# parsaeskandar/pangenome-index

Measured on AMD Instinct MI355X. Metric: find_mems reads/sec (150 bp batch), higher is better.
Workload: dtype u64

## Files before the change

### pangenome-index_amd/csrc/pgx_batch.hip

```cpp
#include <memory>
#include <string>
#include <thread>

#include "pgx_runtime_internal.hpp"

struct pgx_chunk { uint64_t r0, r1, slot_base, slots; };

struct CompactWork {
    DevBuf sizes, tab, bytes, scan_tmp;
    HostBuf h_tab, h_bytes;
    hipEvent_t ev[4] = {nullptr, nullptr, nullptr, nullptr};
    void release() {
        DevBuf *all[] = {&sizes, &tab, &bytes, &scan_tmp};
        for (DevBuf *d : all) d->release();
        h_tab.release(); h_bytes.release();
        for (auto &e : ev)
            if (e) { (void)hipEventDestroy(e); e = nullptr; }
    }
};

struct pgx_batch {
    pgx_index *h = nullptr;
    pgx_device_image *dimg = nullptr;
    int device = 0;
    hipStream_t own = nullptr;
    hipStream_t side = nullptr;
    hipEvent_t ev_side[2] = {nullptr, nullptr};
    bool class_valid = false, class_ok = false;
    uint64_t side_reads_est = 0;
    uint64_t n_reads = 0, read_bytes = 0;
    HostBuf h_off[2];
    int h_off_cur = 0;
    const uint64_t *h_offsets() const { return h_off[h_off_cur].as<uint64_t>(); }
    std::vector<pgx_chunk> chunks;
    bool plan_valid = false, slot_off_valid = false;
    uint64_t slot_off_min_len = 0;
    uint64_t plan_min_len = 0, plan_budget = 0;
    DevBuf reads, offsets;
    DevBuf slot_off, slots, mem_count, mem_off, mems, scan_tmp, counters, heavy_list, heavy_scratch, read_flags, side_list, side_count, packed, ovf_base;
    DevBuf up_side_ids, up_side_off, up_side_bytes;
    DevBuf fx_text, fx_tiles, fx_tile_base, fx_lines, fx_contrib, fx_rec, fx_out_off, fx_rec_idx, fx_offs, fx_scal, fx_scan_tmp;
    std::vector<uint64_t> h_side_off;
    hipEvent_t ev_up[2] = {nullptr, nullptr};
    float ms_upload_passes = 0;
    uint64_t last_ovf_used = 0;
    uint64_t max_read_len = 0;
    TagWork tw;
    LocWork lw;
    CompactWork cw;
    uint64_t n_mems = 0, n_positions = 0, n_ext = 0, n_tag_overflow = 0;
    bool ran = false, ran_tags = false;
    bool shape_valid = false;
    uint64_t shape_reads = 0, shape_min_len = 0, shape_min_occ = 0, last_mems = 0;
    bool shape_tags = false;
    uint32_t spec_runs = 0, spec_fallbacks = 0;
    HostBuf h_mem_off, h_mems, h_run_nums, h_pos_off, h_positions;
    hipEvent_t ev[10] = {nullptr, nullptr, nullptr, nullptr, nullptr, nullptr, nullptr, nullptr, nullptr, nullptr};
    bool timed = false;
    pgx_timing timing{};
};

static void batch_release(pgx_batch *b) {
    if (!b) return;
    if (hipSetDevice(b->device) == hipSuccess) {
        DevBuf *all[] = {&b->reads, &b->offsets, &b->slot_off, &b->slots, &b->mem_count, &b->mem_off, &b->mems, &b->scan_tmp,
                         &b->counters, &b->heavy_list, &b->heavy_scratch, &b->read_flags, &b->side_list, &b->side_count, &b->packed, &b->ovf_base,
                         &b->up_side_ids, &b->up_side_off, &b->up_side_bytes, &b->fx_text, &b->fx_tiles, &b->fx_tile_base, &b->fx_lines,
                         &b->fx_contrib, &b->fx_rec, &b->fx_out_off, &b->fx_rec_idx, &b->fx_offs, &b->fx_scal, &b->fx_scan_tmp};
        for (DevBuf *d : all) d->release();
        b->tw.release();
        b->lw.release();
        b->cw.release();
        HostBuf *hb[] = {&b->h_mem_off, &b->h_mems, &b->h_run_nums, &b->h_pos_off, &b->h_positions, &b->h_off[0], &b->h_off[1]};
        for (HostBuf *x : hb) x->release();
        for (auto &e : b->ev)
            if (e) { (void)hipEventDestroy(e); e = nullptr; }
        if (b->own) { (void)hipStreamDestroy(b->own); b->own = nullptr; }
        if (b->side) { (void)hipStreamDestroy(b->side); b->side = nullptr; }
        for (auto &e : b->ev_side)
            if (e) { (void)hipEventDestroy(e); e = nullptr; }
        for (auto &e : b->ev_up)
            if (e) { (void)hipEventDestroy(e); e = nullptr; }
    }
    delete b;
}

extern "C" void pgx_batch_free(pgx_batch *b) { batch_release(b); }

static void batch_reset_for_upload(pgx_batch *b, uint64_t n_reads, uint64_t max_read_len, uint64_t read_bytes) {
    b->h_off_cur ^= 1;
    b->n_reads = n_reads;
    b->ran = b->ran_tags = false;
    b->lw.valid = false;
    b->plan_valid = false;
    b->slot_off_valid = false;
    b->class_valid = false;
    b->ms_upload_passes = 0;
    b->max_read_len = max_read_len;
    b->read_bytes = read_bytes;
}

static void batch_take_offsets(pgx_batch *b, const uint64_t *offsets, uint64_t n_reads, const char *who) {
    const uint64_t lo = offsets[0];
    HostBuf &hb = b->h_off[b->h_off_cur ^ 1];
    hb.ensure((n_reads + 1) * 8);
    uint64_t *ho = hb.as<uint64_t>();
    ho[0] = 0;
    const unsigned nt = n_reads >= (1u << 20) ? 4u : 1u;
    uint64_t longest[4] = {0, 0, 0, 0};
    bool bad[4] = {false, false, false, false};
    auto slice = [&](unsigned t) {
        const uint64_t i0 = 1 + n_reads * t / nt, i1 = 1 + n_reads * (t + 1) / nt;
        uint64_t prev = offsets[i0 - 1], mx = 0;
        bool b_ = false;
        for (uint64_t i = i0; i < i1; i++) {
            const uint64_t o = offsets[i];
            b_ |= o < prev;
            mx = std::max(mx, o - prev);
            ho[i] = o - lo;
            prev = o;
        }
        longest[t] = mx; bad[t] = b_;
    };
    if (nt == 1) slice(0);
    else {
        std::thread th[3];
        for (unsigned t = 1; t < nt; t++) th[t - 1] = std::thread(slice, t);
        slice(0);
        for (unsigned t = 1; t < nt; t++) th[t - 1].join();
    }
    uint64_t mx = 0;
    for (unsigned t = 0; t < nt; t++) {
        if (bad[t]) throw Error(PGX_ERR_ARG, std::string(who) + ": offsets must be non-decreasing");
        mx = std::max(mx, longest[t]);
    }
    if (mx >= (1ull << 31)) throw Error(PGX_ERR_UNSUPPORTED, "read longer than 2^31 bytes");
    batch_reset_for_upload(b, n_reads, mx, offsets[n_reads] - lo);
    b->offsets.ensure((n_reads + 1) * 8);
    HIPCHECK(hipMemcpyAsync(b->offsets.p, ho, (n_reads + 1) * 8, hipMemcpyHostToDevice, b->own));
}

static void batch_upload(pgx_batch *b, const uint8_t *reads, const uint64_t *offsets, uint64_t n_reads) {
    batch_take_offsets(b, offsets, n_reads, "pgx_batch_upload");
    b->reads.ensure(b->read_bytes + 32);
    HIPCHECK(hipMemsetAsync((uint8_t *)b->reads.p + b->read_bytes, 0, 32, b->own));
    if (b->read_bytes) HIPCHECK(hipMemcpyAsync(b->reads.p, reads + offsets[0], b->read_bytes, hipMemcpyHostToDevice, b->own));
    HIPCHECK(hipStreamSynchronize(b->own));
}

static void batch_upload_packed(pgx_batch *b, const uint32_t *packed, const uint64_t *offsets, uint64_t n_reads, const uint64_t *side_ids,
                                const uint8_t *side_bytes, uint64_t n_side) {
    if (offsets[0] != 0) throw Error(PGX_ERR_ARG, "pgx_batch_upload_packed: offsets[0] must be 0 (word w of the packed stream holds symbols 16 w .. 16 w + 15)");
    if (n_side > n_reads) throw Error(PGX_ERR_ARG, "pgx_batch_upload_packed: more listed reads than reads");
    for (uint64_t k = 0; k < n_side; k++)
        if (side_ids[k] >= n_reads || (k && side_ids[k] <= side_ids[k - 1])) throw Error(PGX_ERR_ARG, "pgx_batch_upload_packed: listed read ids must ascend and lie inside the batch");
    batch_take_offsets(b, offsets, n_reads, "pgx_batch_upload_packed");
    b->h_side_off.resize(n_side + 1);
    b->h_side_off[0] = 0;
    for (uint64_t k = 0; k < n_side; k++) b->h_side_off[k + 1] = b->h_side_off[k] + (offsets[side_ids[k] + 1] - offsets[side_ids[k]]);
    const uint64_t n_chunks = (b->read_bytes + 15) >> 4, side_total = b->h_side_off[n_side];
    hipStream_t s = b->own;
    b->packed.ensure((n_chunks + 64) * 4);
    b->reads.ensure(n_chunks * 16 + 32);
    b->read_flags.ensure(((n_reads + 3) & ~3ull) + 4);
    b->side_list.ensure((n_reads ? n_reads : 1) * sizeof(pgx_heavy_item));
    b->side_count.ensure(16);
    if (n_chunks) HIPCHECK(hipMemcpyAsync(b->packed.p, packed, n_chunks * 4, hipMemcpyHostToDevice, s));
    if (n_side) {
        b->up_side_ids.ensure(n_side * 8);
        b->up_side_off.ensure((n_side + 1) * 8);
        b->up_side_bytes.ensure(side_total ? side_total : 1);
        HIPCHECK(hipMemcpyAsync(b->up_side_ids.p, side_ids, n_side * 8, hipMemcpyHostToDevice, s));
        HIPCHECK(hipMemcpyAsync(b->up_side_off.p, b->h_side_off.data(), (n_side + 1) * 8, hipMemcpyHostToDevice, s));
        if (side_total) HIPCHECK(hipMemcpyAsync(b->up_side_bytes.p, side_bytes, side_total, hipMemcpyHostToDevice, s));
    }
    for (auto &e : b->ev_up)
        if (!e) HIPCHECK(hipEventCreate(&e));
    HIPCHECK(hipEventRecord(b->ev_up[0], s));
    HIPCHECK(hipMemsetAsync(b->side_count.p, 0, 16, s));
    HIPCHECK(hipMemsetAsync(b->read_flags.p, 0, ((n_reads + 3) & ~3ull) + 4, s));
    if (n_chunks) {
        int cus = 0;
        HIPCHECK(hipDeviceGetAttribute(&cus, hipDeviceAttributeMultiprocessorCount, b->device));
        hipLaunchKernelGGL(pgx_unpack_reads_kernel, dim3(std::min<unsigned>(grid_for(n_chunks, 256), (unsigned)cus * 16u)), dim3(256), 0, s, b->packed.as<uint32_t>(), n_chunks,
                           b->reads.as<uint8_t>());
        HIPCHECK(hipGetLastError());
    }
    HIPCHECK(hipMemsetAsync((uint8_t *)b->reads.p + b->read_bytes, 0, 32, s));
    if (n_side) {
        hipLaunchKernelGGL(pgx_side_reads_kernel, dim3(grid_for(n_side * 64, 256)), dim3(256), 0, s, b->reads.as<uint8_t>(), b->offsets.as<uint64_t>(), b->up_side_ids.as<uint64_t>(),
                           b->up_side_off.as<uint64_t>(), b->up_side_bytes.as<uint8_t>(), n_side, b->read_flags.as<uint8_t>(), b->side_list.as<pgx_heavy_item>(),
                           b->side_count.as<unsigned long long>());
        HIPCHECK(hipGetLastError());
    }
    HIPCHECK(hipEventRecord(b->ev_up[1], s));
    HIPCHECK(hipStreamSynchronize(s));
    HIPCHECK(hipEventElapsedTime(&b->ms_upload_passes, b->ev_up[0], b->ev_up[1]));
    b->class_valid = true;
    b->class_ok = true;
    b->side_reads_est = n_side;
}

static void batch_upload_text(pgx_batch *b, const uint8_t *text, uint64_t n_bytes, uint32_t format, uint64_t *n_reads_out) {
    static const char *const fmt_name[3] = {"LINES", "FASTA", "FASTQ"};
    if (n_bytes >= (1ull << 40)) throw Error(PGX_ERR_UNSUPPORTED, "pgx_batch_upload_text: text of 2^40 bytes or more");
    if (n_bytes == 0) {
        static const uint64_t none[1] = {0};
        batch_upload(b, nullptr, none, 0);
        *n_reads_out = 0;
        return;
    }
    hipStream_t s = b->own;
    const uint64_t n_tiles = (n_bytes + PGX_FASTX_TILE - 1) / PGX_FASTX_TILE;
    b->fx_text.ensure(n_bytes + 64);
    b->fx_tiles.ensure(n_tiles * 4);
    b->fx_tile_base.ensure((n_tiles + 1) * 8);
    b->fx_scal.ensure(64);
    unsigned long long *scal = b->fx_scal.as<unsigned long long>();
    HIPCHECK(hipMemcpyAsync(b->fx_text.p, text, n_bytes, hipMemcpyHostToDevice, s));
    HIPCHECK(hipMemsetAsync(scal, 0, 64, s));
    HIPCHECK(hipMemsetAsync(scal, 0xFF, 8, s));
    const uint8_t *dt = b->fx_text.as<uint8_t>();
    hipLaunchKernelGGL(pgx_fastx_count_kernel, dim3(grid_for(n_tiles, 1)), dim3(256), 0, s, dt, n_bytes, b->fx_tiles.as<uint32_t>());
    HIPCHECK(hipGetLastError());
    scan_excl(0, b->fx_tiles.p, n_tiles, 0, b->fx_tile_base.as<uint64_t>(), b->fx_scan_tmp, s);
    const uint64_t n_nl = read_u64(b->fx_tile_base.as<uint64_t>() + n_tiles, s);
    const uint32_t tail = text[n_bytes - 1] != '\n';
    const uint64_t n_lines = n_nl + tail;
    b->fx_lines.ensure((n_lines + 1) * 8);
    b->fx_contrib.ensure(n_lines * 4);
    b->fx_rec.ensure(n_lines);
    b->fx_out_off.ensure((n_lines + 1) * 8);
    b->fx_rec_idx.ensure((n_lines + 1) * 8);
    b->fx_offs.ensure((n_lines + 1) * 8);
    uint64_t *ls = b->fx_lines.as<uint64_t>(), *out_off = b->fx_out_off.as<uint64_t>(), *rec_idx = b->fx_rec_idx.as<uint64_t>(), *offs = b->fx_offs.as<uint64_t>();
    hipLaunchKernelGGL(pgx_fastx_lines_kernel, dim3(grid_for(n_tiles, 1)), dim3(256), 0, s, dt, n_bytes, b->fx_tile_base.as<uint64_t>(), ls, n_lines, tail);
    hipLaunchKernelGGL(pgx_fastx_role_kernel, dim3(grid_for(n_lines, 256)), dim3(256), 0, s, dt, (const uint64_t *)ls, n_lines, format, b->fx_contrib.as<uint32_t>(),
                       b->fx_rec.as<uint8_t>(), scal);
    HIPCHECK(hipGetLastError());
    scan_excl(0, b->fx_contrib.p, n_lines, 0, out_off, b->fx_scan_tmp, s, reinterpret_cast<uint64_t *>(scal + 2));
    scan_excl(4, b->fx_rec.p, n_lines, 0, rec_idx, b->fx_scan_tmp, s, reinterpret_cast<uint64_t *>(scal + 1));
    hipLaunchKernelGGL(pgx_fastx_records_kernel, dim3(grid_for(n_lines, 256)), dim3(256), 0, s, n_lines, format, (const uint32_t *)b->fx_contrib.as<uint32_t>(),
                       (const uint8_t *)b->fx_rec.as<uint8_t>(), (const uint64_t *)out_off, (const uint64_t *)rec_idx, offs, scal);
    hipLaunchKernelGGL(pgx_fastx_longest_kernel, dim3(std::min<unsigned>(grid_for(n_lines, 256), 2048u)), dim3(256), 0, s, (const uint64_t *)offs, (const uint64_t *)(rec_idx + n_lines), scal + 3);
    HIPCHECK(hipGetLastError());
    uint64_t sc[4];
    read_scalars(sc, scal, 32, s);
    if (sc[0] != ~0ull) {
        const uint64_t line = sc[0] >> 8, code = sc[0] & 0xFF, w0 = line >= 2 ? line - 2 : 0;
        uint64_t win[4] = {0, 0, 0, 0}, ri = 0;
        read_scalars(win, ls + w0, (line + 2 - w0) * 8, s);
        ri = read_u64(rec_idx + line, s);
        const uint64_t at = win[line - w0], len = win[line - w0 + 1] - 1 - at;
        const unsigned long long rec = format == PGX_READS_FASTQ ? line / 4 + 1 : format == PGX_READS_FASTA ? std::max<uint64_t>(ri, 1) : ri + 1;
        char msg[256];
        const char *f = fmt_name[format];
        auto stripped = [&](uint64_t a, uint64_t l) { return l - ((l && text[a + l - 1] == '\r') ? 1 : 0); };
        switch (code) {
        case PGX_FASTX_ERR_NO_AT: std::snprintf(msg, sizeof msg, "%s record %llu (byte %llu): header line does not start with '@'", f, rec, (unsigned long long)at); break;
        case PGX_FASTX_ERR_NO_PLUS: std::snprintf(msg, sizeof msg, "%s record %llu (byte %llu): third line does not start with '+'", f, rec, (unsigned long long)at); break;
        case PGX_FASTX_ERR_QUAL_LEN: {
            const uint64_t sa = win[line - 2 - w0], sl = win[line - 1 - w0] - 1 - sa;
            std::snprintf(msg, sizeof msg, "%s record %llu (byte %llu): quality length %llu != sequence length %llu", f, rec, (unsigned long long)at,
                          (unsigned long long)stripped(at, len), (unsigned long long)stripped(sa, sl));
            break;
        }
        case PGX_FASTX_ERR_TRUNCATED:
            std::snprintf(msg, sizeof msg, "%s record %llu (byte %llu): truncated record (%llu of 4 lines)", f, rec, (unsigned long long)at, (unsigned long long)(n_lines - line));
            break;
        case PGX_FASTX_ERR_BEFORE_FIRST: std::snprintf(msg, sizeof msg, "%s record 1 (byte %llu): text before the first '>'", f, (unsigned long long)at); break;
        default: std::snprintf(msg, sizeof msg, "%s record %llu (byte %llu): line of 2^31 bytes or more", f, rec, (unsigned long long)at); break;
        }
        throw Error(code == PGX_FASTX_ERR_LONG_LINE ? PGX_ERR_UNSUPPORTED : PGX_ERR_FORMAT, std::string("pgx_batch_upload_text: ") + msg);
    }
    const uint64_t n_reads = sc[1], total = sc[2], longest = sc[3];
    if (longest >= (1ull << 31)) throw Error(PGX_ERR_UNSUPPORTED, "read longer than 2^31 bytes");
    HostBuf &hb = b->h_off[b->h_off_cur ^ 1];
    hb.ensure((n_reads + 1) * 8);
    b->reads.ensure(total + 32);
    if (total) {
        hipLaunchKernelGGL(pgx_fastx_copy_kernel, dim3(grid_for(total, 4096)), dim3(256), 0, s, dt, (const uint64_t *)ls, (const uint64_t *)out_off, n_lines, total,
                           b->reads.as<uint8_t>());
        HIPCHECK(hipGetLastError());
    }
    HIPCHECK(hipMemsetAsync((uint8_t *)b->reads.p + total, 0, 32, s));
    std::swap(b->offsets, b->fx_offs);
    HIPCHECK(hipMemcpyAsync(hb.p, b->offsets.p, (n_reads + 1) * 8, hipMemcpyDeviceToHost, s));
    HIPCHECK(hipStreamSynchronize(s));
    batch_reset_for_upload(b, n_reads, longest, total);
    *n_reads_out = n_reads;
}

extern "C" pgx_status pgx_batch_create(pgx_index *h, int device, const uint8_t *reads, const uint64_t *offsets,
                                       uint64_t n_reads, pgx_batch **out) {
    PGX_GUARD_BEGIN
    if (!h || !out || !offsets || (!reads && n_reads && offsets[n_reads] != offsets[0]))
        throw Error(PGX_ERR_ARG, "pgx_batch_create: null argument");
    if (!h->has_rank) throw Error(PGX_ERR_ARG, "pgx_batch_create: index opened without an r-index");
    *out = nullptr;
    pgx_device_image *dimg = device_image(h, device);
    ensure_lce(h, dimg);
    std::unique_ptr<pgx_batch, void (*)(pgx_batch *)> b(new pgx_batch(), batch_release);
    b->h = h;
    b->dimg = dimg;
    b->device = device;
    HIPCHECK(hipStreamCreateWithFlags(&b->own, hipStreamNonBlocking));
    batch_upload(b.get(), reads, offsets, n_reads);
    *out = b.release();
    return PGX_OK;
    PGX_GUARD_END
}

extern "C" pgx_status pgx_batch_upload(pgx_batch *b, const uint8_t *reads, const uint64_t *offsets, uint64_t n_reads) {
    PGX_GUARD_BEGIN
    RoctxRange range("pgx_batch_upload");
    if (!b || !offsets || (!reads && n_reads && offsets[n_reads] != offsets[0])) throw Error(PGX_ERR_ARG, "pgx_batch_upload: null argument");
    use_device(b->device);
    batch_upload(b, reads, offsets, n_reads);
    return PGX_OK;
    PGX_GUARD_END
}

extern "C" pgx_status pgx_batch_upload_packed(pgx_batch *b, const uint32_t *packed, const uint64_t *offsets, uint64_t n_reads, const uint64_t *side_ids,
                                              const uint8_t *side_bytes, uint64_t n_side) {
    PGX_GUARD_BEGIN
    RoctxRange range("pgx_batch_upload_packed");
    if (!b || !offsets || (!packed && n_reads && offsets[n_reads] != offsets[0]) || (n_side && (!side_ids || !side_bytes)))
        throw Error(PGX_ERR_ARG, "pgx_batch_upload_packed: null argument");
    use_device(b->device);
    batch_upload_packed(b, packed, offsets, n_reads, side_ids, side_bytes, n_side);
    return PGX_OK;
    PGX_GUARD_END
}

extern "C" pgx_status pgx_batch_upload_text(pgx_batch *b, const uint8_t *text, uint64_t n_bytes, uint32_t format, uint64_t *n_reads) {
    PGX_GUARD_BEGIN
    RoctxRange range("pgx_batch_upload_text");
    if (!b || !n_reads || (!text && n_bytes)) throw Error(PGX_ERR_ARG, "pgx_batch_upload_text: null argument");
    if (format > PGX_READS_FASTQ) throw Error(PGX_ERR_ARG, "pgx_batch_upload_text: unknown format " + std::to_string(format));
    use_device(b->device);
    batch_upload_text(b, text, n_bytes, format, n_reads);
    return PGX_OK;
    PGX_GUARD_END
}


struct RunKnobs {
    bool spec;
    bool arena;
    bool has_arena_cap;
    uint64_t arena_cap;
    uint64_t budget_slots;
    bool narrow;
    bool force_redo;
    bool pairs;
    bool side;
    bool packed;
    int coop;
    bool lce;
    bool has_wg_per_cu;
    int wg_per_cu;
    uint32_t heavy_ext;
    bool has_side_heavy_ext;
    uint32_t side_heavy_ext;
    bool debug_counters;
    bool fm_stats;
};

static RunKnobs read_run_knobs() {
    auto is_set = [](const char *name) { return std::getenv(name) != nullptr; };
    auto not_zero = [](const char *name) { const char *e = std::getenv(name); return !(e && e[0] == '0'); };
    RunKnobs k{};
    k.spec = not_zero("PGX_SPEC");
    k.arena = not_zero("PGX_SLOT_ARENA");
    if (const char *e = std::getenv("PGX_SLOT_ARENA_CAP")) { k.has_arena_cap = true; k.arena_cap = std::strtoull(e, nullptr, 10); }
    if (const char *e = std::getenv("PGX_SLOT_BUDGET_MB")) k.budget_slots = std::max<uint64_t>(1, std::strtoull(e, nullptr, 10)) * (1ull << 20) / sizeof(pgx_mem);
    k.narrow = not_zero("PGX_FM_NARROW");
    k.force_redo = is_set("PGX_FM_NARROW_FORCE_REDO");
    k.pairs = not_zero("PGX_FM_PAIRS");
    k.side = !is_set("PGX_FM_NO_SIDE");
    k.packed = not_zero("PGX_FM_PACKED");
    k.coop = -1;
    if (const char *e = std::getenv("PGX_FM_COOP")) k.coop = e[0] == '1';
    k.lce = not_zero("PGX_FM_LCE");
    if (const char *e = std::getenv("PGX_FM_WG_PER_CU")) { k.has_wg_per_cu = true; k.wg_per_cu = std::atoi(e); }
    k.heavy_ext = PGX_FM_HEAVY_EXT;
    if (const char *e = std::getenv("PGX_FM_HEAVY_EXT")) k.heavy_ext = (uint32_t)std::strtoul(e, nullptr, 10);
    if (const char *e = std::getenv("PGX_FM_SIDE_HEAVY_EXT")) { k.has_side_heavy_ext = true; k.side_heavy_ext = (uint32_t)std::strtoul(e, nullptr, 10); }
    k.debug_counters = is_set("PGX_DEBUG_COUNTERS");
    k.fm_stats = is_set("PGX_FM_STATS");
    return k;
}

static const void *find_mems_entry(bool in_lds, uint32_t kind, bool narrow, bool seeded) {
    using K = const void *;
    static const K tab[2][4][2][2] = {
        {{{(K)pgx_find_mems_kernel<false, 0, false, false>, nullptr}, {nullptr, nullptr}},
         {{(K)pgx_find_mems_kernel<false, 1, false, false>, (K)pgx_find_mems_kernel<false, 1, false, true>},
          {(K)pgx_find_mems_kernel<false, 1, true, false>, (K)pgx_find_mems_kernel<false, 1, true, true>}},
         {{(K)pgx_find_mems_kernel<false, 2, false, false>, (K)pgx_find_mems_kernel<false, 2, false, true>},
          {(K)pgx_find_mems_kernel<false, 2, true, false>, (K)pgx_find_mems_kernel<false, 2, true, true>}},
         {{(K)pgx_find_mems_kernel<false, 3, false, false>, (K)pgx_find_mems_kernel<false, 3, false, true>}, {nullptr, nullptr}}},
        {{{(K)pgx_find_mems_kernel<true, 0, false, false>, nullptr}, {nullptr, nullptr}},
         {{(K)pgx_find_mems_kernel<true, 1, false, false>, (K)pgx_find_mems_kernel<true, 1, false, true>},
          {(K)pgx_find_mems_kernel<true, 1, true, false>, (K)pgx_find_mems_kernel<true, 1, true, true>}},
         {{nullptr, nullptr}, {nullptr, nullptr}},
         {{nullptr, nullptr}, {nullptr, nullptr}}}};
    return kind < 4 ? tab[in_lds][kind][narrow][seeded] : nullptr;
}

static uint32_t find_mems_bits(bool in_lds, uint32_t kind, bool narrow, bool seeded) {
    return PGX_KERNELS_FM | (seeded ? PGX_KERNELS_FM_SEEDED : 0u) | (narrow ? PGX_KERNELS_FM_NARROW : 0u) | (kind << PGX_KERNELS_FM_KIND_SHIFT) | (in_lds ? PGX_KERNELS_FM_LDS : 0u);
}

static const void *find_mems_variant(bool in_lds, uint32_t kind, bool narrow, bool seeded, uint32_t &bits) {
    if (kind == 0) seeded = false;
    const void *f = find_mems_entry(in_lds, kind, narrow, seeded);
    if (!f) throw Error(PGX_ERR_UNSUPPORTED, "pgx_batch_run: no find_mems kernel for this image");
    bits = find_mems_bits(in_lds, kind, narrow, seeded);
    return f;
}

static const void *find_mems_pairs_entry(bool wide, bool packed, bool coop, bool s64, bool lce) {
    using K = const void *;
    static const K plain[2][2] = {
        {(K)pgx_find_mems_pairs_kernel<false, false, false, false, false>, (K)pgx_find_mems_pairs_kernel<false, false, false, true, false>},
        {(K)pgx_find_mems_pairs_kernel<true, false, false, false, false>, (K)pgx_find_mems_pairs_kernel<true, false, false, true, false>}};
    static const K pack[2][2][2] = {
        {{(K)pgx_find_mems_pairs_kernel<false, true, false, false, false>, (K)pgx_find_mems_pairs_kernel<false, true, false, true, false>},
         {(K)pgx_find_mems_pairs_kernel<false, true, true, false, false>, (K)pgx_find_mems_pairs_kernel<false, true, true, true, false>}},
        {{(K)pgx_find_mems_pairs_kernel<true, true, false, false, false>, (K)pgx_find_mems_pairs_kernel<true, true, false, true, false>},
         {(K)pgx_find_mems_pairs_kernel<true, true, true, false, false>, (K)pgx_find_mems_pairs_kernel<true, true, true, true, false>}}};
    static const K with_lce[2] = {(K)pgx_find_mems_pairs_kernel<false, true, false, false, true>, (K)pgx_find_mems_pairs_kernel<false, true, false, true, true>};
    if (lce) return (wide || !packed || coop) ? nullptr : with_lce[s64];
    if (!packed) return coop ? nullptr : plain[wide][s64];
    return pack[wide][coop][s64];
}

static uint32_t find_mems_pairs_bits(bool wide, bool packed, bool coop, bool s64, bool lce) {
    return PGX_KERNELS_PAIRS | (s64 ? PGX_KERNELS_PAIRS_S64 : 0u) | (coop ? PGX_KERNELS_PAIRS_COOP : 0u) | (packed ? PGX_KERNELS_PAIRS_PACKED : 0u) |
           (wide ? PGX_KERNELS_PAIRS_WIDE : 0u) | (lce ? PGX_KERNELS_PAIRS_LCE : 0u);
}

static const void *find_mems_pairs_variant(bool wide, bool packed, bool coop, bool s64, bool lce, uint32_t &bits) {
    const void *f = find_mems_pairs_entry(wide, packed, coop, s64, lce);
    if (!f && lce) throw Error(PGX_ERR_UNSUPPORTED, "pgx_batch_run: no LCE pairs kernel for this image");
    if (!f) throw Error(PGX_ERR_UNSUPPORTED, "pgx_batch_run: no cooperative pairs kernel without the packed reads");
    bits = find_mems_pairs_bits(wide, packed, coop, s64, lce);
    return f;
}

extern "C" uint32_t pgx_kernel_variants(uint32_t *out, uint32_t cap) {
    uint32_t n = 0;
    auto put = [&](uint32_t bits) { if (out && n < cap) out[n] = bits; n++; };
    for (int c = 0; c < 32; c++) {
        const bool in_lds = c & 16, narrow = c & 2, seeded = c & 1;
        const uint32_t kind = (c >> 2) & 3;
        if (find_mems_entry(in_lds, kind, narrow, seeded)) put(find_mems_bits(in_lds, kind, narrow, seeded));
    }
    for (int c = 0; c < 32; c++) {
        const bool wide = c & 16, packed = c & 8, coop = c & 4, s64 = c & 2, lce = c & 1;
        if (find_mems_pairs_entry(wide, packed, coop, s64, lce)) put(find_mems_pairs_bits(wide, packed, coop, s64, lce));
    }
    return n;
}

struct RunCtx {
    pgx_batch *b;
    hipStream_t s;
    RunKnobs k;
    PgxDevImage img;
    uint64_t n, min_len, min_occ;
    bool want_tags;
    unsigned long long *ctr = nullptr;
    bool spec = false, arena_on = false;
    uint64_t cm_cap = 0;
    const void *kfn = nullptr, *kfn_wide = nullptr, *kfn_pairs = nullptr;
    uint32_t kfn_bits = 0, kfn_pairs_bits = 0;
    size_t pairs_lds = 0;
    int cus = 0;
    bool fresh_work = false, fresh_mark = false;
    uint64_t n_ext = 0;
    float ms_fm = 0, ms_cp = 0, ms_main = 0;
};

struct FmArgs {
    PgxDevImage img;
    const uint8_t *reads;
    const uint64_t *off, *slot_off;
    uint64_t n, min_len, min_occ, base, first;
    pgx_mem *slots;
    uint32_t *cnt;
    unsigned long long *next, *cur;
    uint32_t hext, hcap;
    pgx_heavy_item *hlist;
    unsigned long long *hcount;
    uint32_t *ovf;
    uint64_t ovf_cap;
};

static void record(pgx_batch *b, int i, hipStream_t s) {
    static const char *const stage[10] = {"pgx: run begins (classify, sizing)", "pgx: find_mems launches follow", "pgx: find_mems enqueued", "pgx: compaction enqueued",
                                          "pgx: tag locate enqueued", "pgx: tag gather enqueued", "pgx: tag sort/unique enqueued", "pgx: run enqueued", "pgx: main find_mems kernel enqueued",
                                          "pgx: per-upload passes enqueued"};
    if (roctx().on) roctx().mark(stage[i]);
    if (!b->timed) return;
    if (!b->ev[i]) HIPCHECK(hipEventCreate(&b->ev[i]));
    HIPCHECK(hipEventRecord(b->ev[i], s));
}

static unsigned find_mems_grid(const RunCtx &r, const void *kfn, size_t lds, bool few_suffice, uint64_t cn) {
    int wg = 0;
    HIPCHECK(hipOccupancyMaxActiveBlocksPerMultiprocessor(&wg, kfn, PGX_FM_THREADS, lds));
    if (wg < 1) wg = 1;
    if (r.k.has_wg_per_cu) {
        if (r.k.wg_per_cu >= 1 && r.k.wg_per_cu < wg) wg = r.k.wg_per_cu;
    } else if (few_suffice)
        wg = (int)std::min<uint64_t>((uint64_t)wg, std::max<uint64_t>(2, cn / (5ull * (uint64_t)r.cus * PGX_FM_THREADS)));
    return std::min(grid_for(cn, 64), (unsigned)(wg * r.cus));
}

static void plan_slots(RunCtx &r) {
    pgx_batch *b = r.b;
    const uint64_t n = r.n, min_len = r.min_len;
    b->slot_off.ensure((n + 1) * 8);
    if (!b->slot_off_valid || b->slot_off_min_len != min_len) {
        r.fresh_work = true;
        scan_excl(2, b->offsets.p, n, min_len, b->slot_off.as<uint64_t>(), b->scan_tmp, r.s);
        b->slot_off_valid = true;
        b->slot_off_min_len = min_len;
    }
    b->mem_count.ensure((n ? n : 1) * 4);
    b->mem_off.ensure((n + 1) * 8);
    uint64_t budget_slots = (16ull << 30) / sizeof(pgx_mem);
    {
        size_t mem_free = 0, mem_total = 0;
        if (hipMemGetInfo(&mem_free, &mem_total) == hipSuccess) budget_slots = std::max<uint64_t>(budget_slots, (uint64_t)(mem_total / 4) / sizeof(pgx_mem));
        else (void)hipGetLastError();
    }
    if (r.k.budget_slots) budget_slots = r.k.budget_slots;
    if (!b->plan_valid || b->plan_min_len != min_len || b->plan_budget != budget_slots) {
        b->chunks.clear();
        uint64_t r0 = 0, base = 0, acc = 0;
        if (n && b->read_bytes <= budget_slots) b->chunks.push_back({0, n, 0, std::max<uint64_t>(b->read_bytes, 1)});
        else {
            for (uint64_t i = 0; i < n; i++) {
                const uint64_t len = b->h_offsets()[i + 1] - b->h_offsets()[i];
                const uint64_t cap = len < min_len ? 0 : std::min<uint64_t>(len, len - min_len + 1);
                if (acc && acc + cap > budget_slots) { b->chunks.push_back({r0, i, base, acc}); r0 = i; base += acc; acc = 0; }
                acc += cap;
            }
            if (n) b->chunks.push_back({r0, n, base, acc});
        }
        b->plan_valid = true; b->plan_min_len = min_len; b->plan_budget = budget_slots;
    }
    uint64_t max_chunk_reads = 1;
    for (auto &c : b->chunks) max_chunk_reads = std::max(max_chunk_reads, c.r1 - c.r0);
    b->ovf_base.ensure(max_chunk_reads * 4);
}

static void choose_kernels(RunCtx &r) {
    pgx_batch *b = r.b;
    const PgxDevImage &img = r.img;
    const bool in_lds = b->dimg->lds_bytes != 0;
    const bool seeded = img.seed_k != 0 && r.min_len >= img.seed_k;
    r.kfn = r.kfn_wide = find_mems_variant(in_lds, img.dense, false, seeded, r.kfn_bits);
    bool c_fits = true;
    for (int i = 0; i < 8; i++) c_fits = c_fits && !(b->h->img.consts.C[i] >> 32);
    if (img.dense && img.dense != 3 && img.n < (1ull << 30) && c_fits && r.k.narrow) r.kfn = find_mems_variant(in_lds, img.dense, true, seeded, r.kfn_bits);
    r.kfn_pairs = nullptr;
    if (img.pairs && seeded && !(r.n >> 32) && b->read_bytes < (1ull << 35) && r.k.pairs)
        r.kfn_pairs = find_mems_pairs_variant(img.wide != 0, false, false, img.pairs_stride == PGX_PAIRS_STRIDE64, false, r.kfn_pairs_bits);
    r.pairs_lds = img.wide ? (size_t)img.n_sbp * 192 : 0;
    HIPCHECK(hipDeviceGetAttribute(&r.cus, hipDeviceAttributeMultiprocessorCount, b->device));
}

static void classify_reads(RunCtx &r, uint64_t cn) {
    pgx_batch *b = r.b;
    hipStream_t s = r.s;
    r.fresh_work = true;
    const uint64_t cap = std::max<uint64_t>(cn, 1024);
    b->read_flags.ensure(((cn + 3) & ~3ull) + 4);
    b->side_list.ensure((cn ? cn : 1) * sizeof(pgx_heavy_item));
    b->side_count.ensure(16);
    b->scan_tmp.ensure(cap * 8);
    b->scan_tmp.scan_epoch = 0;
    b->packed.ensure(((b->read_bytes + 15) / 16 + 64) * 4);
    HIPCHECK(hipMemsetAsync(b->side_count.p, 0, 16, s));
    HIPCHECK(hipMemsetAsync(b->read_flags.p, 0, ((cn + 3) & ~3ull) + 4, s));
    unsigned long long *d_bad = b->side_count.as<unsigned long long>() + 1;
    hipLaunchKernelGGL(pgx_bad_chunks_kernel, dim3(std::min<unsigned>(grid_for((b->read_bytes + 15) / 16, 256), (unsigned)r.cus * 16u)), dim3(256), 0, s,
                       (const uint8_t *)b->reads.as<uint8_t>(), b->read_bytes, b->scan_tmp.as<uint64_t>(), d_bad, cap, b->packed.as<uint32_t>());
    HIPCHECK(hipGetLastError());
    unsigned long long n_bad = 0;
    read_scalars(&n_bad, d_bad, sizeof n_bad, s);
    b->class_ok = n_bad <= cap;
    b->side_reads_est = n_bad / 4;
    if (b->class_ok && n_bad) {
        hipLaunchKernelGGL(pgx_classify_reads_kernel, dim3(grid_for(n_bad, 256)), dim3(256), 0, s, (const uint8_t *)b->reads.as<uint8_t>(),
                           (const uint64_t *)b->offsets.as<uint64_t>(), cn, (const uint64_t *)b->scan_tmp.as<uint64_t>(), (const unsigned long long *)d_bad, cap,
                           b->read_flags.as<uint32_t>(), b->side_list.as<pgx_heavy_item>(), b->side_count.as<unsigned long long>());
        HIPCHECK(hipGetLastError());
    }
    b->class_valid = true;
}

static void launch_side(RunCtx &r, FmArgs &a, const void *kf, unsigned grid) {
    pgx_batch *b = r.b;
    HIPCHECK(hipEventRecord(b->ev_side[0], r.s));
    HIPCHECK(hipStreamWaitEvent(b->side, b->ev_side[0], 0));
    const pgx_heavy_item *s_list = b->side_list.as<pgx_heavy_item>();
    const unsigned long long *s_count = b->side_count.as<unsigned long long>();
    unsigned long long *s_cur = r.ctr + PGX_CTR_SIDE_CURSOR;
    uint32_t s_hext = r.k.heavy_ext ? std::min<uint32_t>(r.k.heavy_ext, PGX_FM_SIDE_HEAVY_EXT) : 0u;
    if (r.k.has_side_heavy_ext) s_hext = r.k.side_heavy_ext;
    void *sargs[] = {&a.img, &a.reads, &a.off, &a.n, &a.min_len, &a.min_occ, &a.slot_off, &a.slots, &a.cnt, &a.next, &s_cur, &a.first, &a.base,
                     &s_hext, &a.hcap, &a.hlist, &a.hcount, &s_list, &s_count, &a.ovf, &a.ovf_cap};
    const uint64_t cus = (uint64_t)r.cus;
    const unsigned side_wgs = (unsigned)std::min<uint64_t>(4 * cus, std::max<uint64_t>(cus, b->side_reads_est / (2ull * PGX_FM_THREADS) + 1));
    HIPCHECK(hipLaunchKernel(kf, dim3(std::min<unsigned>(grid, side_wgs)), dim3(PGX_FM_THREADS), sargs, b->dimg->lds_bytes, b->side));
    b->timing.kernels |= r.kfn_bits | PGX_KERNELS_SIDE | (kf != r.kfn ? PGX_KERNELS_FM_REDO : 0u);
    HIPCHECK(hipEventRecord(b->ev_side[1], b->side));
}

static void launch_pairs(RunCtx &r, FmArgs &a, const uint8_t *skip, uint64_t cn, unsigned grid) {
    pgx_batch *b = r.b;
    const PgxDevImage &img = r.img;
    const void *kp = r.kfn_pairs;
    uint32_t kp_bits = r.kfn_pairs_bits;
    size_t plds = r.pairs_lds;
    const uint32_t *a_packed = nullptr;
    uint32_t a_pkw = 0;
    const uint32_t pkw = (uint32_t)((15 + b->max_read_len + 15) >> 4) + 1u;
    if (skip && pkw <= 24 && r.k.packed) {
        const bool coop = r.k.coop >= 0 ? r.k.coop != 0 : b->h->img.pairs.size() > (3ull << 30);
        const bool lce = img.lce_sa && !coop && !img.wide && r.min_occ <= 1 && r.k.lce;
        kp = find_mems_pairs_variant(img.wide != 0, true, coop, img.pairs_stride == PGX_PAIRS_STRIDE64, lce, kp_bits);
        const size_t lce_lds = lce ? (size_t)PGX_FM_THREADS * (16 + 4 + 20) : 0;
        a_packed = b->packed.as<uint32_t>();
        a_pkw = pkw;
        plds = (size_t)pkw * PGX_FM_THREADS * 4 + (coop ? (size_t)(PGX_FM_THREADS / 64) * 8192 : 0) + (img.wide ? (size_t)img.n_sbp * 192 : 0) + lce_lds;
        b->timing.pairs_reads = lce ? 4u : coop ? 3u : 2u;
        grid = find_mems_grid(r, kp, plds, true, cn);
    }
    void *pargs[] = {&a.img, &a.reads, &a.off, &a.n, &a.min_len, &a.min_occ, &a.slot_off, &a.slots, &a.cnt, &a.next, &a.cur, &a.first, &a.base,
                     &a.hext, &a.hcap, &a.hlist, &a.hcount, &skip, &a_packed, &a_pkw, &a.ovf, &a.ovf_cap};
    HIPCHECK(hipLaunchKernel(kp, dim3(grid), dim3(PGX_FM_THREADS), pargs, plds, r.s));
    b->timing.kernels |= kp_bits;
}

static uint64_t arena_slots(const RunCtx &r, const pgx_chunk &c) {
    const pgx_batch *b = r.b;
    if (!r.arena_on) return 0;
    const uint64_t cn = c.r1 - c.r0;
    uint64_t want = b->shape_valid && b->shape_reads == r.n && b->shape_min_len == r.min_len && b->chunks.size() == 1 ? with_slack(b->last_ovf_used) + 4096 : 8 * cn + 4096;
    if (r.k.has_arena_cap) want = r.k.arena_cap;
    want = std::max<uint64_t>(want, b->max_read_len + 1);
    want = std::max<uint64_t>(want, (uint64_t)PGX_ARENA_SUBS * (b->max_read_len + 1));
    want = (want + PGX_ARENA_SUBS - 1) / PGX_ARENA_SUBS * PGX_ARENA_SUBS;
    return want < c.slots && want < (1ull << 32) ? want : 0;
}

static uint64_t find_mems_chunk(RunCtx &r, size_t ci, uint64_t &ovf_cap) {
    pgx_batch *b = r.b;
    hipStream_t s = r.s;
    const pgx_chunk &c = b->chunks[ci];
    const uint64_t cn = c.r1 - c.r0;
    const bool one_chunk = b->chunks.size() == 1;
    const uint32_t heavy_ext = r.k.heavy_ext;
    const unsigned grid = find_mems_grid(r, r.kfn_pairs ? r.kfn_pairs : r.kfn, r.kfn_pairs ? r.pairs_lds : b->dimg->lds_bytes, r.img.dense != 0, cn);
    uint64_t *local = b->mem_off.as<uint64_t>() + c.r0;
    const void *kf = r.kfn;
    ovf_cap = arena_slots(r, c);
    for (int attempt = 0;; attempt++) {
        b->slots.ensure(((ovf_cap ? ovf_cap : c.slots) + 4 * cn) * sizeof(pgx_mem));
        if (ci || attempt) {
            HIPCHECK(hipMemsetAsync(r.ctr, 0, PGX_CTR_TAG0 * 8, s));
            HIPCHECK(hipMemsetAsync(r.ctr + PGX_CTR_ARENA0, 0, (PGX_CTR_ALL - PGX_CTR_ARENA0) * 8, s));
        }
        FmArgs a;
        a.img = r.img;
        a.reads = b->reads.as<uint8_t>();
        a.off = b->offsets.as<uint64_t>(); a.slot_off = b->slot_off.as<uint64_t>();
        a.n = c.r1; a.min_len = r.min_len; a.min_occ = r.min_occ; a.base = c.slot_base; a.first = c.r0;
        a.slots = b->slots.as<pgx_mem>();
        a.cnt = b->mem_count.as<uint32_t>();
        a.next = r.ctr; a.cur = r.ctr + PGX_CTR_CURSOR;
        a.hext = heavy_ext; a.hcap = PGX_FM_HEAVY_CAP;
        a.hlist = b->heavy_list.as<pgx_heavy_item>();
        a.hcount = r.ctr + PGX_CTR_HEAVY;
        a.ovf = b->ovf_base.as<uint32_t>() - c.r0;
        a.ovf_cap = ovf_cap;
        bool side_running = false;
        if (r.kfn_pairs) {
            const uint8_t *skip = nullptr;
            if (one_chunk && r.k.side) {
                if (!b->side) {
                    HIPCHECK(hipStreamCreateWithFlags(&b->side, hipStreamNonBlocking));
                    for (auto &e : b->ev_side) HIPCHECK(hipEventCreateWithFlags(&e, hipEventDisableTiming));
                }
                if (!b->class_valid) classify_reads(r, cn);
                record(b, 9, s); r.fresh_mark = true;
                if (b->class_ok) {
                    skip = b->read_flags.as<uint8_t>();
                    launch_side(r, a, kf, grid);
                    side_running = true;
                }
            }
            launch_pairs(r, a, skip, cn, grid);
        } else {
            const pgx_heavy_item *a_rlist = nullptr;
            const unsigned long long *a_rcount = nullptr;
            void *args[] = {&a.img, &a.reads, &a.off, &a.n, &a.min_len, &a.min_occ, &a.slot_off, &a.slots, &a.cnt, &a.next, &a.cur, &a.first, &a.base,
                            &a.hext, &a.hcap, &a.hlist, &a.hcount, &a_rlist, &a_rcount, &a.ovf, &a.ovf_cap};
            if (ci == 0 && attempt == 0) { record(b, 9, s); r.fresh_mark = true; }
            HIPCHECK(hipLaunchKernel(kf, dim3(grid), dim3(PGX_FM_THREADS), args, b->dimg->lds_bytes, s));
            b->timing.kernels |= r.kfn_bits | (kf != r.kfn ? PGX_KERNELS_FM_REDO : 0u);
        }
        record(b, 8, s);
        if (side_running) HIPCHECK(hipStreamWaitEvent(s, b->ev_side[1], 0));
        if (heavy_ext) {
            b->timing.kernels |= PGX_KERNELS_HEAVY;
            if (b->dimg->lds_bytes)
                hipLaunchKernelGGL(pgx_find_mems_heavy_kernel<true>, dim3(PGX_FM_HEAVY_GRID), dim3(256), b->dimg->lds_bytes, s, r.img, a.reads, a.off,
                                   r.min_len, r.min_occ, a.slot_off, c.slot_base, a.slots, a.cnt, r.ctr, (const pgx_heavy_item *)a.hlist,
                                   (const unsigned long long *)a.hcount, (uint32_t)PGX_FM_HEAVY_CAP, b->heavy_scratch.as<PgxHeavyResult>(), c.r0, cn, a.ovf, a.ovf_cap);
            else
                hipLaunchKernelGGL(pgx_find_mems_heavy_kernel<false>, dim3(PGX_FM_HEAVY_GRID), dim3(256), 0, s, r.img, a.reads, a.off, r.min_len, r.min_occ,
                                   a.slot_off, c.slot_base, a.slots, a.cnt, r.ctr, (const pgx_heavy_item *)a.hlist,
                                   (const unsigned long long *)a.hcount, (uint32_t)PGX_FM_HEAVY_CAP, b->heavy_scratch.as<PgxHeavyResult>(), c.r0, cn, a.ovf, a.ovf_cap);
        }
        if (ovf_cap) hipLaunchKernelGGL(pgx_arena_demand_kernel, dim3(1), dim3(PGX_ARENA_SUBS), 0, s, r.ctr);
        HIPCHECK(hipGetLastError());
        b->timing.find_mems_launches++;
        record(b, 2, s);
        scan_excl(0, b->mem_count.as<uint32_t>() + c.r0, cn, 0, local, b->scan_tmp, s, reinterpret_cast<uint64_t *>(r.ctr + PGX_CTR_MEMS));
        if (r.spec) return r.cm_cap;
        unsigned long long cc[16];
        read_scalars(cc, r.ctr, sizeof cc, s);
        if (ovf_cap) b->last_ovf_used = cc[PGX_CTR_OVF_TOP];
        if (ovf_cap && cc[PGX_CTR_OVF_ABORT]) { ovf_cap = 0; continue; }
        const bool forced = attempt == 0 && kf != r.kfn_wide && r.k.force_redo;
        if ((cc[PGX_CTR_OVF32] || forced) && kf != r.kfn_wide) { kf = r.kfn_wide; continue; }
        r.n_ext += cc[PGX_CTR_EXT];
        b->timing.heavy_reads += (uint32_t)std::min<unsigned long long>(cc[PGX_CTR_HEAVY], PGX_FM_HEAVY_CAP);
        b->timing.pairs_other_steps += (uint32_t)cc[PGX_CTR_REDO];
        return cc[PGX_CTR_MEMS];
    }
}

static void compact_chunk(RunCtx &r, const pgx_chunk &c, uint64_t cm, uint64_t mem_base, uint64_t ovf_cap) {
    pgx_batch *b = r.b;
    hipStream_t s = r.s;
    const uint64_t cn = c.r1 - c.r0;
    b->mems.ensure_keep((mem_base + cm ? mem_base + cm : 1) * sizeof(pgx_mem), mem_base * sizeof(pgx_mem));
    hipLaunchKernelGGL(pgx_compact_mems_kernel, dim3(grid_for(cn, 256)), dim3(256), 0, s, c.r0, cn, b->slot_off.as<uint64_t>(),
                       c.slot_base, b->slots.as<pgx_mem>(), b->mem_count.as<uint32_t>(), (const uint64_t *)(b->mem_off.as<uint64_t>() + c.r0), mem_base,
                       b->mems.as<pgx_mem>(), r.spec ? r.cm_cap : ~0ull, reinterpret_cast<uint64_t *>(r.ctr + PGX_CTR_ABORT),
                       (const uint32_t *)(b->ovf_base.as<uint32_t>() - c.r0), ovf_cap);
    HIPCHECK(hipGetLastError());
    record(b, 3, s);
    if (b->timed && b->chunks.size() > 1) {
        HIPCHECK(hipStreamSynchronize(s));
        float t1 = 0, t2 = 0, t3 = 0;
        HIPCHECK(hipEventElapsedTime(&t1, b->ev[1], b->ev[2]));
        HIPCHECK(hipEventElapsedTime(&t2, b->ev[2], b->ev[3]));
        HIPCHECK(hipEventElapsedTime(&t3, b->ev[1], b->ev[8]));
        r.ms_fm += t1; r.ms_cp += t2; r.ms_main += t3;
    }
}

static bool read_back(RunCtx &r, bool &force_worst) {
    pgx_batch *b = r.b;
    const size_t n_chunks = b->chunks.size();
    unsigned long long cnt[PGX_CTR_SLOTS];
    read_scalars(cnt, b->counters.p, sizeof cnt, r.s);
    if (r.spec) {
        b->spec_runs++;
        if (cnt[PGX_CTR_OVF_ABORT]) { force_worst = true; b->last_ovf_used = cnt[PGX_CTR_OVF_TOP]; }
        if (r.k.debug_counters)
            std::fprintf(stderr, "[pgx] speculative run: abort flags %llu, 32-bit overflow %llu, arena overflow %llu (top %llu), MEMs %llu of capacity %llu\n", cnt[PGX_CTR_ABORT], cnt[PGX_CTR_OVF32],
                         cnt[PGX_CTR_OVF_ABORT], cnt[PGX_CTR_OVF_TOP], cnt[PGX_CTR_MEMS], (unsigned long long)r.cm_cap);
        if (cnt[PGX_CTR_ABORT] || cnt[PGX_CTR_OVF32] || cnt[PGX_CTR_OVF_ABORT] || cnt[PGX_CTR_MEMS] > r.cm_cap) { b->spec_fallbacks++; b->ran_tags = false; return false; }
        b->last_ovf_used = cnt[PGX_CTR_OVF_TOP];
        b->n_mems = cnt[PGX_CTR_MEMS];
        r.n_ext = cnt[PGX_CTR_EXT];
        b->timing.heavy_reads = (uint32_t)std::min<unsigned long long>(cnt[PGX_CTR_HEAVY], PGX_FM_HEAVY_CAP);
        b->timing.pairs_other_steps = (uint32_t)cnt[PGX_CTR_REDO];
        if (r.want_tags) {
            TagWork &w = b->tw;
            const unsigned long long *tc = cnt + PGX_CTR_TAG0;
            w.last_big = tc[0]; w.last_large = tc[1]; w.last_largest = tc[2]; w.last_G = tc[3]; w.last_small = tc[5];
            w.last_rep = tc[6]; w.last_dup = tc[7]; w.last_P = tc[8];
            w.n_positions = tc[8];
            b->n_positions = tc[8];
        }
    }
    if (r.kfn_pairs) {
        b->timing.main_lines = cnt[PGX_CTR_PAIRS_LINES]; b->timing.main_seed_loads = cnt[PGX_CTR_PAIRS_SEEDS];
        b->timing.other_lines = cnt[PGX_CTR_FM_LINES]; b->timing.other_seed_loads = cnt[PGX_CTR_FM_SEEDS];
        b->timing.two_step_trips = cnt[PGX_CTR_PAIRS_TWO];
    } else { b->timing.main_lines = cnt[PGX_CTR_FM_LINES]; b->timing.main_seed_loads = cnt[PGX_CTR_FM_SEEDS]; }
    b->last_mems = b->n_mems;
    b->shape_valid = true; b->shape_reads = r.n; b->shape_min_len = r.min_len; b->shape_min_occ = r.min_occ; b->shape_tags = r.want_tags;
    if (cnt[PGX_CTR_ST_TRIPS] && r.k.fm_stats)
        std::fprintf(stderr, "[pgx] find_mems wave trips %llu, live lane-trips %llu (%.1f%% of lanes), longest wave %llu trips, extensions %llu\n", cnt[PGX_CTR_ST_TRIPS],
                     cnt[PGX_CTR_ST_LIVE], 100.0 * (double)cnt[PGX_CTR_ST_LIVE] / (64.0 * (double)cnt[PGX_CTR_ST_TRIPS]), cnt[PGX_CTR_ST_LONGEST], cnt[PGX_CTR_EXT]);
    if (cnt[PGX_CTR_ST_PAIR_TRIPS] && r.k.fm_stats)
        std::fprintf(stderr, "[pgx] pairs kernel wave trips %llu, live lane-trips %llu (%.1f%%), with two extensions %llu, waiting for a second block %llu, fresh %llu, extensions through the other image %llu\n",
                     cnt[PGX_CTR_ST_PAIR_TRIPS], cnt[PGX_CTR_ST_PAIR_LIVE], 100.0 * (double)cnt[PGX_CTR_ST_PAIR_LIVE] / (64.0 * (double)cnt[PGX_CTR_ST_PAIR_TRIPS]),
                     cnt[PGX_CTR_PAIRS_TWO], cnt[PGX_CTR_ST_PAIR_WAIT], cnt[PGX_CTR_ST_PAIR_FRESH], cnt[PGX_CTR_REDO]);
    if (cnt[PGX_CTR_ST_PAIR_T_TOTAL] && r.k.fm_stats)
        std::fprintf(stderr, "[pgx] pairs kernel clock ticks: %.1f%% of the waves' time in the refill loop (%llu of %llu), %llu trips with a refill round; waiting for the seed entry %.1f%%, then for the block line %.1f%%\n",
                     100.0 * (double)cnt[PGX_CTR_ST_PAIR_T_REFILL] / (double)cnt[PGX_CTR_ST_PAIR_T_TOTAL], cnt[PGX_CTR_ST_PAIR_T_REFILL], cnt[PGX_CTR_ST_PAIR_T_TOTAL], cnt[PGX_CTR_ST_PAIR_REFILLS],
                     100.0 * (double)cnt[PGX_CTR_ST_PAIR_T_SEED] / (double)cnt[PGX_CTR_ST_PAIR_T_TOTAL], 100.0 * (double)cnt[PGX_CTR_ST_PAIR_T_LINE] / (double)cnt[PGX_CTR_ST_PAIR_T_TOTAL]);
    if (r.k.debug_counters)
        std::fprintf(stderr, "[pgx] counters: extensions %llu tag overflows %llu heavy %llu other-image steps %llu lines %llu + %llu seeds %llu + %llu\n", cnt[PGX_CTR_EXT], cnt[PGX_CTR_TAG_OVERFLOW],
                     cnt[PGX_CTR_HEAVY], cnt[PGX_CTR_REDO], cnt[PGX_CTR_PAIRS_LINES], cnt[PGX_CTR_FM_LINES], cnt[PGX_CTR_PAIRS_SEEDS], cnt[PGX_CTR_FM_SEEDS]);
    b->n_ext = r.n_ext;
    b->n_tag_overflow = cnt[PGX_CTR_TAG_OVERFLOW];
    if (b->timed) {
        auto el = [&](int a, int c) { float ms = 0; HIPCHECK(hipEventElapsedTime(&ms, b->ev[a], b->ev[c])); return ms; };
        b->timing.ms_find_mems = n_chunks > 1 ? r.ms_fm : el(1, 2);
        b->timing.ms_find_mems_main = n_chunks > 1 ? r.ms_main : (r.n ? el(1, 8) : 0.0f);
        b->timing.ms_compact = n_chunks > 1 ? r.ms_cp : el(2, 3);
        if (r.want_tags) {
            b->timing.ms_tag_locate = el(3, 4);
            b->timing.ms_tag_gather = el(4, 5);
            b->timing.ms_tag_sort = el(5, 6);
        }
        b->timing.ms_total = el(0, 7);
        if (r.fresh_work) b->timing.ms_per_upload = b->ms_upload_passes + (r.fresh_mark ? el(0, 9) : 0.0f);
    }
    if (r.fresh_work) b->ms_upload_passes = 0;
    return true;
}

static bool run_pass(RunCtx &r, bool may_speculate, bool &force_worst) {
    pgx_batch *b = r.b;
    hipStream_t s = r.s;
    b->n_mems = b->n_positions = b->n_ext = b->n_tag_overflow = 0;
    std::memset(&b->timing, 0, sizeof b->timing);
    r.fresh_work = r.fresh_mark = false;
    r.n_ext = 0;
    r.ms_fm = r.ms_cp = r.ms_main = 0;
    b->counters.ensure(PGX_CTR_ALL * 8);
    HIPCHECK(hipMemsetAsync(b->counters.p, 0, PGX_CTR_ALL * 8, s));
    r.ctr = b->counters.as<unsigned long long>();

    record(b, 0, s);
    plan_slots(r);
    const std::vector<pgx_chunk> &chunks = b->chunks;
    r.arena_on = r.k.arena && !force_worst;
    r.kfn = r.kfn_wide = r.kfn_pairs = nullptr;
    r.cus = 0;
    if (r.n) choose_kernels(r);
    if (r.k.heavy_ext) {
        b->heavy_list.ensure((size_t)PGX_FM_HEAVY_CAP * sizeof(pgx_heavy_item));
        b->heavy_scratch.ensure((size_t)PGX_FM_HEAVY_GRID * PGX_FM_HEAVY_MAXLEN * sizeof(PgxHeavyResult));
    }
    r.spec = may_speculate && chunks.size() == 1 && b->shape_valid && b->shape_reads == r.n && b->shape_min_len == r.min_len && b->shape_min_occ == r.min_occ &&
             b->shape_tags == r.want_tags && (!r.want_tags || (b->tw.have_last && b->tw.last_largest <= PGX_SORT_WG_LDS_CAP)) && r.k.spec && !r.k.force_redo;
    r.cm_cap = with_slack(b->last_mems);
    uint64_t mem_base = 0;
    for (size_t ci = 0; ci < chunks.size(); ci++) {
        record(b, 1, s);
        uint64_t ovf_cap = 0;
        const uint64_t cm = find_mems_chunk(r, ci, ovf_cap);
        compact_chunk(r, chunks[ci], cm, mem_base, ovf_cap);
        mem_base += cm;
    }
    b->n_mems = mem_base;
    if (!r.kfn_pairs) b->timing.pairs_reads = 0u;
    else if (!b->timing.pairs_reads) b->timing.pairs_reads = 1u;
    b->timing.seed_depth = (r.img.seed_k != 0 && r.min_len >= r.img.seed_k && r.img.dense) ? r.img.seed_k : 0u;
    if (chunks.size() != 1) {
        if (chunks.empty()) { record(b, 1, s); record(b, 2, s); }
        scan_excl(0, b->mem_count.p, r.n, 0, b->mem_off.as<uint64_t>(), b->scan_tmp, s);
        b->mems.ensure_keep((b->n_mems ? b->n_mems : 1) * sizeof(pgx_mem), b->n_mems * sizeof(pgx_mem));
        record(b, 3, s);
    }
    record(b, 3, s);
    if (r.want_tags) {
        tag_pipeline(r.img, b->mems.as<pgx_mem>(), nullptr, nullptr, b->n_mems, b->tw, r.ctr + PGX_CTR_TAG_OVERFLOW, r.ctr + PGX_CTR_TAG0, s,
                     [&](int stage) { record(b, 4 + stage, s); }, r.spec, reinterpret_cast<const uint64_t *>(r.ctr + PGX_CTR_MEMS),
                     reinterpret_cast<uint64_t *>(r.ctr + PGX_CTR_ABORT));
        b->n_positions = b->tw.n_positions;
        b->ran_tags = true;
    }
    record(b, 7, s);
    return read_back(r, force_worst);
}

extern "C" pgx_status pgx_batch_run(pgx_batch *b, uint64_t min_len, uint64_t min_occ, uint32_t flags, void *stream) {
    PGX_GUARD_BEGIN
    RoctxRange range("pgx_batch_run");
    if (!b) throw Error(PGX_ERR_ARG, "pgx_batch_run: null batch");
    use_device(b->device);
    RunCtx r{b, stream ? (hipStream_t)stream : b->own, read_run_knobs(), b->dimg->img, b->n_reads, min_len, min_occ, (flags & PGX_RUN_TAGS) != 0};
    PgxDevImage &img = r.img;
    if (img.seed_k_main && min_len < img.seed_k_main && img.seed_k_small && min_len >= img.seed_k_small) { img.seed = img.seed_small; img.seed_k = img.seed_k_small; }
    if (r.want_tags && !b->h->has_tags) throw Error(PGX_ERR_ARG, "pgx_batch_run: PGX_RUN_TAGS without a tag array");
    b->timed = (flags & PGX_RUN_TIMING) != 0;
    b->ran = false;
    b->ran_tags = false;
    b->lw.valid = false;
    b->n_mems = b->n_positions = b->n_ext = b->n_tag_overflow = 0;
    std::memset(&b->timing, 0, sizeof b->timing);
    bool force_worst = false;
    if (!run_pass(r, true, force_worst)) run_pass(r, false, force_worst);
    b->ran = true;
    return PGX_OK;
    PGX_GUARD_END
}

extern "C" pgx_status pgx_batch_device_result(pgx_batch *b, pgx_device_result *out) {
    PGX_GUARD_BEGIN
    if (!b || !out || !b->ran) throw Error(PGX_ERR_ARG, "pgx_batch_device_result: batch has not been run");
    std::memset(out, 0, sizeof *out);
    out->n_reads = b->n_reads;
    out->n_mems = b->n_mems;
    out->mem_offsets = b->mem_off.as<uint64_t>();
    out->mems = b->mems.as<pgx_mem>();
    if (b->ran_tags) {
        out->n_positions = b->n_positions;
        out->tag_run_counts = b->tw.run_nums.as<uint64_t>();
        out->pos_offsets = b->tw.pos_off.as<uint64_t>();
        out->positions = b->tw.positions.as<uint64_t>();
    }
    return PGX_OK;
    PGX_GUARD_END
}

extern "C" pgx_status pgx_batch_counts(pgx_batch *b, uint64_t *n_mems, uint64_t *n_positions, uint64_t *n_extensions) {
    PGX_GUARD_BEGIN
    if (!b || !b->ran) throw Error(PGX_ERR_ARG, "pgx_batch_counts: batch has not been run");
    if (n_mems) *n_mems = b->n_mems;
    if (n_positions) *n_positions = b->n_positions;
    if (n_extensions) *n_extensions = b->n_ext;
    return PGX_OK;
    PGX_GUARD_END
}

extern "C" pgx_status pgx_batch_spec_stats(pgx_batch *b, uint32_t *speculative_runs, uint32_t *fallbacks) {
    PGX_GUARD_BEGIN
    if (!b) throw Error(PGX_ERR_ARG, "pgx_batch_spec_stats: null batch");
    if (speculative_runs) *speculative_runs = b->spec_runs;
    if (fallbacks) *fallbacks = b->spec_fallbacks;
    return PGX_OK;
    PGX_GUARD_END
}

extern "C" pgx_status pgx_batch_timing(pgx_batch *b, pgx_timing *out) {
    PGX_GUARD_BEGIN
    if (!b || !out || !b->ran) throw Error(PGX_ERR_ARG, "pgx_batch_timing: batch has not been run");
    if (!b->timed) throw Error(PGX_ERR_ARG, "pgx_batch_timing: run without PGX_RUN_TIMING");
    *out = b->timing;
    return PGX_OK;
    PGX_GUARD_END
}

extern "C" pgx_status pgx_batch_result(pgx_batch *b, pgx_result *out) {
    PGX_GUARD_BEGIN
    RoctxRange range("pgx_batch_result");
    if (!b || !out || !b->ran) throw Error(PGX_ERR_ARG, "pgx_batch_result: batch has not been run");
    use_device(b->device);
    const uint64_t n = b->n_reads, m = b->n_mems;
    b->h_mem_off.ensure((n + 1) * 8);
    HIPCHECK(hipMemcpyAsync(b->h_mem_off.p, b->mem_off.p, (n + 1) * 8, hipMemcpyDeviceToHost, b->own));
    b->h_mems.ensure((m ? m : 1) * sizeof(pgx_mem));
    if (m) HIPCHECK(hipMemcpyAsync(b->h_mems.p, b->mems.p, m * sizeof(pgx_mem), hipMemcpyDeviceToHost, b->own));
    std::memset(out, 0, sizeof *out);
    out->n_reads = n;
    out->n_mems = m;
    out->mem_offsets = b->h_mem_off.as<uint64_t>();
    out->mems = b->h_mems.as<pgx_mem>();
    out->n_extensions = b->n_ext;
    if (b->ran_tags) {
        b->h_run_nums.ensure((m ? m : 1) * 8);
        b->h_pos_off.ensure((m + 1) * 8);
        b->h_positions.ensure((b->n_positions ? b->n_positions : 1) * 8);
        if (m) HIPCHECK(hipMemcpyAsync(b->h_run_nums.p, b->tw.run_nums.p, m * 8, hipMemcpyDeviceToHost, b->own));
        HIPCHECK(hipMemcpyAsync(b->h_pos_off.p, b->tw.pos_off.p, (m + 1) * 8, hipMemcpyDeviceToHost, b->own));
        if (b->n_positions) HIPCHECK(hipMemcpyAsync(b->h_positions.p, b->tw.positions.p, b->n_positions * 8, hipMemcpyDeviceToHost, b->own));
        out->tag_run_counts = b->h_run_nums.as<uint64_t>();
        out->pos_offsets = b->h_pos_off.as<uint64_t>();
        out->positions = b->h_positions.as<uint64_t>();
        out->n_positions = b->n_positions;
        out->n_tag_overflow = b->n_tag_overflow;
    }
    HIPCHECK(hipStreamSynchronize(b->own));
    return PGX_OK;
    PGX_GUARD_END
}

static uint64_t compact_tables(CompactWork &w, const uint64_t *d_mem_off, const pgx_mem *d_mems, const uint64_t *d_run_nums, const uint64_t *d_pos_off,
                               const uint64_t *d_positions, uint64_t n_reads, bool tags, bool timed, hipStream_t s) {
    const uint64_t nb = (n_reads + PGX_COMPACT_BLOCK_READS - 1) / PGX_COMPACT_BLOCK_READS;
    w.sizes.ensure((nb ? nb : 1) * 8);
    w.tab.ensure(3 * (nb + 1) * 8);
    w.h_tab.ensure(3 * (nb + 1) * 8);
    uint64_t *bo = w.tab.as<uint64_t>(), *fm = bo + (nb + 1), *fp = fm + (nb + 1);
    if (timed) {
        for (auto &e : w.ev)
            if (!e) HIPCHECK(hipEventCreate(&e));
        HIPCHECK(hipEventRecord(w.ev[0], s));
    }
    hipLaunchKernelGGL(pgx_compact_size_kernel, dim3(grid_for(nb + 1, 4)), dim3(256), 0, s, d_mem_off, d_mems, d_run_nums, d_pos_off, d_positions, n_reads, nb,
                       tags ? 1 : 0, w.sizes.as<uint64_t>(), fm, fp);
    HIPCHECK(hipGetLastError());
    scan_excl(1, w.sizes.p, nb, 0, bo, w.scan_tmp, s);
    if (timed) HIPCHECK(hipEventRecord(w.ev[1], s));
    HIPCHECK(hipMemcpyAsync(w.h_tab.p, w.tab.p, 3 * (nb + 1) * 8, hipMemcpyDeviceToHost, s));
    HIPCHECK(hipStreamSynchronize(s));
    return w.h_tab.as<uint64_t>()[nb];
}

static void compact_fill(CompactWork &w, const uint64_t *d_mem_off, const pgx_mem *d_mems, const uint64_t *d_run_nums, const uint64_t *d_pos_off,
                         const uint64_t *d_positions, uint64_t n_reads, bool tags, bool timed, uint64_t total, hipStream_t s) {
    const uint64_t nb = (n_reads + PGX_COMPACT_BLOCK_READS - 1) / PGX_COMPACT_BLOCK_READS;
    w.bytes.ensure(total ? total : 8);
    if (timed) HIPCHECK(hipEventRecord(w.ev[2], s));
    if (nb) {
        const char *e = std::getenv("PGX_COMPACT_STAGE");
        const bool staged = e && e[0] == '1' && e[1] == 0;
        hipLaunchKernelGGL(staged ? pgx_compact_fill_staged_kernel : pgx_compact_fill_kernel, dim3(grid_for(nb, 4)), dim3(256), 0, s, d_mem_off, d_mems, d_run_nums, d_pos_off, d_positions, n_reads, nb,
                           tags ? 1 : 0, (const uint64_t *)w.tab.as<uint64_t>(), w.bytes.as<uint8_t>());
        HIPCHECK(hipGetLastError());
    }
    if (timed) HIPCHECK(hipEventRecord(w.ev[3], s));
}

static float compact_ms(CompactWork &w) {
    float a = 0, c = 0;
    HIPCHECK(hipEventElapsedTime(&a, w.ev[0], w.ev[1]));
    HIPCHECK(hipEventElapsedTime(&c, w.ev[2], w.ev[3]));
    return a + c;
}

extern "C" pgx_status pgx_batch_result_compact(pgx_batch *b, pgx_compact_result *out) {
    PGX_GUARD_BEGIN
    RoctxRange range("pgx_batch_result_compact");
    checked_device_count();
    if (!b || !out || !b->ran) throw Error(PGX_ERR_ARG, "pgx_batch_result_compact: batch has not been run");
    use_device(b->device);
    CompactWork &w = b->cw;
    hipStream_t s = b->own;
    const bool tags = b->ran_tags, timed = b->timed;
    const uint64_t n = b->n_reads, nb = (n + PGX_COMPACT_BLOCK_READS - 1) / PGX_COMPACT_BLOCK_READS;
    const uint64_t *run_nums = tags ? b->tw.run_nums.as<uint64_t>() : nullptr, *pos_off = tags ? b->tw.pos_off.as<uint64_t>() : nullptr;
    const uint64_t *positions = tags ? b->tw.positions.as<uint64_t>() : nullptr;
    const uint64_t total = compact_tables(w, b->mem_off.as<uint64_t>(), b->mems.as<pgx_mem>(), run_nums, pos_off, positions, n, tags, timed, s);
    compact_fill(w, b->mem_off.as<uint64_t>(), b->mems.as<pgx_mem>(), run_nums, pos_off, positions, n, tags, timed, total, s);
    w.h_bytes.ensure(total ? total : 8);
    if (total) HIPCHECK(hipMemcpyAsync(w.h_bytes.p, w.bytes.p, total, hipMemcpyDeviceToHost, s));
    HIPCHECK(hipStreamSynchronize(s));
    std::memset(out, 0, sizeof *out);
    out->n_reads = n;
    out->n_mems = b->n_mems;
    out->n_extensions = b->n_ext;
    if (tags) {
        out->n_positions = b->n_positions;
        out->n_tag_overflow = b->n_tag_overflow;
        out->flags = PGX_COMPACT_TAGS;
    }
    out->block_reads = PGX_COMPACT_BLOCK_READS;
    out->n_blocks = nb;
    out->n_bytes = total;
    out->block_offsets = w.h_tab.as<uint64_t>();
    out->block_first_mem = out->block_offsets + (nb + 1);
    out->block_first_pos = out->block_first_mem + (nb + 1);
    out->bytes = w.h_bytes.as<uint8_t>();
    out->ms_encode = timed ? compact_ms(w) : 0;
    return PGX_OK;
    PGX_GUARD_END
}

extern "C" pgx_status pgx_compact_encode(int device, const pgx_result *in, uint8_t *bytes, uint64_t bytes_cap, uint64_t *block_offsets,
                                         uint64_t *block_first_mem, uint64_t *block_first_pos, uint64_t *n_bytes) {
    PGX_GUARD_BEGIN
    RoctxRange range("pgx_compact_encode");
    use_device(device);
    if (!in || !in->mem_offsets || (in->n_mems && !in->mems) || (bytes_cap && !bytes) || !block_offsets || !block_first_mem || !block_first_pos || !n_bytes)
        throw Error(PGX_ERR_ARG, "pgx_compact_encode: null argument");
    const bool tags = in->pos_offsets != nullptr;
    const uint64_t n = in->n_reads, m = in->n_mems, np = tags ? in->n_positions : 0;
    if (tags && ((m && !in->tag_run_counts) || (np && !in->positions))) throw Error(PGX_ERR_ARG, "pgx_compact_encode: pos_offsets without tag_run_counts / positions");
    auto check_csr = [](const uint64_t *off, uint64_t cnt, uint64_t last, const char *name) {
        bool ok = off[0] == 0 && off[cnt] == last;
        for (uint64_t i = 0; ok && i < cnt; i++) ok = off[i] <= off[i + 1];
        if (!ok) throw Error(PGX_ERR_ARG, std::string("pgx_compact_encode: ") + name + " must start at 0, never decrease and end at the count of what it indexes");
    };
    check_csr(in->mem_offsets, n, m, "mem_offsets");
    if (tags) check_csr(in->pos_offsets, m, np, "pos_offsets");
    struct Work {
        DevBuf mem_off, mems, run_nums, pos_off, positions;
        CompactWork w;
        ~Work() {
            DevBuf *all[] = {&mem_off, &mems, &run_nums, &pos_off, &positions};
            for (DevBuf *d : all) d->release();
            w.release();
        }
    } k;
    upload(k.mem_off, in->mem_offsets, (n + 1) * 8);
    upload(k.mems, in->mems, m * sizeof(pgx_mem));
    if (tags) {
        upload(k.run_nums, in->tag_run_counts, m * 8);
        upload(k.pos_off, in->pos_offsets, (m + 1) * 8);
        upload(k.positions, in->positions, np * 8);
    }
    hipStream_t s = nullptr;
    const uint64_t nb = (n + PGX_COMPACT_BLOCK_READS - 1) / PGX_COMPACT_BLOCK_READS;
    const uint64_t total = compact_tables(k.w, k.mem_off.as<uint64_t>(), k.mems.as<pgx_mem>(), k.run_nums.as<uint64_t>(), k.pos_off.as<uint64_t>(),
                                          k.positions.as<uint64_t>(), n, tags, false, s);
    *n_bytes = total;
    const uint64_t *t = k.w.h_tab.as<uint64_t>();
    std::memcpy(block_offsets, t, (nb + 1) * 8);
    std::memcpy(block_first_mem, t + (nb + 1), (nb + 1) * 8);
    std::memcpy(block_first_pos, t + 2 * (nb + 1), (nb + 1) * 8);
    if (total > bytes_cap)
        throw Error(PGX_ERR_NOMEM, "pgx_compact_encode: the stream takes " + std::to_string(total) + " bytes, bytes_cap is " + std::to_string(bytes_cap));
    compact_fill(k.w, k.mem_off.as<uint64_t>(), k.mems.as<pgx_mem>(), k.run_nums.as<uint64_t>(), k.pos_off.as<uint64_t>(), k.positions.as<uint64_t>(), n, tags,
                 false, total, s);
    if (total) HIPCHECK(hipMemcpyAsync(bytes, k.w.bytes.p, total, hipMemcpyDeviceToHost, s));
    HIPCHECK(hipStreamSynchronize(s));
    return PGX_OK;
    PGX_GUARD_END
}

static uint64_t locate_budget_values() {
    uint64_t bytes = 0;
    if (const char *e = std::getenv("PGX_LOCATE_BUDGET_MB")) {
        const double mb = std::strtod(e, nullptr);
        if (mb > 0) bytes = (uint64_t)(mb * 1048576.0);
    }
    if (!bytes) {
        size_t mem_free = 0, mem_total = 0;
        if (hipMemGetInfo(&mem_free, &mem_total) != hipSuccess) { (void)hipGetLastError(); mem_free = 1ull << 30; }
        bytes = mem_free / 4;
    }
    return std::max<uint64_t>(bytes / 8, 1);
}

static bool locate_sets_enabled() {
    const char *e = std::getenv("PGX_LOCATE_SETS");
    return !(e && e[0] == '0' && e[1] == 0);
}

extern "C" pgx_status pgx_batch_locate(pgx_batch *b, uint32_t flags, uint64_t max_occ, void *stream) {
    PGX_GUARD_BEGIN
    RoctxRange range("pgx_batch_locate");
    if ((flags & PGX_LOCATE_SEQ_SETS) && (flags & (PGX_LOCATE_SEQ_IDS | PGX_LOCATE_UNIQUE)))
        throw Error(PGX_ERR_ARG, "pgx_batch_locate: PGX_LOCATE_SEQ_SETS goes with PGX_LOCATE_CHAINS alone");
    checked_device_count();
    if (!b) throw Error(PGX_ERR_ARG, "pgx_batch_locate: null batch");
    if (flags & ~(PGX_LOCATE_SEQ_IDS | PGX_LOCATE_UNIQUE | PGX_LOCATE_CHAINS | PGX_LOCATE_SEQ_SETS)) throw Error(PGX_ERR_ARG, "pgx_batch_locate: unknown flag");
    if (!b->ran) throw Error(PGX_ERR_ARG, "pgx_batch_locate: batch has not been run");
    LocWork &w = b->lw;
    w.valid = false;
    locate_check_supported(b->h, "pgx_batch_locate");
    use_device(b->device);
    pgx_device_image *d = locate_image(b->h, b->device);
    hipStream_t s = stream ? (hipStream_t)stream : b->own;
    const uint64_t n = b->n_mems, bwt_n = d->loc.n;
    const bool sets_form = (flags & PGX_LOCATE_SEQ_SETS) != 0;
    const bool seq_ids = sets_form || (flags & PGX_LOCATE_SEQ_IDS) != 0, uniq = (flags & PGX_LOCATE_UNIQUE) != 0;
    const uint64_t n_seq = b->h->ri.C.size() > 1 ? b->h->ri.C[1] - b->h->ri.C[0] : 0;
    const uint64_t W = (n_seq + 63) / 64;
    const bool sets_fit = W >= 1 && W <= PGX_ML_SET_WORDS_MAX;
    if (sets_form && !sets_fit)
        throw Error(PGX_ERR_UNSUPPORTED, "pgx_batch_locate: PGX_LOCATE_SEQ_SETS serves at most " + std::to_string(64 * PGX_ML_SET_WORDS_MAX) + " sequences, the index has " +
                                             std::to_string(n_seq));
    const bool routed = !sets_form && seq_ids && uniq && sets_fit && locate_sets_enabled();
    const bool build_sets = sets_form || routed, sort_uniq = uniq && !routed;
    const bool resident = !(flags & PGX_LOCATE_CHAINS) && d->lce_state == 1 && d->img.lce_sa && d->lce_seq_start.p && d->lce_n_seq && d->img.n == bwt_n;
    const bool timed = b->timed;
    if (timed) {
        for (auto &e : w.ev)
            if (!e) HIPCHECK(hipEventCreate(&e));
        HIPCHECK(hipEventRecord(w.ev[0], s));
    }
    w.cnt.ensure((n ? n : 1) * 8); w.qs.ensure((n ? n : 1) * 8); w.qe.ensure((n ? n : 1) * 8); w.voff.ensure((n + 1) * 8); w.ctr.ensure(64);
    unsigned long long *ctr = w.ctr.as<unsigned long long>();
    HIPCHECK(hipMemsetAsync(w.ctr.p, 0, 64, s));
    if (n) {
        hipLaunchKernelGGL(pgx_ml_plan_kernel, dim3(grid_for(n, 256)), dim3(256), 0, s, (const pgx_mem *)b->mems.as<pgx_mem>(), n, bwt_n, max_occ,
                           w.cnt.as<uint64_t>(), w.qs.as<uint64_t>(), w.qe.as<uint64_t>(), ctr + 4);
        HIPCHECK(hipGetLastError());
    }
    scan_excl(1, w.cnt.p, n, 0, w.voff.as<uint64_t>(), w.scan_tmp, s, reinterpret_cast<uint64_t *>(ctr + 5));
    uint64_t tot[2];
    read_scalars(tot, ctr + 4, 16, s);
    const uint64_t n_not = tot[0], V = tot[1];
    const uint64_t *voff = w.voff.as<uint64_t>();
    const uint64_t budget = locate_budget_values();
    if (sets_form) {
        w.vals.ensure((n ? n * W : 1) * 8); w.uoff.ensure((n + 1) * 8);
        if (n) HIPCHECK(hipMemsetAsync(w.vals.p, 0, n * W * 8, s));
        hipLaunchKernelGGL(pgx_ml_stride_kernel, dim3(grid_for(n + 1, 256)), dim3(256), 0, s, w.uoff.as<uint64_t>(), n + 1, W);
        HIPCHECK(hipGetLastError());
    } else if (!uniq) w.vals.ensure((V ? V : 1) * 8);
    else { w.ucount.ensure((n ? n : 1) * 8); w.uoff.ensure((n + 1) * 8); }
    const bool value_buffer = sort_uniq || (build_sets && !resident);
    const uint64_t set_mems = std::max<uint64_t>(budget / (W ? W : 1), 1);
    uint64_t U = 0;
    for (uint64_t m0 = 0, o0 = 0; m0 < n;) {
        uint64_t m1 = n, o1 = V;
        const bool by_values = !(build_sets && resident) && V - o0 > budget;
        const uint64_t m_lim = routed && n - m0 > set_mems ? m0 + set_mems : n;
        if (by_values || m_lim < n) {
            hipLaunchKernelGGL(pgx_ml_cut_kernel, dim3(1), dim3(64), 0, s, voff, m_lim, m0, by_values ? budget : V, reinterpret_cast<uint64_t *>(ctr + 6));
            HIPCHECK(hipGetLastError());
            uint64_t c[2];
            read_scalars(c, ctr + 6, 16, s);
            m1 = c[0]; o1 = c[1];
        }
        const uint64_t np = m1 - m0, nv = o1 - o0;
        if (value_buffer) w.gbuf.ensure((nv ? nv : 1) * 8);
        uint64_t *dst = value_buffer ? w.gbuf.as<uint64_t>() : w.vals.as<uint64_t>() + o0;
        unsigned long long *sets = nullptr;
        if (sets_form) sets = w.vals.as<unsigned long long>() + m0 * W;
        else if (routed) {
            w.sets.ensure(np * W * 8);
            sets = w.sets.as<unsigned long long>();
            HIPCHECK(hipMemsetAsync(sets, 0, np * W * 8, s));
        }
        if (nv && resident && build_sets) {
            hipLaunchKernelGGL(pgx_ml_sets_kernel, dim3(grid_for(nv, PGX_ML_SPAN)), dim3(256), 0, s, (const pgx_mem *)b->mems.as<pgx_mem>(), voff, m0, m1, o0, nv,
                               (const uint32_t *)d->img.lce_sa, bwt_n, (const uint64_t *)d->lce_seq_start.as<uint64_t>(), d->lce_n_seq, (uint32_t)W, sets);
            HIPCHECK(hipGetLastError());
        } else if (nv && resident) {
            hipLaunchKernelGGL(pgx_ml_gather_kernel, dim3(grid_for(nv, PGX_ML_SPAN)), dim3(256), 0, s, (const pgx_mem *)b->mems.as<pgx_mem>(), voff, m0, m1, o0, nv,
                               (const uint32_t *)d->img.lce_sa, bwt_n, (const uint64_t *)d->lce_seq_start.as<uint64_t>(), d->lce_n_seq, d->loc.max_length,
                               seq_ids ? 1 : 0, dst);
            HIPCHECK(hipGetLastError());
        } else if (nv) {
            w.run0.ensure(np * 8); w.npieces.ensure(np * 8); w.poff.ensure((np + 1) * 8);
            const uint64_t *qs = w.qs.as<uint64_t>() + m0, *qe = w.qe.as<uint64_t>() + m0;
            hipLaunchKernelGGL(pgx_locate_plan_kernel, dim3(grid_for(np, 256)), dim3(256), 0, s, d->loc, qs, qe, np, w.run0.as<uint64_t>(), w.npieces.as<uint64_t>());
            HIPCHECK(hipGetLastError());
            scan_excl(1, w.npieces.p, np, 0, w.poff.as<uint64_t>(), w.scan_tmp, s);
            const uint64_t n_pieces = read_u64(w.poff.as<uint64_t>() + np, s);
            if (n_pieces) {
                hipLaunchKernelGGL(pgx_locate_walk_kernel, dim3(grid_for(n_pieces, 256)), dim3(256), 0, s, d->loc, qs, qe, np, (const uint64_t *)w.run0.as<uint64_t>(),
                                   (const uint64_t *)w.poff.as<uint64_t>(), n_pieces, voff + m0, o0, seq_ids ? 1 : 0, dst);
                HIPCHECK(hipGetLastError());
                if (build_sets) {
                    hipLaunchKernelGGL(pgx_ml_sets_ids_kernel, dim3(grid_for(nv, PGX_ML_SPAN)), dim3(256), 0, s, voff, m0, m1, o0, nv, (const uint64_t *)dst, (uint32_t)W,
                                       sets);
                    HIPCHECK(hipGetLastError());
                }
            }
        }
        if (routed) {
            uint32_t Wp = 1;
            while (Wp < W) Wp <<= 1;
            uint64_t *ucount = w.ucount.as<uint64_t>() + m0;
            w.uloc.ensure((np + 1) * 8);
            hipLaunchKernelGGL(pgx_ml_set_count_kernel, dim3(grid_for(np * Wp, 256)), dim3(256), 0, s, (const unsigned long long *)sets, np, (uint32_t)W, Wp, ucount);
            HIPCHECK(hipGetLastError());
            scan_excl(1, ucount, np, 0, w.uloc.as<uint64_t>(), w.scan_tmp, s, reinterpret_cast<uint64_t *>(ctr + 3));
            const uint64_t Up = read_u64(reinterpret_cast<const uint64_t *>(ctr + 3), s);
            w.vals.ensure_keep((U + Up ? U + Up : 1) * 8, U * 8);
            if (Up) {
                hipLaunchKernelGGL(pgx_ml_set_expand_kernel, dim3(grid_for(np, 4)), dim3(256), 0, s, (const unsigned long long *)sets, np, (uint32_t)W,
                                   (const uint64_t *)w.uloc.as<uint64_t>(), w.vals.as<uint64_t>() + U);
                HIPCHECK(hipGetLastError());
            }
            U += Up;
        }
        if (sort_uniq) {
            w.seg.ensure((np + 1) * 8); w.lists.ensure(2 * np * 8); w.need.ensure(np * 8); w.soff.ensure((np + 1) * 8); w.uloc.ensure((np + 1) * 8);
            uint64_t *seg = w.seg.as<uint64_t>(), *wave_list = w.lists.as<uint64_t>(), *wg_list = wave_list + np, *ucount = w.ucount.as<uint64_t>() + m0;
            const uint64_t *cnt = w.cnt.as<uint64_t>() + m0;
            HIPCHECK(hipMemsetAsync(w.ctr.p, 0, 32, s));
            hipLaunchKernelGGL(pgx_ml_classify_kernel, dim3(grid_for(np + 1, 256)), dim3(256), 0, s, cnt, voff + m0, np, seg, wave_list, wg_list,
                               w.need.as<uint64_t>(), ucount, ctr);
            HIPCHECK(hipGetLastError());
            scan_excl(1, w.need.p, np, 0, w.soff.as<uint64_t>(), w.scan_tmp, s, reinterpret_cast<uint64_t *>(ctr + 2));
            uint64_t c[3];
            read_scalars(c, ctr, 24, s);
            const uint64_t n_wave = c[0], n_wg = c[1], S = c[2];
            if (n_wave)
                hipLaunchKernelGGL(pgx_tag_sort_unique_kernel<PgxTagDense>, dim3(grid_for(n_wave, 4)), dim3(256), 0, s, PgxTagDense{wave_list, cnt, seg}, n_wave,
                                   (const uint64_t *)nullptr, (const uint64_t *)nullptr, w.gbuf.as<uint64_t>(), ucount);
            if (n_wg) {
                w.scratch.ensure((S ? S : 1) * 8);
                HIPCHECK(hipFuncSetAttribute((const void *)pgx_tag_sort_large_kernel<PgxTagDense>, hipFuncAttributeMaxDynamicSharedMemorySize, (int)(PGX_SORT_WG_LDS_CAP * 8)));
                hipLaunchKernelGGL(pgx_tag_sort_large_kernel<PgxTagDense>, dim3(grid_for(n_wg, 1)), dim3(1024), (size_t)PGX_SORT_WG_LDS_CAP * 8, s, PgxTagDense{wg_list, cnt, seg},
                                   n_wg, (const uint64_t *)nullptr, (const uint64_t *)nullptr, w.gbuf.as<uint64_t>(), w.scratch.as<uint64_t>(),
                                   (const uint64_t *)w.soff.as<uint64_t>(), ucount);
            }
            HIPCHECK(hipGetLastError());
            scan_excl(1, ucount, np, 0, w.uloc.as<uint64_t>(), w.scan_tmp, s, reinterpret_cast<uint64_t *>(ctr + 3));
            const uint64_t Up = read_u64(reinterpret_cast<const uint64_t *>(ctr + 3), s);
            w.vals.ensure_keep((U + Up ? U + Up : 1) * 8, U * 8);
            if (Up) {
                hipLaunchKernelGGL(pgx_tag_compact_kernel<PgxTagDense>, dim3(grid_for(np, 16)), dim3(256), 0, s, PgxTagDense{nullptr, nullptr, seg}, np,
                                   (const uint64_t *)nullptr, (const uint64_t *)nullptr, (const uint64_t *)ucount, (const uint64_t *)w.gbuf.as<uint64_t>(),
                                   (const uint64_t *)w.uloc.as<uint64_t>(), w.vals.as<uint64_t>() + U, ~0ull);
                HIPCHECK(hipGetLastError());
            }
            U += Up;
        }
        m0 = m1; o0 = o1;
    }
    if (uniq) scan_excl(1, w.ucount.p, n, 0, w.uoff.as<uint64_t>(), w.scan_tmp, s);
    w.vals.ensure(8);
    if (timed) HIPCHECK(hipEventRecord(w.ev[1], s));
    HIPCHECK(hipStreamSynchronize(s));
    w.ms = 0;
    if (timed) HIPCHECK(hipEventElapsedTime(&w.ms, w.ev[0], w.ev[1]));
    w.d_off = uniq || sets_form ? w.uoff.as<uint64_t>() : voff;
    w.n_mems = n;
    w.n_values = sets_form ? n * W : uniq ? U : V;
    w.n_not_located = n_not;
    w.flags = flags & (PGX_LOCATE_SEQ_IDS | PGX_LOCATE_UNIQUE | PGX_LOCATE_SEQ_SETS);
    w.set_words = build_sets ? (uint32_t)W : 0;
    w.resident = resident;
    w.valid = true;
    return PGX_OK;
    PGX_GUARD_END
}

static void locations_header(const pgx_batch *b, pgx_locations *out) {
    const LocWork &w = b->lw;
    std::memset(out, 0, sizeof *out);
    out->n_mems = w.n_mems;
    out->n_values = w.n_values;
    out->n_not_located = w.n_not_located;
    out->flags = w.flags;
    out->resident = w.resident ? 1u : 0u;
    out->ms_locate = w.ms;
    out->set_words = w.set_words;
}

extern "C" pgx_status pgx_batch_device_locations(pgx_batch *b, pgx_locations *out) {
    PGX_GUARD_BEGIN
    if (!b || !out || !b->lw.valid) throw Error(PGX_ERR_ARG, "pgx_batch_device_locations: batch has no locate result");
    locations_header(b, out);
    out->loc_offsets = b->lw.d_off;
    out->values = b->lw.vals.as<uint64_t>();
    return PGX_OK;
    PGX_GUARD_END
}

extern "C" pgx_status pgx_batch_locations(pgx_batch *b, pgx_locations *out) {
    PGX_GUARD_BEGIN
    if (!b || !out || !b->lw.valid) throw Error(PGX_ERR_ARG, "pgx_batch_locations: batch has no locate result");
    use_device(b->device);
    LocWork &w = b->lw;
    w.h_off.ensure((w.n_mems + 1) * 8);
    w.h_vals.ensure((w.n_values ? w.n_values : 1) * 8);
    HIPCHECK(hipMemcpyAsync(w.h_off.p, w.d_off, (w.n_mems + 1) * 8, hipMemcpyDeviceToHost, b->own));
    if (w.n_values) HIPCHECK(hipMemcpyAsync(w.h_vals.p, w.vals.p, w.n_values * 8, hipMemcpyDeviceToHost, b->own));
    HIPCHECK(hipStreamSynchronize(b->own));
    locations_header(b, out);
    out->loc_offsets = w.h_off.as<uint64_t>();
    out->values = w.h_vals.as<uint64_t>();
    return PGX_OK;
    PGX_GUARD_END
}

extern "C" pgx_status pgx_find_mems_batch(pgx_index *h, int device, const uint8_t *reads, const uint64_t *offsets,
                                          uint64_t n_reads, uint64_t min_len, uint64_t min_occ, uint32_t flags,
                                          pgx_batch **batch_out, pgx_result *result_out) {
    if (!batch_out || !result_out) { pgx::set_last_error("pgx_find_mems_batch: null argument"); return PGX_ERR_ARG; }
    *batch_out = nullptr;
    pgx_batch *b = nullptr;
    pgx_status st = pgx_batch_create(h, device, reads, offsets, n_reads, &b);
    if (st == PGX_OK) st = pgx_batch_run(b, min_len, min_occ, flags, nullptr);
    if (st == PGX_OK) st = pgx_batch_result(b, result_out);
    if (st != PGX_OK) { pgx_batch_free(b); return st; }
    *batch_out = b;
    return PGX_OK;
}

extern "C" pgx_status pgx_find_mems_sharded(pgx_index *h, const int *devices, uint32_t n_slices, const uint8_t *reads, const uint64_t *offsets,
                                            uint64_t n_reads, uint64_t min_len, uint64_t min_occ, uint32_t flags, pgx_batch **batches_out,
                                            pgx_result *results_out, uint64_t *first_read) {
    PGX_GUARD_BEGIN
    if (!h || !devices || !n_slices || !offsets || !batches_out || !results_out || !first_read)
        throw Error(PGX_ERR_ARG, "pgx_find_mems_sharded: null argument");
    for (uint32_t i = 0; i < n_slices; i++) { batches_out[i] = nullptr; first_read[i] = n_reads * i / n_slices; }
    first_read[n_slices] = n_reads;
    for (uint32_t i = 0; i < n_slices; i++) (void)device_image(h, devices[i]);
    std::vector<pgx_status> st(n_slices, PGX_OK);
    std::vector<std::string> err(n_slices);
    std::vector<std::thread> th;
    for (uint32_t i = 0; i < n_slices; i++)
        th.emplace_back([&, i]() {
            const uint64_t a = first_read[i], b = first_read[i + 1];
            st[i] = pgx_find_mems_batch(h, devices[i], reads, offsets + a, b - a, min_len, min_occ, flags, &batches_out[i], &results_out[i]);
            if (st[i] != PGX_OK) err[i] = pgx_last_error();
        });
    for (auto &t : th) t.join();
    for (uint32_t i = 0; i < n_slices; i++)
        if (st[i] != PGX_OK) {
            for (uint32_t k = 0; k < n_slices; k++) { pgx_batch_free(batches_out[k]); batches_out[k] = nullptr; }
            throw Error(st[i], "slice " + std::to_string(i) + " (device " + std::to_string(devices[i]) + "): " + err[i]);
        }
    return PGX_OK;
    PGX_GUARD_END
}
```

### pangenome-index_amd/csrc/pgx_device.h

```cpp
#pragma once

#include <hip/hip_runtime.h>
#include <stdint.h>

#include "../../include/pgx.h"
#include "pgx_image.h"

enum PgxCounterSlot {
    PGX_CTR_EXT = 0,
    PGX_CTR_TAG_OVERFLOW = 1,
    PGX_CTR_CURSOR = 5,
    PGX_CTR_HEAVY = 8,
    PGX_CTR_OVF32 = 9,
    PGX_CTR_MEMS = 10,
    PGX_CTR_REDO = 11,
    PGX_CTR_REDO_CURSOR = 12,
    PGX_CTR_SIDE_CURSOR = 13,
    PGX_CTR_OVF_TOP = 14,
    PGX_CTR_OVF_ABORT = 15,
    PGX_CTR_TAG0 = 16,
    PGX_CTR_ABORT = 30,
    PGX_CTR_PAIRS_LINES = 32,
    PGX_CTR_PAIRS_SEEDS = 33,
    PGX_CTR_FM_LINES = 34,
    PGX_CTR_FM_SEEDS = 35,
    PGX_CTR_PAIRS_TWO = 36,
    PGX_CTR_ST_TRIPS = 40, PGX_CTR_ST_LIVE = 41, PGX_CTR_ST_LONGEST = 42,
    PGX_CTR_ST_PAIR_TRIPS = 43, PGX_CTR_ST_PAIR_LIVE = 44, PGX_CTR_ST_PAIR_WAIT = 45, PGX_CTR_ST_PAIR_FRESH = 46,
    PGX_CTR_ST_PAIR_T_REFILL = 47, PGX_CTR_ST_PAIR_T_TOTAL = 48, PGX_CTR_ST_PAIR_REFILLS = 49, PGX_CTR_ST_PAIR_T_SEED = 50, PGX_CTR_ST_PAIR_T_LINE = 51,
    PGX_CTR_SLOTS = 64,
    PGX_CTR_ARENA0 = 64,
    PGX_CTR_ALL = 64 + 16 * 64
};
#define PGX_ARENA_SUBS 64u
#define PGX_TBUCKET_RUNS 10u

#define PGX_DENSE_LDS_U4 5
#define PGX_FM_THREADS 256
#define PGX_LCE_MAX_OCC 128u
#define PGX_FM_WAVES_PER_SIMD 4

struct PgxDevImage {
    const uint4 *blocks;
    const uint64_t *dir;
    const uint16_t *blow;
    const PgxConsts *consts;
    const uint64_t *tstart;
    const uint64_t *tvals;
    const uint32_t *tdir;
    const ulonglong2 *tpair;
    const uint4 *tbucket;
    uint64_t n_tbuckets;
    uint32_t tbucket_shift;
    uint64_t n;
    uint64_t dir_entries;
    uint64_t n_tag_runs, n_tag_items, tag_dir_entries;
    uint32_t n_blocks;
    uint32_t dir_shift;
    uint32_t excl_mask;
    uint32_t tag_dir_shift;
    uint32_t dense;
    const uint32_t *exc;
    uint32_t seed_k;
    const uint4 *seed;
    uint32_t seed_end_k;
    const uint4 *seed_end;
    uint32_t seed_k_main, seed_k_small;
    const uint4 *seed_main, *seed_small;
    const uint4 *pairs;
    const uint4 *first_ext;
    uint32_t pair_runs;
    const uint64_t *sbase2, *pbase;
    uint32_t d2_sb_shift, pairs_sb_shift, n_sb2, n_sbp;
    uint32_t wide;
    uint32_t pairs_stride;
    const uint32_t *lce_sa;
    const uint32_t *lce_text;
    const uint32_t *lce_flags;
    const uint8_t *lce_lcp;
    uint32_t lce_max;
    uint32_t refill_min;
};
#define PGX_LCP_CAP 254u
#define PGX_LCP_UNKNOWN 255u
#define PGX_SEED_UNUSABLE 255u
#define PGX_SEED_MAX_K 16
#define PGX_SEED_SMALL_K 10

struct pgx_heavy_item {
    uint64_t rid;
    uint32_t x, nm;
};
struct PgxHeavyResult {
    pgx_mem mem;
    uint32_t next_x, n_ext, has_mem, pad;
};
#define PGX_FM_HEAVY_EXT 2048u
#define PGX_FM_SIDE_HEAVY_EXT 2048u
#define PGX_FM_HEAVY_MAXLEN 4096u
#define PGX_FM_HEAVY_CAP 8192u
#define PGX_FM_HEAVY_GRID 64u

template <bool LDS_IMAGE, int DENSE, bool NARROW, bool SEED>
__global__ void pgx_find_mems_kernel(PgxDevImage img, const uint8_t *reads, const uint64_t *offsets, uint64_t n_reads,
                                     uint64_t min_len, uint64_t min_occ, const uint64_t *slot_off, pgx_mem *slots,
                                     uint32_t *mem_count, unsigned long long *n_ext_total, unsigned long long *cursor, uint64_t first_read,
                                     uint64_t slot_base, uint32_t heavy_ext, uint32_t heavy_cap, pgx_heavy_item *heavy_list, unsigned long long *heavy_count,
                                     const pgx_heavy_item *rid_list, const unsigned long long *rid_count, uint32_t *ovf_base, uint64_t ovf_cap);
template <bool LDS_IMAGE>
__global__ void pgx_find_mems_heavy_kernel(PgxDevImage img, const uint8_t *reads, const uint64_t *offsets, uint64_t min_len, uint64_t min_occ,
                                           const uint64_t *slot_off, uint64_t slot_base, pgx_mem *slots, uint32_t *mem_count,
                                           unsigned long long *n_ext_total, const pgx_heavy_item *heavy_list,
                                           const unsigned long long *heavy_count, uint32_t heavy_cap, PgxHeavyResult *scratch, uint64_t chunk_first,
                                           uint64_t chunk_reads, uint32_t *ovf_base, uint64_t ovf_cap);
__global__ void pgx_fmf_kernel(PgxDevImage img, const uint8_t *reads, const uint64_t *offsets, const uint64_t *read_of, const uint64_t *xs, uint64_t n,
                               uint64_t min_len, uint64_t min_occ, PgxHeavyResult *out);
__global__ void pgx_arena_demand_kernel(unsigned long long *ctr);

template <bool WIDE, bool PACKED, bool COOP, bool S64, bool LCE>
__global__ void pgx_find_mems_pairs_kernel(PgxDevImage img, const uint8_t *reads, const uint64_t *offsets, uint64_t n_reads,
                                           uint64_t min_len, uint64_t min_occ, const uint64_t *slot_off, pgx_mem *slots,
                                           uint32_t *mem_count, unsigned long long *n_ext_total, unsigned long long *cursor, uint64_t first_read,
                                           uint64_t slot_base, uint32_t heavy_ext, uint32_t heavy_cap, pgx_heavy_item *heavy_list, unsigned long long *heavy_count,
                                           const uint8_t *skip, const uint32_t *packed, uint32_t pk_words,
                                           uint32_t *ovf_base, uint64_t ovf_cap);

__global__ void pgx_bad_chunks_kernel(const uint8_t *reads, uint64_t n_bytes, uint64_t *chunks, unsigned long long *count, uint64_t cap, uint32_t *packed);
__global__ void pgx_unpack_reads_kernel(const uint32_t *packed, uint64_t n_chunks, uint8_t *reads);
__global__ void pgx_side_reads_kernel(uint8_t *reads, const uint64_t *offsets, const uint64_t *side_ids, const uint64_t *side_off, const uint8_t *side_bytes, uint64_t n_side,
                                      uint8_t *flags, pgx_heavy_item *list, unsigned long long *count);
__global__ void pgx_classify_reads_kernel(const uint8_t *reads, const uint64_t *offsets, uint64_t n_reads, const uint64_t *chunks, const unsigned long long *n_chunks,
                                          uint64_t cap, uint32_t *flag_words, pgx_heavy_item *list, unsigned long long *count);

__global__ void pgx_seed_build_kernel(PgxDevImage img, const uint4 *src, uint4 *dst, uint32_t level, uint64_t n_dst, uint64_t limit, int end_table);
__global__ void pgx_first_ext_kernel(PgxDevImage img, uint4 *out);
__global__ void pgx_rank_kernel(PgxDevImage img, const uint64_t *pos, uint64_t n, int true_codes, uint64_t *out);
template <bool LOOP, bool MULHI> __global__ void pgx_rank_probe_kernel(PgxDevImage img, const uint64_t *pos, uint64_t n, uint64_t *out);
template <bool LDS_IMAGE>
__global__ void pgx_extend_kernel(PgxDevImage img, const pgx_biint *in, const uint8_t *sym, const uint8_t *forward, uint64_t n,
                                  pgx_biint *out);
template <bool LDS_IMAGE>
__global__ void pgx_count_kernel(PgxDevImage img, const uint8_t *reads, const uint64_t *offsets, uint64_t n_reads, pgx_range *out);
__global__ void pgx_lf_kernel(PgxDevImage img, const pgx_range *in, const uint8_t *sym, uint64_t n, pgx_range *out);

__global__ void pgx_scan_partial_kernel(int mode, const void *in, const void *in2, uint64_t n, uint64_t min_len, uint64_t *block_sums, const uint64_t *n_dev);
template <int MODE>
__global__ void pgx_scan_onepass_kernel(const void *in, uint64_t n, uint64_t min_len, uint64_t *out, uint64_t *total_out, const uint64_t *n_dev,
                                        unsigned long long *state, uint32_t epoch);
__global__ void pgx_scan_sums_kernel(uint64_t *block_sums, uint64_t nb);
__global__ void pgx_scan_tag_tail_kernel(const uint64_t *run_nums, const uint64_t *uval, uint64_t n, const uint64_t *n_dev, uint64_t *pos_off, uint64_t *total_out,
                                         uint64_t *positions, uint64_t pos_cap, uint64_t *abort, unsigned long long *state, uint32_t epoch);
__global__ void pgx_scan_apply_kernel(int mode, const void *in, const void *in2, uint64_t n, uint64_t min_len, const uint64_t *block_sums,
                                      uint64_t nb, uint64_t *out, uint64_t *total_out, int raw_sums, const uint64_t *n_dev);
__global__ void pgx_compact_mems_kernel(uint64_t first_read, uint64_t n_reads, const uint64_t *slot_off, uint64_t slot_base,
                                        const pgx_mem *slots, const uint32_t *mem_count, const uint64_t *local_off,
                                        uint64_t mem_base, pgx_mem *mems, uint64_t cap_mems, uint64_t *abort, const uint32_t *ovf_base, uint64_t ovf_cap);

__global__ void pgx_compact_size_kernel(const uint64_t *mem_off, const pgx_mem *mems, const uint64_t *run_nums, const uint64_t *pos_off,
                                        const uint64_t *positions, uint64_t n_reads, uint64_t n_blocks, int tags, uint64_t *sizes, uint64_t *first_mem,
                                        uint64_t *first_pos);
__global__ void pgx_compact_fill_kernel(const uint64_t *mem_off, const pgx_mem *mems, const uint64_t *run_nums, const uint64_t *pos_off,
                                        const uint64_t *positions, uint64_t n_reads, uint64_t n_blocks, int tags, const uint64_t *block_offsets,
                                        uint8_t *bytes);
__global__ void pgx_compact_fill_staged_kernel(const uint64_t *mem_off, const pgx_mem *mems, const uint64_t *run_nums, const uint64_t *pos_off,
                                               const uint64_t *positions, uint64_t n_reads, uint64_t n_blocks, int tags, const uint64_t *block_offsets,
                                               uint8_t *bytes);

__global__ void pgx_tag_pair_kernel(const uint64_t *tstart, const uint64_t *tvals, uint64_t n_runs, uint64_t n_items, ulonglong2 *out);
__global__ void pgx_tag_bucket_kernel(const uint64_t *tstart, const uint64_t *tvals, uint64_t n_runs, uint64_t n_items, uint32_t shift, uint64_t n_buckets, uint4 *out);
#define PGX_TAG_LOCATE_THREADS 1024
#define PGX_SORT_LDS_CAP 2048
#define PGX_TAG_SMALL 16
#define PGX_SORT_WG_LDS_CAP 16384

struct __attribute__((aligned(32))) PgxTagRec { uint64_t q, first, cnt, seg; };
struct PgxTagRecs {
    const PgxTagRec *recs;
    __device__ __forceinline__ void get(uint64_t e, uint64_t &q, uint64_t &cnt, uint64_t &seg) const { const PgxTagRec r = recs[e]; q = r.q; cnt = r.cnt; seg = r.seg; }
    __device__ __forceinline__ uint64_t scratch_index(uint64_t e, uint64_t q) const { return e; }
};
struct PgxTagDense {
    const uint64_t *list, *cnt, *seg;
    __device__ __forceinline__ void get(uint64_t e, uint64_t &q, uint64_t &c, uint64_t &s) const { q = list ? list[e] : e; c = cnt ? cnt[q] : 0; s = seg[q]; }
    __device__ __forceinline__ uint64_t scratch_index(uint64_t e, uint64_t q) const { return q; }
};

__global__ void pgx_tag_locate_kernel(PgxDevImage img, const pgx_mem *mems, const uint64_t *qstart, const uint64_t *qend,
                                      uint64_t n, const uint64_t *n_dev, const uint64_t *abort, uint64_t *run_nums, uint64_t *uval,
                                      PgxTagRec *small_recs, PgxTagRec *big_recs, PgxTagRec *large_recs, unsigned long long *sc,
                                      unsigned long long *n_overflow);
__global__ void pgx_tag_small_kernel(PgxDevImage img, const PgxTagRec *recs, uint64_t n, const uint64_t *n_dev, const uint64_t *abort, uint64_t *buf,
                                     uint64_t *uval, unsigned long long *n_overflow);
__global__ void pgx_tag_gather_kernel(PgxDevImage img, const PgxTagRec *recs, uint64_t n_list, const uint64_t *n_dev, const uint64_t *abort, uint64_t *buf,
                                      unsigned long long *n_overflow);
template <class L>
__global__ void pgx_tag_sort_unique_kernel(L src, uint64_t n_list, const uint64_t *n_dev, const uint64_t *abort, uint64_t *buf, uint64_t *ucount);
template <class L>
__global__ void pgx_tag_sort_large_kernel(L src, uint64_t n_list, const uint64_t *n_dev, const uint64_t *abort, uint64_t *buf, uint64_t *scratch,
                                          const uint64_t *scratch_off, uint64_t *ucount);
__global__ void pgx_tag_need_kernel(const PgxTagRec *recs, uint64_t n_list, uint64_t *need);
__global__ void pgx_tag_dedup_kernel(const PgxTagRec *recs, uint64_t n_list, const uint64_t *n_dev, const uint64_t *abort, unsigned long long *table,
                                     uint64_t table_mask, PgxTagRec *reps, unsigned long long *n_rep, uint64_t *pairs, unsigned long long *n_dup);
__global__ void pgx_tag_copy_dups_kernel(const uint64_t *pairs, uint64_t n_pairs, const uint64_t *n_dev, const uint64_t *abort, uint64_t n_tag_items,
                                         PgxTagRec *recs, uint64_t *uval, unsigned long long *n_overflow);
template <class L>
__global__ void pgx_tag_compact_kernel(L src, uint64_t n, const uint64_t *n_dev, const uint64_t *abort, const uint64_t *ucount, const uint64_t *buf,
                                       const uint64_t *pos_off, uint64_t *positions, uint64_t max_count);
__global__ void pgx_tag_compact_single_kernel(uint64_t n, const uint64_t *n_dev, const uint64_t *abort, const uint64_t *run_nums, const uint64_t *uval,
                                              const uint64_t *pos_off, uint64_t *positions);
template <class L>
__global__ void pgx_tag_compact_list_kernel(L src, uint64_t n_list, const uint64_t *n_dev, const uint64_t *abort, const uint64_t *ucount,
                                            const uint64_t *buf, const uint64_t *pos_off, uint64_t *positions, uint64_t max_count);
__global__ void pgx_spec_check_kernel(const uint64_t *v0, uint64_t c0, const uint64_t *v1, uint64_t c1, const uint64_t *v2, uint64_t c2,
                                      const uint64_t *v3, uint64_t c3, const uint64_t *v4, uint64_t c4, uint64_t *abort);
#define PGX_TAG_COMPACT_SMALL 256

struct PgxLocImage {
    const uint64_t *rstart, *rsamp;
    const uint32_t *rdir;
    const uint64_t *lpos, *lnext;
    const uint32_t *ldir;
    uint64_t n, n_runs, n_last, max_length, rdir_entries, ldir_entries;
    uint32_t rdir_shift, ldir_shift;
};
__global__ void pgx_locate_next_kernel(PgxLocImage loc, const uint64_t *prev, uint64_t n, uint64_t *out);
__global__ void pgx_lce_seqlen_kernel(const uint64_t *sa, uint64_t n_seq, uint64_t max_length, unsigned long long *seq_len);
__global__ void pgx_lce_scatter_kernel(const uint64_t *sa, uint64_t n, uint64_t max_length, const uint64_t *seq_start, uint64_t n_seq, uint64_t c1, uint64_t c2, uint64_t c3,
                                       uint64_t c4, uint64_t c5, uint32_t *sa32, uint8_t *text8, unsigned long long *bad);
__global__ void pgx_lce_pack_kernel(const uint8_t *text8, uint64_t n, uint64_t n_words, uint32_t *text32, uint32_t *flags);
__global__ void pgx_lce_lcp_kernel(const uint32_t *sa32, const uint32_t *text32, const uint32_t *flags, uint64_t n, uint8_t *lcp);
__global__ void pgx_lce_rc_check_kernel(const uint8_t *text8, const uint64_t *seq_start, uint64_t n_seq, uint64_t n, unsigned long long *bad);
__global__ void pgx_locate_plan_kernel(PgxLocImage loc, const uint64_t *qs, const uint64_t *qe, uint64_t n, uint64_t *run0,
                                       uint64_t *n_pieces);
__global__ void pgx_locate_walk_kernel(PgxLocImage loc, const uint64_t *qs, const uint64_t *qe, uint64_t n_queries,
                                       const uint64_t *run0, const uint64_t *piece_off, uint64_t n_pieces, const uint64_t *val_off,
                                       uint64_t val_base, int seq_ids, uint64_t *out);

#define PGX_ML_SPAN 4096
#define PGX_ML_WIN 1024
__global__ void pgx_ml_plan_kernel(const pgx_mem *mems, uint64_t n, uint64_t bwt_n, uint64_t max_occ, uint64_t *cnt, uint64_t *qs, uint64_t *qe,
                                   unsigned long long *n_not_located);
__global__ void pgx_ml_cut_kernel(const uint64_t *off, uint64_t n, uint64_t m0, uint64_t budget, uint64_t *out);
__global__ void pgx_ml_gather_kernel(const pgx_mem *mems, const uint64_t *off, uint64_t m0, uint64_t m1, uint64_t o_first, uint64_t nv,
                                     const uint32_t *sa32, uint64_t bwt_n, const uint64_t *seq_start, uint64_t n_seq, uint64_t max_length,
                                     int seq_ids, uint64_t *out);
__global__ void pgx_ml_classify_kernel(const uint64_t *cnt, const uint64_t *off, uint64_t np, uint64_t *seg, uint64_t *wave_list,
                                       uint64_t *wg_list, uint64_t *need, uint64_t *ucount, unsigned long long *ctr);
#define PGX_ML_SET_WORDS_MAX 64
#define PGX_ML_SET_BATCH 8
#define PGX_ML_SET_WIN 2048
__global__ void pgx_ml_sets_kernel(const pgx_mem *mems, const uint64_t *off, uint64_t m0, uint64_t m1, uint64_t o_first, uint64_t nv,
                                   const uint32_t *sa32, uint64_t bwt_n, const uint64_t *seq_start, uint64_t n_seq, uint32_t W,
                                   unsigned long long *sets);
__global__ void pgx_ml_sets_ids_kernel(const uint64_t *off, uint64_t m0, uint64_t m1, uint64_t o_first, uint64_t nv, const uint64_t *ids, uint32_t W,
                                       unsigned long long *sets);
__global__ void pgx_ml_set_count_kernel(const unsigned long long *sets, uint64_t np, uint32_t W, uint32_t Wp, uint64_t *ucount);
__global__ void pgx_ml_set_expand_kernel(const unsigned long long *sets, uint64_t np, uint32_t W, const uint64_t *uloc, uint64_t *out);
__global__ void pgx_ml_stride_kernel(uint64_t *out, uint64_t n, uint64_t stride);

struct PgxLitImage {
    const uint64_t *bstart, *cum, *runs;
    const uint32_t *roff;
    const uint32_t *code_of, *cslot_of;
    uint64_t C[8];
    uint64_t n, n_blocks;
};
__global__ void pgx_lit_count_kernel(PgxLitImage lit, const uint8_t *reads, const uint64_t *offsets, const pgx_range *in, const uint8_t *sym,
                                     uint64_t n, pgx_range *out);

__global__ void pgx_mt_file_of_kernel(const uint64_t *da, uint64_t n, uint64_t n_seq, const uint32_t *seq_to_file, uint32_t n_files,
                                      uint8_t *file_of, unsigned long long *n_bad);
__global__ void pgx_mt_expand_kernel(const uint64_t *start, const uint64_t *val, uint64_t n_runs, uint64_t *out);
__global__ void pgx_mt_gather_kernel(const uint8_t *file_of, uint32_t f, const uint64_t *rank, const uint64_t *expanded, uint64_t total,
                                     uint64_t n, uint64_t *tags);
__global__ void pgx_mt_flags_kernel(const uint64_t *tags, uint64_t n, uint64_t n_seq, uint8_t *flags);
__global__ void pgx_mt_compact_kernel(const uint64_t *tags, const uint8_t *flags, const uint64_t *idx, uint64_t n, uint64_t n_seq,
                                      uint64_t *out_val, uint64_t *out_start);

__global__ void pgx_bt_endmarker_kernel(const uint64_t *sa, uint64_t n_seq, uint64_t max_length, uint64_t *idx_len);
__global__ void pgx_bt_tag_kernel(uint64_t *sa, uint64_t n, uint64_t n_seq, uint64_t max_length, const uint64_t *seq_len, const uint64_t *dir_off,
                                  const uint64_t *dir, const uint64_t *node_start, const uint64_t *path_nodes, unsigned long long *bad);
__global__ void pgx_bt_heads_kernel(const uint64_t *tags, uint64_t n, uint64_t n_seq, uint8_t *head);
__global__ void pgx_bt_compact_kernel(const uint64_t *tags, const uint8_t *head, const uint64_t *idx, uint64_t n, uint64_t *run_val, uint64_t *run_start);
__global__ void pgx_bt_length_kernel(const uint64_t *run_start, uint64_t n_runs, uint64_t n, uint32_t reference_runs, uint64_t *run_len);
__global__ void pgx_bt_size_kernel(const uint64_t *run_val, const uint64_t *run_len, uint64_t n_runs, uint64_t *bytes);
__global__ void pgx_bt_write_kernel(const uint64_t *run_val, const uint64_t *run_len, const uint64_t *byte_off, uint64_t n_runs, uint8_t *body);

#define PGX_FASTX_ROUNDS 4
#define PGX_FASTX_TILE (256 * 16 * PGX_FASTX_ROUNDS)
#define PGX_FASTX_ERR_NO_AT 1u
#define PGX_FASTX_ERR_NO_PLUS 2u
#define PGX_FASTX_ERR_QUAL_LEN 3u
#define PGX_FASTX_ERR_TRUNCATED 4u
#define PGX_FASTX_ERR_BEFORE_FIRST 5u
#define PGX_FASTX_ERR_LONG_LINE 6u
__global__ void pgx_fastx_count_kernel(const uint8_t *text, uint64_t n, uint32_t *tile_count);
__global__ void pgx_fastx_lines_kernel(const uint8_t *text, uint64_t n, const uint64_t *tile_base, uint64_t *ls, uint64_t n_lines, uint32_t tail);
__global__ void pgx_fastx_role_kernel(const uint8_t *text, const uint64_t *ls, uint64_t n_lines, uint32_t format, uint32_t *contrib, uint8_t *rec,
                                      unsigned long long *err);
__global__ void pgx_fastx_records_kernel(uint64_t n_lines, uint32_t format, const uint32_t *contrib, const uint8_t *rec, const uint64_t *out_off,
                                         const uint64_t *rec_idx, uint64_t *offs, unsigned long long *err);
__global__ void pgx_fastx_longest_kernel(const uint64_t *offs, const uint64_t *n_reads, unsigned long long *longest);
__global__ void pgx_fastx_copy_kernel(const uint8_t *text, const uint64_t *ls, const uint64_t *out_off, uint64_t n_lines, uint64_t total, uint8_t *out);

#define PGX_SA_K 10
#define PGX_SA_TILE 2048
#define PGX_SA_SORT_TILE 4096
__global__ void pgx_sa_classify_kernel(const uint8_t *text, uint64_t n, uint64_t *codes, uint64_t n_words, uint32_t *tile_nl, unsigned long long *first_bad);
__global__ void pgx_sa_keys_kernel(const uint64_t *codes, uint64_t n_words, uint64_t n, const uint64_t *tile_off, uint64_t n_seq, uint32_t *hi, uint32_t *lo,
                                   uint32_t *idx, uint32_t *seq_start);
__global__ void pgx_sa_hist_kernel(const uint32_t *key, uint64_t n, uint32_t shift, uint32_t n_blocks, uint32_t *hist);
__global__ void pgx_sa_scatter_kernel(const uint32_t *hi, const uint32_t *lo, const uint32_t *idx, uint64_t n, int key_is_hi, uint32_t shift, uint32_t n_blocks,
                                      const uint64_t *offs, uint32_t *hi_out, uint32_t *lo_out, uint32_t *idx_out);
__global__ void pgx_sa_heads_kernel(const uint32_t *hi, const uint32_t *lo, uint64_t n, uint32_t *tile_cnt);
__global__ void pgx_sa_ranks_kernel(const uint32_t *hi, const uint32_t *lo, const uint32_t *idx, uint64_t n, const uint64_t *tile_off, uint32_t *hi_out,
                                    uint32_t *rank);
__global__ void pgx_sa_gather_kernel(const uint32_t *idx, const uint32_t *rank, uint64_t n, uint64_t h, uint32_t *lo);
__global__ void pgx_sa_bwt_kernel(const uint32_t *sa, const uint8_t *text, uint64_t n, uint8_t *bwt);
__global__ void pgx_sa_run_heads_kernel(const uint8_t *bwt, uint64_t n, uint32_t *tile_cnt);
__global__ void pgx_sa_runs_kernel(const uint8_t *bwt, const uint32_t *sa, uint64_t n, const uint64_t *tile_off, uint64_t n_runs, uint8_t *run_sym,
                                   uint32_t *run_start, uint32_t *run_head, uint32_t *run_tail);

#define PGX_SCAN_BLOCK_ITEMS 2048
#define PGX_SCAN1_TILE_ITEMS 4096
```

### pangenome-index_amd/csrc/pgx_pairs_kernels.hip

```cpp
#include <hip/hip_runtime.h>
#include <stdint.h>

#include <type_traits>

#include "pgx_device.h"
#include "pgx_rank_device.h"
#include "pgx_slots_device.h"

#ifndef PGX_PAIRS_PACKED_WAVES
#define PGX_PAIRS_PACKED_WAVES 5
#endif
#ifndef PGX_LCE_WAVES
#define PGX_LCE_WAVES PGX_FM_WAVES_PER_SIMD
#endif
#ifndef PGX_LCE_ENTRY_CAP
#define PGX_LCE_ENTRY_CAP 3u
#endif
#define PGX_PK_GROUP 12u

__device__ __forceinline__ uint32_t pgx_window_byte(uint64_t w0, uint64_t w1, uint64_t a) {
    return (uint32_t)(((a & 8ull) ? w1 : w0) >> (8u * (uint32_t)(a & 7ull))) & 0xFFu;
}
__device__ __forceinline__ uint32_t pgx_packed_seed_index(const uint32_t *s_rd, uint32_t rd_stride, uint32_t q, int32_t K) {
    const uint32_t w0 = s_rd[(q >> 4) * rd_stride + threadIdx.x], w1 = s_rd[((q >> 4) + 1u) * rd_stride + threadIdx.x];
    return (uint32_t)((((uint64_t)w1 << 32) | w0) >> (2u * (q & 15u))) & (uint32_t)((1ull << (2 * K)) - 1ull);
}
template <bool WIDE, bool PACKED, bool COOP, bool S64, bool LCE>
__global__ void __launch_bounds__(PGX_FM_THREADS, LCE ? PGX_LCE_WAVES : ((PACKED && !WIDE && !COOP) ? PGX_PAIRS_PACKED_WAVES : PGX_FM_WAVES_PER_SIMD))
pgx_find_mems_pairs_kernel(PgxDevImage img, const uint8_t *__restrict__ reads, const uint64_t *__restrict__ offsets,
                           uint64_t n_reads, uint64_t min_len, uint64_t min_occ, const uint64_t *__restrict__ slot_off,
                           pgx_mem *__restrict__ slots, uint32_t *__restrict__ mem_count, unsigned long long *__restrict__ n_ext_total,
                           unsigned long long *__restrict__ cursor, uint64_t first_read, uint64_t slot_base, uint32_t heavy_ext, uint32_t heavy_cap,
                           pgx_heavy_item *__restrict__ heavy_list, unsigned long long *__restrict__ heavy_count, const uint8_t *__restrict__ skip,
                           const uint32_t *__restrict__ packed, uint32_t pk_words, uint32_t *__restrict__ ovf_base, uint64_t ovf_cap) {
    typedef typename std::conditional<WIDE, uint64_t, uint32_t>::type pos_t;
    __shared__ uint32_t s_ext[512];
    __shared__ pos_t s_C[8];
    __shared__ pos_t s_t2[32];
    __shared__ uint4 s_fe[PACKED ? 16 : 512];
    extern __shared__ __align__(16) unsigned char pgx_dyn_lds[];
    static_assert(!COOP || PACKED, "the cooperative loads come with the packed reads");
    static_assert(!LCE || (PACKED && !WIDE && !COOP), "the text comparison reads the packed reads and 32-bit suffix array entries");
    constexpr uint32_t SYMS = PGX_PAIRS_SYMS, STRIDE = S64 ? PGX_PAIRS_STRIDE64 : PGX_PAIRS_SYMS;
    uint32_t *s_rd = reinterpret_cast<uint32_t *>(pgx_dyn_lds);
    const uint32_t rd_stride = blockDim.x;
    uint4 *s_stage = reinterpret_cast<uint4 *>(pgx_dyn_lds + (size_t)pk_words * PGX_FM_THREADS * 4) + (size_t)(threadIdx.x >> 6) * 512;
    uint64_t *s_pb = reinterpret_cast<uint64_t *>(pgx_dyn_lds + (size_t)pk_words * PGX_FM_THREADS * 4 + (COOP ? (size_t)(PGX_FM_THREADS / 64) * 8192 : 0));
    uint4 *s_sa4 = reinterpret_cast<uint4 *>(pgx_dyn_lds + (size_t)pk_words * PGX_FM_THREADS * 4);
    uint32_t *s_sae = reinterpret_cast<uint32_t *>(s_sa4 + PGX_FM_THREADS);
    uint32_t *s_lcp = s_sae + PGX_FM_THREADS;
    for (uint32_t i = threadIdx.x; i < 512; i += blockDim.x) s_ext[i] = img.consts->ext_tab[i];
    if (threadIdx.x < 8) s_C[threadIdx.x] = (pos_t)img.consts->C[threadIdx.x];
    if (threadIdx.x < 32) s_t2[threadIdx.x] = (pos_t)img.consts->pair_t2w[threadIdx.x];
    if (WIDE) for (uint32_t i = threadIdx.x; i < img.n_sbp * 24u; i += blockDim.x) s_pb[i] = img.pbase[i];
    if (PACKED) { if (threadIdx.x < 9) s_fe[threadIdx.x] = img.first_ext[threadIdx.x == 4 ? 0u : (threadIdx.x > 4 ? 256u : 0u) + ((0x47544341u >> (8u * ((threadIdx.x > 4 ? threadIdx.x - 5u : threadIdx.x) & 3u))) & 0xFFu)]; }
    else for (uint32_t i = threadIdx.x; i < 512; i += blockDim.x) s_fe[i] = img.first_ext[i];
    __syncthreads();

    const int lane = threadIdx.x & 63;
    const pos_t n = (pos_t)img.n;
    const pos_t mo = WIDE ? (pos_t)min_occ : (pos_t)(min_occ > 0xFFFFFFFFull ? 0xFFFFFFFFu : (uint32_t)min_occ);
    const bool mo_huge = !WIDE && min_occ > 0xFFFFFFFFull;
    auto ent_k = [](const uint4 &e) { return WIDE ? (pos_t)((uint64_t)e.x | ((uint64_t)(e.w & 0xFFu) << 32)) : (pos_t)e.x; };
    auto ent_q = [](const uint4 &e) { return WIDE ? (pos_t)((uint64_t)e.y | ((uint64_t)((e.w >> 8) & 0xFFu) << 32)) : (pos_t)e.y; };
    auto ent_s = [](const uint4 &e) { return WIDE ? (pos_t)((uint64_t)e.z | ((uint64_t)((e.w >> 16) & 0xFFu) << 32)) : (pos_t)e.z; };
    uint32_t rid = 0;
    uint64_t base = 0;
    int32_t len = 0, x = 0, j = 0;
    pos_t k = 0, kp = 0, s = 0, Jk = 0, Js = 0;
    uint32_t nm = 0, next = 0, next0 = 0;
    int ph = 0;
    uint64_t win = 0, win_hi = 0;
    uint32_t win_at = ~0u;
    uint32_t X0 = 0;
    pos_t X0e = 0, X0f = 0;
    uint32_t pend = 0, fresh = 0, restart = 0;
    uint64_t rnext = 0, rend = 0;
    bool exhausted = false;
    unsigned long long ln_blk = 0, ln_seed = 0, ln_two = 0;
    uint32_t did2 = 0;
    uint32_t lce_st = 0, lce_best = 0, lce_pos = 0;
    constexpr bool FUSE = LCE;
    typedef uint32_t pgx_u32x4 __attribute__((ext_vector_type(4)));
    pgx_u32x4 row = {0u, 0u, 0u, 0u}, hs = row, d0 = row, d1 = row, d2 = row;
    uint32_t lce_f0 = 0u, lce_f1 = 0u;
    auto ld4 = [](const uint4 *q) __attribute__((always_inline)) { return *reinterpret_cast<const pgx_u32x4 *>(q); };
#ifdef PGX_FM_STATS
    unsigned long long st_trips = 0, st_live = 0, st_wait = 0, st_fresh = 0;
    unsigned long long st_t_refill = 0, st_refills = 0, st_t_seed = 0, st_t_line = 0;
    const unsigned long long st_t0 = __builtin_readcyclecounter();
#endif

    auto begin = [&]() __attribute__((always_inline)) {
        if (x >= len || (uint64_t)(len - x) < min_len) { ph = 0; mem_count[rid] = nm; return; }
        if (heavy_ext && next - next0 >= heavy_ext && len <= (int32_t)PGX_FM_HEAVY_MAXLEN) {
            const unsigned long long at = atomicAdd(heavy_count, 1ull);
            if (at < (unsigned long long)heavy_cap) {
                pgx_heavy_item it;
                it.rid = (uint64_t)rid; it.x = (uint32_t)x; it.nm = nm;
                heavy_list[at] = it;
                ph = 0;
                return;
            }
        }
        k = 0; kp = 0; s = n;
        if (LCE) lce_st = 0u;
        if (min_len == 0) { Jk = 0; Js = n; j = x; ph = 2; }
        else { j = x + (int32_t)min_len - 1; ph = 1; fresh = 1u; }
    };
    auto lce_ask = [&](uint32_t k32, uint32_t t, bool cmp) __attribute__((always_inline)) {
        if (cmp) __builtin_amdgcn_global_load_lds((const void __attribute__((address_space(1))) *)(img.lce_sa + k32 + t), (void __attribute__((address_space(3))) *)(s_sae + (threadIdx.x >> 6) * 64u), 4, 0, 0);
        if (img.lce_lcp) {
            const uint32_t e0 = k32 + t + (cmp ? 1u : 0u), lb = e0 & ~3u;
#pragma unroll
            for (uint32_t q = 0; q < 5u; q++)
                if (q < 4u || (e0 & 3u) != 0u)
                    __builtin_amdgcn_global_load_lds((const void __attribute__((address_space(1))) *)(img.lce_lcp + lb + 4u * q),
                                                     (void __attribute__((address_space(3))) *)(s_lcp + ((threadIdx.x >> 6) * 5u + q) * 64u), 4, 0, 0);
        }
    };
    auto emit = [&]() __attribute__((always_inline)) {
        pgx_mem m;
        m.start = (uint64_t)x; m.end = (uint64_t)j; m.bwt_start = (uint64_t)Jk; m.size = (int64_t)(uint64_t)Js;
        const uint64_t slot = nm < PGX_FAST_SLOTS ? 0ull : pgx_slot_extent(slot_off, slot_base, ovf_base, ovf_cap, n_ext_total, (uint64_t)rid, nm, len, x, min_len);
        slots[pgx_slot_index((uint64_t)rid - first_read, n_reads - first_read, slot, nm)] = m;
        nm++;
        k = 0; kp = 0; s = n;
        if (LCE) lce_st = 0u;
        const bool more = j > x;
        ph = more ? 3 : ph;
        fresh = more ? 1u : fresh;
        x = more ? x : x + 1;
        restart = more ? restart : 1u;
    };

    for (;;) {
        __builtin_amdgcn_s_setprio(3);
        unsigned long long idle = __ballot(ph == 0);
        if (LCE && idle && (uint32_t)__popcll(idle) < img.refill_min && __popcll(idle) != 64) idle = 0ull;
#ifdef PGX_FM_STATS
        const unsigned long long st_r0 = __builtin_readcyclecounter();
        if (idle) st_refills++;
#endif
        while (idle) {
            if (rnext == rend) {
                if (exhausted) break;
                unsigned long long got = 0;
                if (lane == 0) got = first_read + atomicAdd(cursor, 32ull);
                got = ((unsigned long long)(uint32_t)__builtin_amdgcn_readfirstlane((int)(uint32_t)(got >> 32)) << 32) |
                      (uint32_t)__builtin_amdgcn_readfirstlane((int)(uint32_t)got);
                if (got >= n_reads) { exhausted = true; break; }
                rnext = got;
                rend = got + 32ull < n_reads ? got + 32ull : n_reads;
            }
            const uint64_t avail = rend - rnext;
            const uint32_t rank = (uint32_t)__popcll(idle & ((1ull << lane) - 1ull));
            if (ph == 0 && (uint64_t)rank < avail) {
                rid = (uint32_t)(rnext + rank);
                const uint8_t *skp = skip ? skip + rid : reinterpret_cast<const uint8_t *>(offsets);
                const uint32_t skv = (uint32_t)*skp;
                const uint64_t o0 = offsets[rid], o1 = offsets[rid + 1];
                const uint32_t sk = skip ? skv : 0u;
                base = o0;
                len = (int32_t)(o1 - o0);
                if (sk) ph = -1;
                else {
                    if (PACKED) {
                        const uint32_t *src = packed + (base >> 4);
                        const uint32_t nw = ((uint32_t)(base & 15ull) + (uint32_t)len + 15u) >> 4;
#pragma unroll 1
                        for (uint32_t w0 = 0; w0 < nw; w0 += PGX_PK_GROUP) {
                            uint32_t t[PGX_PK_GROUP];
#pragma unroll
                            for (uint32_t i = 0; i < PGX_PK_GROUP; i++) t[i] = src[w0 + i < nw ? w0 + i : nw - 1u];
#pragma unroll
                            for (uint32_t i = 0; i < PGX_PK_GROUP; i++) if (w0 + i < nw) s_rd[(w0 + i) * rd_stride + threadIdx.x] = t[i];
                        }
                    }
                    x = 0; nm = 0;
                    next0 = next;
                    begin();
                    if (ph == 0) ph = -1;
                }
            }
            const uint32_t want = (uint32_t)__popcll(idle);
            rnext += (uint64_t)want < avail ? (uint64_t)want : avail;
            idle = __ballot(ph == 0);
        }
#ifdef PGX_FM_STATS
        asm volatile("s_waitcnt vmcnt(0) lgkmcnt(0)" ::: "memory");
        st_t_refill += __builtin_readcyclecounter() - st_r0;
#endif
        if (ph == -1) ph = 0;
        if (!__any(ph > 0)) {
            if (exhausted && rnext == rend) break;
            continue;
        }
#ifdef PGX_FM_STATS
        st_trips++;
        st_live += (unsigned long long)__popcll(__ballot(ph > 0));
        st_fresh += (unsigned long long)__popcll(__ballot(ph > 0 && fresh != 0u));
#endif
        if (!FUSE) ln_blk += (unsigned long long)__popcll(__ballot(ph > 0 && fresh == 0u));
        ln_two += (unsigned long long)__popcll(__ballot(did2 != 0u));
        did2 = 0u;
        if (!FUSE) ln_seed += (unsigned long long)__popcll(__ballot(ph > 0 && fresh != 0u));
        if (COOP) {
            const pos_t kk_c = (ph == 2) ? kp : k;
            const uint32_t myblk = ph > 0 ? (S64 ? (uint32_t)(kk_c >> 6) : (uint32_t)(((uint64_t)(kk_c >> 5) * 0xAAAAAAABull) >> 33)) + pend : 0u;
#pragma unroll
            for (int i = 0; i < 8; i++) {
                const uint32_t q = 8u * (uint32_t)i + ((uint32_t)lane >> 3), piece = ((uint32_t)lane & 7u) ^ (q & 7u);
                const uint32_t blk = (uint32_t)__shfl((int)myblk, (int)q, 64);
                __builtin_amdgcn_global_load_lds((const void __attribute__((address_space(1))) *)(img.pairs + ((size_t)blk * 8 + piece)),
                                                 (void __attribute__((address_space(3))) *)(s_stage + 64 * i), 16, 0, 0);
            }
            __builtin_amdgcn_s_setprio(0);
            asm volatile("s_waitcnt vmcnt(0)" ::: "memory");
            __builtin_amdgcn_wave_barrier();
        }
        if (LCE) asm volatile("" : "=v"(row), "=v"(hs), "=v"(d0), "=v"(lce_f0), "=v"(lce_f1));
        const bool lce_lane = LCE && ph == 2 && (lce_st & 1u) != 0u;
        uint32_t lce_g0 = 0u;
        bool em_now = false;
        restart = 0u;
        if (LCE && __any(lce_lane)) asm volatile("s_waitcnt vmcnt(0)" ::: "memory");
#ifdef PGX_FM_STATS
        if (FUSE && __any(ph > 0 && fresh >= 2u)) {
            const unsigned long long st_s0 = __builtin_readcyclecounter();
            asm volatile("s_waitcnt vmcnt(0)" ::: "memory");
            st_t_seed += __builtin_readcyclecounter() - st_s0;
        }
#endif
        if (FUSE && __any(ph > 0 && fresh >= 0x100u)) asm volatile("s_waitcnt vmcnt(0)" ::: "memory");
        auto prestep = [&]() __attribute__((always_inline)) {
            const uint32_t kuse = fresh >> 8;
            const uint4 se_pre = s_sa4[threadIdx.x];
            fresh = 0u;
            const bool at_end = j >= len, q1 = ph == 1;
            const uint32_t qa = (uint32_t)(base & 15ull) + (uint32_t)(at_end ? len : j);
            const uint32_t qs1 = at_end ? qa - 1u : qa, qs2 = qa ? qa - 1u : 0u;
            const uint32_t wa = s_rd[(qs1 >> 4) * rd_stride + threadIdx.x], wb = s_rd[(qs2 >> 4) * rd_stride + threadIdx.x];
            const uint4 f1 = s_fe[at_end ? 4u : ((wa >> (2u * (qs1 & 15u))) & 3u)], f2 = s_fe[5u + ((wb >> (2u * (qs2 & 15u))) & 3u)];
            const bool small1 = f1.z == 0u || f1.z < mo || mo_huge;
            const uint32_t sdepth = se_pre.w >> 24, se_s = se_pre.z;
            const bool seed_alive = kuse != 0u && se_s != 0u && se_s >= mo && !mo_huge;
            const bool seed_dead = kuse != 0u && se_s == 0u && sdepth != PGX_SEED_UNUSABLE && min_occ <= 1;
            const bool rem2 = q1 ? (j - 1 >= x) : (j - 1 > x);
            const bool do2 = at_end && rem2 && !seed_alive && !seed_dead && !small1;
            uint32_t ns = do2 ? f2.z : f1.z, nk = do2 ? f2.x : f1.x, nq = do2 ? f2.y : f1.y;
            if (ns == 0u) { nk = 0u; nq = 0u; }
            j -= do2 ? 1 : 0;
            next += do2 ? 2u : 1u;
            did2 = do2 ? 1u : 0u;
            s = ns; k = nk; kp = nq;
            bool small = ns == 0u || ns < mo || mo_huge;
            if (seed_alive) {
                k = se_pre.x; kp = se_pre.y; s = se_s;
                small = false;
                j -= (int32_t)kuse - 1;
                next += kuse - 1u;
            } else if (seed_dead) {
                k = 0u; kp = 0u; s = 0u;
                small = true;
                j -= (int32_t)sdepth - 1;
                next += sdepth - 1u;
            }
            const bool adv = !small, at_x = j == x;
            const bool to2 = q1 && adv && at_x;
            Jk = to2 ? k : Jk;
            Js = to2 ? s : Js;
            const int32_t jn = adv ? (q1 ? (at_x ? x + (int32_t)min_len : j - 1) : j - 1) : j;
            const bool rs_end = !q1 && adv && jn <= x;
            restart = (small || rs_end) ? 1u : 0u;
            x = small ? j + 1 : (rs_end ? x + 1 : x);
            ph = to2 ? 2 : ph;
            j = jn;
            em_now = to2 && jn >= len;
        };
        auto prefetch = [&]() __attribute__((always_inline)) {
            const bool ask = ph > 0 && fresh == 1u;
            bool asked = false;
            if (ask) {
                const bool endw = j >= len;
                const int32_t K = endw ? (int32_t)img.seed_end_k : (int32_t)img.seed_k;
                const int32_t avail = (ph == 1) ? (j - x + 1) : (j - x);
                uint32_t kuse = 0u;
                if (K && avail >= K + (endw ? 1 : 0)) {
                    const uint32_t sidx = pgx_packed_seed_index(s_rd, rd_stride, (uint32_t)(base & 15ull) + (uint32_t)((endw ? len - 1 : j) - K + 1), K);
                    const uint4 *sp = (endw ? img.seed_end : img.seed) + sidx;
                    __builtin_amdgcn_global_load_lds((const void __attribute__((address_space(1))) *)sp, (void __attribute__((address_space(3))) *)(s_sa4 + (threadIdx.x >> 6) * 64u), 16, 0, 0);
                    kuse = (uint32_t)K + (endw ? 1u : 0u);
                    asked = true;
                }
                fresh = 2u | (kuse << 8);
            }
            ln_seed += (unsigned long long)__popcll(__ballot(asked));
        };
        if (FUSE && ph > 0 && fresh >= 2u) prestep();
        const bool sit_out = FUSE && (fresh != 0u || em_now || restart != 0u);
        if (FUSE) ln_blk += (unsigned long long)__popcll(__ballot(ph > 0 && !sit_out));
        const bool lce_cmp = lce_lane && (lce_st & 4u) == 0u;
        if (LCE && lce_cmp) {
            lce_pos = s_sae[threadIdx.x];
            lce_g0 = lce_pos + (uint32_t)(j - x);
            const uint32_t w0 = lce_g0 >> 4;
            const uint32_t *tp = img.lce_text + w0;
            asm volatile("global_load_dwordx4 %0, %3, off\n\tglobal_load_dwordx4 %1, %3, off offset:16\n\tglobal_load_dwordx4 %2, %3, off offset:32"
                         : "+v"(row), "+v"(hs), "+v"(d0) : "v"(tp) : "memory");
            const uint32_t l0 = w0 >> 5, l1 = (w0 + 11u) >> 5;
            const uint32_t *fp0 = img.lce_flags + (l0 >> 5), *fp1 = img.lce_flags + (l1 >> 5);
            asm volatile("global_load_dword %0, %2, off\n\tglobal_load_dword %1, %3, off" : "+v"(lce_f0), "+v"(lce_f1) : "v"(fp0), "v"(fp1) : "memory");
        }
        if (LCE) ln_blk += (unsigned long long)(__popcll(__ballot(lce_cmp && ((lce_g0 >> 4) >> 5) != (((lce_g0 >> 4) + 11u) >> 5))) +
                                                __popcll(__ballot(lce_cmp)) +
                                                (img.lce_lcp ? __popcll(__ballot(lce_lane && s > 1u)) : 0)) -
                             (unsigned long long)__popcll(__ballot(lce_lane && !lce_cmp));
        if (ph > 0 && !lce_lane && !sit_out) {
            const bool fr = !FUSE && fresh != 0u;
            bool seed_lane = false;
            uint32_t kuse = 0u;
            uint4 se = make_uint4(0u, 0u, 0u, 0u);
            if (!FUSE) {
                const uint4 *sp = img.seed;
                if (fr) {
                    const bool endw = j >= len;
                    const int32_t K = endw ? (int32_t)img.seed_end_k : (int32_t)img.seed_k;
                    const int32_t avail = (ph == 1) ? (j - x + 1) : (j - x);
                    if (K && avail >= K + (endw ? 1 : 0)) {
                        if (PACKED) {
                            const uint32_t sidx = pgx_packed_seed_index(s_rd, rd_stride, (uint32_t)(base & 15ull) + (uint32_t)((endw ? len - 1 : j) - K + 1), K);
                            seed_lane = true; sp = (endw ? img.seed_end : img.seed) + sidx; kuse = (uint32_t)K + (endw ? 1u : 0u);
                        } else {
                        const uint64_t a = base + (uint64_t)((endw ? len - 1 : j) - K + 1);
                        const uint32_t sh = (uint32_t)(a & 7ull) * 8u;
                        const uint64_t *wp = reinterpret_cast<const uint64_t *>(reads + (a & ~7ull));
                        const uint64_t w0 = wp[0], w1 = wp[1], w2 = wp[2];
                        const uint64_t lo = sh ? (w0 >> sh) | (w1 << (64u - sh)) : w0, hi = sh ? (w1 >> sh) | (w2 << (64u - sh)) : w1;
                        uint32_t sidx;
                        if (pgx_seed_index(lo, hi, (uint32_t)K, sidx)) { seed_lane = true; sp = (endw ? img.seed_end : img.seed) + sidx; kuse = (uint32_t)K + (endw ? 1u : 0u); }
                        }
                    }
                }
#ifdef PGX_FM_STATS
                const unsigned long long st_s0 = __builtin_readcyclecounter();
#endif
                se = *sp;
#ifdef PGX_FM_STATS
                asm volatile("s_waitcnt vmcnt(0)" ::: "memory");
                st_t_seed += __builtin_readcyclecounter() - st_s0;
#endif
            }
            if (!FUSE) fresh = 0u;
            const bool fwd = (ph == 2);
            const uint64_t at = base + (uint64_t)j;
            const bool at_end = j >= len;
            uint32_t byte, byte2;
            bool have2;
            if (PACKED) {
                const uint32_t qa = (uint32_t)(base & 15ull) + (uint32_t)(at_end ? len : j);
                const uint32_t q1 = at_end ? qa - 1u : qa, q2 = (fwd && !at_end) ? qa + 1u : (qa ? qa - 1u : 0u);
                const uint32_t wa = s_rd[(q1 >> 4) * rd_stride + threadIdx.x], wb = s_rd[(q2 >> 4) * rd_stride + threadIdx.x];
                byte = at_end ? 0u : ((0x47544341u >> (8u * ((wa >> (2u * (q1 & 15u))) & 3u))) & 0xFFu);
                byte2 = (0x47544341u >> (8u * ((wb >> (2u * (q2 & 15u))) & 3u))) & 0xFFu;
                have2 = true;
            } else {
            const uint64_t atw = at_end ? at - 1ull : at;
            if ((uint32_t)(atw >> 4) != win_at) {
                win_at = (uint32_t)(atw >> 4);
                const ulonglong2 w2 = *reinterpret_cast<const ulonglong2 *>(reads + (atw & ~15ull));
                win = w2.x; win_hi = w2.y;
            }
            byte = at_end ? 0u : pgx_window_byte(win, win_hi, at);
            const uint64_t at2 = (fwd && !at_end) ? at + 1ull : at - 1ull;
            have2 = (uint32_t)(at2 >> 4) == win_at;
            byte2 = pgx_window_byte(win, win_hi, at2);
            }
            const uint32_t e1 = s_ext[(fwd ? 256u : 0u) + byte], e2 = s_ext[(fwd ? 256u : 0u) + byte2];
            const uint32_t cv1 = PGX_EXT_CV(e1), cv2 = PGX_EXT_CV(e2);
            const bool reg1 = !PGX_EXT_KILL(e1) && ((0x2Eu >> cv1) & 1u), reg2 = !PGX_EXT_KILL(e2) && ((0x2Eu >> cv2) & 1u);
            const uint32_t t1 = reg1 ? cv1 - 1u - (cv1 >> 2) : 0u, t2 = reg2 ? cv2 - 1u - (cv2 >> 2) : 0u;
            const bool rem2 = ph == 1 ? (j - 1 >= x) : (fwd ? (j + 1 < len) : (j - 1 > x));
            const bool two = !fr && rem2 && have2 && reg1 && reg2;
            const pos_t kk = fwd ? kp : k, kq = fwd ? k : kp;
            const pos_t p0 = kk, p1 = kk + s;
            const uint32_t bfirst = S64 ? (uint32_t)(p0 >> 6) : (uint32_t)(((uint64_t)(p0 >> 5) * 0xAAAAAAABull) >> 33);
            const pos_t endrel_p = p1 - (pos_t)bfirst * STRIDE;
            const uint32_t endrel = endrel_p > (pos_t)0xFFFFu ? 0xFFFFu : (uint32_t)endrel_p;
            const uint32_t relA = pend ? SYMS - STRIDE : p0 - bfirst * STRIDE;
            const uint32_t relB = pend ? endrel - STRIDE : (endrel < SYMS ? endrel : SYMS);
            if (COOP) {
                const uint4 *mine = s_stage + (uint32_t)lane * 8u;
                const uint32_t sw = (uint32_t)lane & 7u;
                row = ld4(mine + (t1 ^ sw)); hs = ld4(mine + (4u ^ sw)); d0 = ld4(mine + (5u ^ sw)); d1 = ld4(mine + (6u ^ sw)); d2 = ld4(mine + (7u ^ sw));
            } else {
#ifdef PGX_FM_STATS
                const unsigned long long st_l0 = __builtin_readcyclecounter();
#endif
                const uint4 *bp = img.pairs + (size_t)(bfirst + pend) * 8;
                if (LCE) {
                    const uint4 *rp = bp + t1;
                    asm volatile("global_load_dwordx4 %0, %3, off\n\tglobal_load_dwordx4 %1, %4, off offset:64\n\tglobal_load_dwordx4 %2, %4, off offset:80"
                                 : "+v"(row), "+v"(hs), "+v"(d0) : "v"(rp), "v"(bp) : "memory");
                    d1 = ld4(bp + 6); d2 = ld4(bp + 7);
                } else {
                    row = ld4(bp + t1); hs = ld4(bp + 4); d0 = ld4(bp + 5); d1 = ld4(bp + 6); d2 = ld4(bp + 7);
                }
                __builtin_amdgcn_s_setprio(0);
#ifdef PGX_FM_STATS
                asm volatile("s_waitcnt vmcnt(0)" : "+v"(row), "+v"(hs), "+v"(d0), "+v"(d1), "+v"(d2) :: "memory");
                st_t_line += __builtin_readcyclecounter() - st_l0;
#endif
            }
            const uint32_t i0 = (t1 & 1u) ? 0u : 0xFFFFFFFFu, i1 = (t1 & 2u) ? 0u : 0xFFFFFFFFu, j0 = (t2 & 1u) ? 0u : 0xFFFFFFFFu, j1 = (t2 & 2u) ? 0u : 0xFFFFFFFFu;
            const uint32_t ua = t1 < 2u ? 0xFFFFFFFFu : 0u, va = t1 == 0u ? 0xFFFFFFFFu : 0u, wa = (t1 & 1u) ? 0u : 0xFFFFFFFFu;
            const uint32_t ub = t2 < 2u ? 0xFFFFFFFFu : 0u, vb = t2 == 0u ? 0xFFFFFFFFu : 0u, wb = (t2 & 1u) ? 0u : 0xFFFFFFFFu;
            if (LCE && !COOP) asm volatile("s_waitcnt vmcnt(0)" : "+v"(row), "+v"(hs), "+v"(d0) :: "memory");
            const bool flagged = (hs.x >> 31) != 0u;
            const uint32_t pts = (t1 == 0u ? hs.x : (t1 == 1u ? hs.y : (t1 == 2u ? hs.z : hs.w))) & 0x00FFFFFFu;
            const uint32_t PX[3] = {d0.x, d0.y, d0.z}, PY[3] = {d0.w, d1.x, d1.y}, PU[3] = {d1.z, d1.w, d2.x}, PV[3] = {d2.y, d2.z, d2.w};
            uint32_t e1p = 0, e2p = 0, e1r = 0, g1r = 0, e2r = 0, g2r = 0;
#pragma unroll
            for (int h = 0; h < 3; h++) {
                const int32_t ta = (int32_t)relA - 32 * h, tb = (int32_t)relB - 32 * h;
                const uint32_t mP = ta >= 32 ? 0xFFFFFFFFu : (ta > 0 ? ((1u << ta) - 1u) : 0u);
                const uint32_t mR = (tb >= 32 ? 0xFFFFFFFFu : (tb > 0 ? ((1u << tb) - 1u) : 0u)) & ~mP;
                const uint32_t x = PX[h], y = PY[h], u = PU[h], v = PV[h];
                const uint32_t m1 = (x ^ i0) & (y ^ i1);
                const uint32_t g1 = (y & ua) | (x & (y | va) & wa);
                const uint32_t q2 = m1 & (u ^ j0) & (v ^ j1);
                const uint32_t g2 = m1 & ((v & ub) | (u & (v | vb) & wb));
                e1p += __popc(m1 & mP); e2p += __popc(q2 & mP);
                e1r += __popc(m1 & mR); g1r += __popc(g1 & mR); e2r += __popc(q2 & mR); g2r += __popc(g2 & mR);
            }
            pos_t a01 = (pos_t)(row.x + row.y + row.z + row.w + pts + e1p);
            pos_t a02 = (pos_t)((t2 == 0u ? row.x : (t2 == 1u ? row.y : (t2 == 2u ? row.z : row.w))) + e2p);
            if (WIDE) {
                const uint64_t *pb = s_pb + (size_t)((bfirst + pend) >> img.pairs_sb_shift) * 24u;
                a01 += (pos_t)pb[16u + t1];
                a02 += (pos_t)pb[4u * t1 + t2];
            }
            const bool straddle = endrel > SYMS, far = endrel > STRIDE + SYMS;
            const uint32_t over = endrel - SYMS;
            const bool cont2 = !pend && straddle && over <= (hs.y >> 24), cont1 = !pend && straddle && !cont2 && over <= (hs.z >> 24);
            const bool cont = cont1 || cont2;
            if (cont) {
                const uint32_t l1 = (PX[2] >> 31) | ((PY[2] >> 31) << 1), l2 = (PU[2] >> 31) | ((PV[2] >> 31) << 1);
                e1r += l1 == t1 ? over : 0u;
                g1r += l1 > t1 ? over : 0u;
                e2r += (cont2 && l1 == t1 && l2 == t2) ? over : 0u;
                g2r += (cont2 && l1 == t1 && l2 > t2) ? over : 0u;
            }
            const bool bail = !fr && (flagged || (far && !cont));
            const bool wait = !fr && !pend && straddle && !bail && !cont;
#ifdef PGX_FM_STATS
            st_wait += wait ? 1ull : 0ull;
#endif
            if (wait) {
                X0 = e1r | (g1r << 8) | (e2r << 16) | (g2r << 24); X0e = a01; X0f = a02;
                pend = 1u;
            } else {
                const uint32_t Xp = pend ? X0 : 0u;
                const uint32_t c1 = (Xp & 0xFFu) + e1r, w1 = ((Xp >> 8) & 0xFFu) + g1r, c2 = ((Xp >> 16) & 0xFFu) + e2r, w2 = (Xp >> 24) + g2r;
                const pos_t r1 = pend ? X0e : a01, r2 = pend ? X0f : a02;
                pend = 0u;
                pos_t s1 = reg1 ? (pos_t)c1 : (pos_t)0;
                pos_t k1 = r1 + s_C[PGX_EXT_V(e1)], q1v = kq + (pos_t)w1;
                if (bail) {
                    const uint64_t q0 = (uint64_t)p0 > (uint64_t)n ? (uint64_t)n : (uint64_t)p0, q1 = (uint64_t)p1 > (uint64_t)n ? (uint64_t)n : (uint64_t)p1;
                    uint64_t A0 = 0, A1 = 0, B0 = 0, B1 = 0;
#pragma unroll 1
                    for (int it = 0; it < 2; it++) {
                        const uint64_t q = it ? q1 : q0;
                        uint64_t a, bq;
                        if (WIDE) pgx_dense2w_rank(img, q, PGX_EXT_CV(e1), PGX_EXT_M(e1), a, bq);
                        else if (img.dense == 1) {
                            const PgxDenseBlk db = pgx_dense_load<false>(img, nullptr, q);
                            pgx_dense_rank(db, q, PGX_EXT_CV(e1), PGX_EXT_M(e1), a, bq);
                        } else pgx_dense2_rank(img, (uint32_t)q, PGX_EXT_CV(e1), PGX_EXT_M(e1), a, bq);
                        A1 = a; B1 = bq;
                        if (!it) { A0 = a; B0 = bq; }
                    }
                    const uint64_t dB = B1 - B0;
                    {
                        const unsigned long long here = __ballot(true);
                        if (lane == (int)__ffsll((long long)here) - 1) {
                            atomicAdd(n_ext_total + PGX_CTR_REDO, (unsigned long long)__popcll(here));
                            atomicAdd(n_ext_total + PGX_CTR_PAIRS_LINES, 2ull * (unsigned long long)__popcll(here));
                        }
                    }
                    const bool none = PGX_EXT_KILL(e1) || A0 >= A1;
                    s1 = none ? (pos_t)0 : (pos_t)(A1 - A0);
                    k1 = (pos_t)A0 + s_C[PGX_EXT_V(e1)];
                    q1v = kq + (pos_t)dB;
                }
                if (fr) { const uint4 f = s_fe[PACKED ? (at_end ? 4u : ((byte >> 1) & 3u)) : byte]; k1 = ent_k(f); q1v = ent_q(f); s1 = ent_s(f); }
                const bool small1 = s1 == 0u || s1 < mo || mo_huge;
                const uint32_t sdepth = se.w >> 24;
                const pos_t se_s = ent_s(se);
                const bool seed_alive = seed_lane && se_s != 0u && se_s >= mo && !mo_huge;
                const bool seed_dead = seed_lane && se_s == 0u && sdepth != PGX_SEED_UNUSABLE && min_occ <= 1;
                const bool do2 = (fr ? (at_end && rem2 && have2 && !seed_alive && !seed_dead) : (two && !bail && !cont1)) && !small1;
                pos_t s2 = (pos_t)c2, k2 = r2 + s_C[PGX_EXT_V(e2)] + s_t2[8u * t1 + cv2], q2v = q1v + (pos_t)w2;
                if (fr) { const uint4 f = s_fe[PACKED ? 5u + ((byte2 >> 1) & 3u) : 256u + byte2]; k2 = ent_k(f); q2v = ent_q(f); s2 = ent_s(f); }
                pos_t ns = do2 ? s2 : s1, nk = do2 ? k2 : k1, nq = do2 ? q2v : q1v;
                if (ns == 0u) { nk = 0u; nq = 0u; }
                if (do2) {
                    Jk = fwd ? q1v : Jk;
                    Js = fwd ? s1 : Js;
                    j = fwd ? j + 1 : j - 1;
                }
                next += do2 ? 2u : 1u;
                did2 = do2 ? 1u : 0u;
                s = ns;
                k = fwd ? nq : nk;
                kp = fwd ? nk : nq;
                bool small = ns == 0u || ns < mo || mo_huge;
                if (seed_alive) {
                    k = ent_k(se); kp = ent_q(se); s = se_s;
                    small = false;
                    j -= (int32_t)kuse - 1;
                    next += kuse - 1u;
                } else if (seed_dead) {
                    k = 0u; kp = 0u; s = 0u;
                    small = true;
                    j -= (int32_t)sdepth - 1;
                    next += sdepth - 1u;
                }
                const bool adv = !small, q1 = ph == 1, q2 = ph == 2, at_x = j == x;
                const bool to2 = q1 && adv && at_x;
                const bool keep = adv && (to2 || q2);
                Jk = keep ? k : Jk;
                Js = keep ? s : Js;
                const int32_t jn = adv ? (q1 ? (at_x ? x + (int32_t)min_len : j - 1) : (q2 ? j + 1 : j - 1)) : j;
                const bool em = (q2 && (small || jn >= len)) || (to2 && jn >= len);
                const bool rs_small = small && !q2, rs_end = !q1 && !q2 && adv && jn <= x;
                restart = (rs_small || rs_end) ? 1u : 0u;
                x = rs_small ? j + 1 : (rs_end ? x + 1 : x);
                ph = to2 ? 2 : ph;
                j = jn;
                em_now = em;
                if (LCE && img.lce_sa && ph == 2 && !em && !restart && !(lce_st & 2u) && s >= 1u && (uint32_t)s <= img.lce_max && mo <= 1u && j < len &&
                    (uint32_t)(len - j) >= 2u * (img.lce_lcp && (uint32_t)s > PGX_LCE_ENTRY_CAP ? PGX_LCE_ENTRY_CAP : (uint32_t)s) && (uint32_t)(len - j) <= 144u &&
                    ((uint32_t)s <= 16u || (img.lce_lcp && (uint32_t)(len - x) <= PGX_LCP_CAP - 1u))) {
                    lce_st = 1u;
                    lce_best = 0u;
                    lce_ask((uint32_t)k, 0u, true);
                }
            }
        }
        if (LCE) asm volatile("s_waitcnt vmcnt(0)" : "+v"(row), "+v"(hs), "+v"(d0), "+v"(lce_f0), "+v"(lce_f1) :: "memory");
        if (LCE && lce_lane) {
            const uint32_t rem = (uint32_t)(len - j), i = (lce_st >> 8) & 0xFFu;
            uint32_t a = (lce_st >> 16) & 0xFFu, cnt = lce_st >> 24, t0 = i;
            bool fin = false, banned = false;
            if (lce_cmp) {
                const uint32_t T[12] = {row.x, row.y, row.z, row.w, hs.x, hs.y, hs.z, hs.w, d0.x, d0.y, d0.z, d0.w};
                const uint32_t fl0 = lce_g0 >> 9, fl1 = ((lce_g0 >> 4) + 11u) >> 5;
                banned = (((lce_f0 >> (fl0 & 31u)) | (lce_f1 >> (fl1 & 31u))) & 1u) != 0u;
                const uint32_t q0 = (uint32_t)(base & 15ull) + (uint32_t)j;
                const uint32_t tsh = 2u * (lce_g0 & 15u), rsh = 2u * (q0 & 15u), rw0 = q0 >> 4;
                uint32_t R[10];
#pragma unroll
                for (uint32_t u = 0; u < 10; u++) { const uint32_t wi = rw0 + u; R[u] = s_rd[(wi < pk_words ? wi : pk_words - 1u) * rd_stride + threadIdx.x]; }
                uint32_t l = 144u;
#pragma unroll
                for (int u = 8; u >= 0; u--) {
                    const uint32_t df = __builtin_amdgcn_alignbit(R[u + 1], R[u], rsh) ^ __builtin_amdgcn_alignbit(T[u + 1], T[u], tsh);
                    l = df ? 16u * (uint32_t)u + ((uint32_t)__builtin_ctz(df) >> 1) : l;
                }
                l = l < rem ? l : rem;
                const bool better = i == 0u || l > lce_best;
                fin = !better && l < lce_best;
                cnt = better ? 1u : (l == lce_best ? cnt + 1u : cnt);
                a = better ? i : a;
                lce_best = better ? l : lce_best;
                t0 = i + 1u;
            }
            if (banned) lce_st = 2u;
            else {
                uint32_t tt = t0;
                bool cmp_next = true;
                if (!fin && tt < (uint32_t)s && img.lce_lcp && (uint32_t)(len - x) <= PGX_LCP_CAP - 1u) {
                    const uint32_t m = (uint32_t)(j - x), bsh = ((uint32_t)k + t0) & 3u;
                    uint32_t L5[5];
#pragma unroll
                    for (uint32_t t = 0; t < 5u; t++) L5[t] = s_lcp[((threadIdx.x >> 6) * 5u + t) * 64u + (uint32_t)lane];
                    const uint32_t W[4] = {__builtin_amdgcn_alignbyte(L5[1], L5[0], bsh), __builtin_amdgcn_alignbyte(L5[2], L5[1], bsh), __builtin_amdgcn_alignbyte(L5[3], L5[2], bsh),
                                           __builtin_amdgcn_alignbyte(L5[4], L5[3], bsh)};
                    bool stop = false;
                    cmp_next = false;
#pragma unroll
                    for (uint32_t u = 0; u < 16u; u++) {
                        if ((u & 3u) == 0u && u > 0u && !__any(!stop && t0 + u < (uint32_t)s)) break;
                        const uint32_t c = (W[u >> 2] >> (8u * (u & 3u))) & 0xFFu, rel = c - m;
                        const bool act = !stop && t0 + u < (uint32_t)s;
                        const bool hard = c == PGX_LCP_UNKNOWN || c < m || (rel == lce_best && lce_best < rem);
                        const bool drop = !hard && rel < lce_best;
                        cmp_next = cmp_next || (act && hard);
                        fin = fin || (act && drop);
                        stop = stop || (act && (hard || drop));
                        if (act && !hard && !drop) { cnt++; tt = t0 + u + 1u; }
                    }
                }
                if (!fin && tt < (uint32_t)s) {
                    lce_st = 1u | (cmp_next ? 0u : 4u) | (tt << 8) | (a << 16) | (cnt << 24);
                    lce_ask((uint32_t)k, tt, cmp_next);
                } else {
                    Jk = k + (pos_t)a; Js = (pos_t)cnt;
                    next += lce_best + (lce_best < rem ? 1u : 0u);
                    j += (int32_t)lce_best;
                    lce_st = 0u;
                    em_now = true;
                }
            }
        }
        if (em_now) emit();
        if (restart) begin();
        if (FUSE) prefetch();
    }
    unsigned long long tot = next;
#pragma unroll
    for (int off = 32; off > 0; off >>= 1) tot += __shfl_down(tot, off, 64);
    if (lane == 0 && tot) atomicAdd(n_ext_total + PGX_CTR_EXT, tot);
    ln_two += (unsigned long long)__popcll(__ballot(did2 != 0u));
    if (lane == 0 && ln_blk) { atomicAdd(n_ext_total + PGX_CTR_PAIRS_LINES, ln_blk); atomicAdd(n_ext_total + PGX_CTR_PAIRS_SEEDS, ln_seed); atomicAdd(n_ext_total + PGX_CTR_PAIRS_TWO, ln_two); }
#ifdef PGX_FM_STATS
#pragma unroll
    for (int off = 32; off > 0; off >>= 1) st_wait += __shfl_down(st_wait, off, 64);
    if (lane == 0) { atomicAdd(n_ext_total + PGX_CTR_ST_PAIR_T_REFILL, st_t_refill); atomicAdd(n_ext_total + PGX_CTR_ST_PAIR_T_TOTAL, __builtin_readcyclecounter() - st_t0); atomicAdd(n_ext_total + PGX_CTR_ST_PAIR_REFILLS, st_refills);
                     atomicAdd(n_ext_total + PGX_CTR_ST_PAIR_T_SEED, st_t_seed); atomicAdd(n_ext_total + PGX_CTR_ST_PAIR_T_LINE, st_t_line); }
    if (lane == 0) { atomicAdd(n_ext_total + PGX_CTR_ST_PAIR_TRIPS, st_trips); atomicAdd(n_ext_total + PGX_CTR_ST_PAIR_LIVE, st_live); atomicAdd(n_ext_total + PGX_CTR_ST_PAIR_WAIT, st_wait); atomicAdd(n_ext_total + PGX_CTR_ST_PAIR_FRESH, st_fresh); }
#endif
}
#define PGX_PAIRS_INSTANTIATE(...)                                                                                                                \
    template __global__ void pgx_find_mems_pairs_kernel<__VA_ARGS__>(PgxDevImage, const uint8_t *, const uint64_t *, uint64_t, uint64_t, uint64_t, const uint64_t *, \
                                                                     pgx_mem *, uint32_t *, unsigned long long *, unsigned long long *, uint64_t, uint64_t, uint32_t, \
                                                                     uint32_t, pgx_heavy_item *, unsigned long long *, const uint8_t *, const uint32_t *, uint32_t,  \
                                                                     uint32_t *, uint64_t);
PGX_PAIRS_INSTANTIATE(false, false, false, false, false)
PGX_PAIRS_INSTANTIATE(true, false, false, false, false)
PGX_PAIRS_INSTANTIATE(false, true, false, false, false)
PGX_PAIRS_INSTANTIATE(true, true, false, false, false)
PGX_PAIRS_INSTANTIATE(false, true, true, false, false)
PGX_PAIRS_INSTANTIATE(true, true, true, false, false)
PGX_PAIRS_INSTANTIATE(false, false, false, true, false)
PGX_PAIRS_INSTANTIATE(true, false, false, true, false)
PGX_PAIRS_INSTANTIATE(false, true, false, true, false)
PGX_PAIRS_INSTANTIATE(true, true, false, true, false)
PGX_PAIRS_INSTANTIATE(false, true, true, true, false)
PGX_PAIRS_INSTANTIATE(true, true, true, true, false)
PGX_PAIRS_INSTANTIATE(false, true, false, false, true)
PGX_PAIRS_INSTANTIATE(false, true, false, true, true)
```

Measured before the change: 1.140 billion.

## Pass a compact pairs-kernel argument struct and reload cold fields from kernarg

Replaces the large PgxDevImage-by-value parameter list of the pairs kernel with a flat PgxPairsArgs struct that carries only the fields the kernel uses. Rarely used fields (heavy list, overflow slot state, counters, dense rank tables) are read through a volatile kernarg-segment pointer at their point of use instead of being held in scalar registers. Read cursors and line counters are narrowed to 32 bits, and the LCE variant gets constant-folded min_occ and heavy_ext checks. The aim is to cut SGPR/VGPR pressure in the hot loop, at the cost of extra scalar loads on cold paths and a more fragile interface.

```diff
diff --git a/pangenome-index_amd/csrc/pgx_batch.hip b/pangenome-index_amd/csrc/pgx_batch.hip
--- a/pangenome-index_amd/csrc/pgx_batch.hip
+++ b/pangenome-index_amd/csrc/pgx_batch.hip
@@ -643,8 +643,21 @@
         b->timing.pairs_reads = lce ? 4u : coop ? 3u : 2u;
         grid = find_mems_grid(r, kp, plds, true, cn);
     }
-    void *pargs[] = {&a.img, &a.reads, &a.off, &a.n, &a.min_len, &a.min_occ, &a.slot_off, &a.slots, &a.cnt, &a.next, &a.cur, &a.first, &a.base,
-                     &a.hext, &a.hcap, &a.hlist, &a.hcount, &skip, &a_packed, &a_pkw, &a.ovf, &a.ovf_cap};
+    PgxPairsArgs p = {};
+    p.pairs = img.pairs; p.seed = img.seed; p.seed_end = img.seed_end;
+    p.lce_sa = img.lce_sa; p.lce_text = img.lce_text; p.lce_flags = img.lce_flags; p.lce_lcp = img.lce_lcp;
+    p.reads = a.reads; p.slots = a.slots; p.mem_count = a.cnt;
+    p.n = img.n; p.min_len = a.min_len; p.min_occ = a.min_occ;
+    p.first_read = a.first; p.n_reads = a.n;
+    p.seed_k = img.seed_k; p.seed_end_k = img.seed_end_k; p.lce_max = img.lce_max; p.refill_min = img.refill_min;
+    p.pk_words = a_pkw; p.heavy_ext = a.hext; p.pairs_sb_shift = img.pairs_sb_shift; p.dense = img.dense;
+    p.consts = img.consts; p.first_ext = img.first_ext; p.pbase = img.pbase; p.n_sbp = img.n_sbp;
+    p.offsets = a.off; p.skip = skip; p.packed = a_packed;
+    p.cursor = a.cur; p.ctr = a.next;
+    p.slot_off = a.slot_off; p.slot_base = a.base; p.ovf_base = a.ovf; p.ovf_cap = a.ovf_cap;
+    p.heavy_list = a.hlist; p.heavy_count = a.hcount; p.heavy_cap = a.hcap; p.d2_sb_shift = img.d2_sb_shift;
+    p.blocks = img.blocks; p.exc = img.exc; p.sbase2 = img.sbase2;
+    void *pargs[] = {&p};
     HIPCHECK(hipLaunchKernel(kp, dim3(grid), dim3(PGX_FM_THREADS), pargs, plds, r.s));
     b->timing.kernels |= kp_bits;
 }
diff --git a/pangenome-index_amd/csrc/pgx_device.h b/pangenome-index_amd/csrc/pgx_device.h
--- a/pangenome-index_amd/csrc/pgx_device.h
+++ b/pangenome-index_amd/csrc/pgx_device.h
@@ -117,13 +117,39 @@
                                uint64_t min_len, uint64_t min_occ, PgxHeavyResult *out);
 __global__ void pgx_arena_demand_kernel(unsigned long long *ctr);
 
+struct PgxPairsArgs {
+    const uint4 *pairs;
+    const uint4 *seed, *seed_end;
+    const uint32_t *lce_sa, *lce_text, *lce_flags;
+    const uint8_t *lce_lcp;
+    const uint8_t *reads;
+    pgx_mem *slots;
+    uint32_t *mem_count;
+    uint64_t n, min_len, min_occ;
+    uint64_t first_read, n_reads;
+    uint32_t seed_k, seed_end_k, lce_max, refill_min;
+    uint32_t pk_words, heavy_ext, pairs_sb_shift, dense;
+    const PgxConsts *consts;
+    const uint4 *first_ext;
+    const uint64_t *pbase;
+    uint32_t n_sbp, pad0;
+    const uint64_t *offsets;
+    const uint8_t *skip;
+    const uint32_t *packed;
+    unsigned long long *cursor, *ctr;
+    const uint64_t *slot_off;
+    uint64_t slot_base;
+    uint32_t *ovf_base;
+    uint64_t ovf_cap;
+    pgx_heavy_item *heavy_list;
+    unsigned long long *heavy_count;
+    uint32_t heavy_cap, d2_sb_shift;
+    const uint4 *blocks;
+    const uint32_t *exc;
+    const uint64_t *sbase2;
+};
 template <bool WIDE, bool PACKED, bool COOP, bool S64, bool LCE>
-__global__ void pgx_find_mems_pairs_kernel(PgxDevImage img, const uint8_t *reads, const uint64_t *offsets, uint64_t n_reads,
-                                           uint64_t min_len, uint64_t min_occ, const uint64_t *slot_off, pgx_mem *slots,
-                                           uint32_t *mem_count, unsigned long long *n_ext_total, unsigned long long *cursor, uint64_t first_read,
-                                           uint64_t slot_base, uint32_t heavy_ext, uint32_t heavy_cap, pgx_heavy_item *heavy_list, unsigned long long *heavy_count,
-                                           const uint8_t *skip, const uint32_t *packed, uint32_t pk_words,
-                                           uint32_t *ovf_base, uint64_t ovf_cap);
+__global__ void pgx_find_mems_pairs_kernel(PgxPairsArgs a);
 
 __global__ void pgx_bad_chunks_kernel(const uint8_t *reads, uint64_t n_bytes, uint64_t *chunks, unsigned long long *count, uint64_t cap, uint32_t *packed);
 __global__ void pgx_unpack_reads_kernel(const uint32_t *packed, uint64_t n_chunks, uint8_t *reads);
diff --git a/pangenome-index_amd/csrc/pgx_pairs_kernels.hip b/pangenome-index_amd/csrc/pgx_pairs_kernels.hip
--- a/pangenome-index_amd/csrc/pgx_pairs_kernels.hip
+++ b/pangenome-index_amd/csrc/pgx_pairs_kernels.hip
@@ -27,40 +27,53 @@
 }
 template <bool WIDE, bool PACKED, bool COOP, bool S64, bool LCE>
 __global__ void __launch_bounds__(PGX_FM_THREADS, LCE ? PGX_LCE_WAVES : ((PACKED && !WIDE && !COOP) ? PGX_PAIRS_PACKED_WAVES : PGX_FM_WAVES_PER_SIMD))
-pgx_find_mems_pairs_kernel(PgxDevImage img, const uint8_t *__restrict__ reads, const uint64_t *__restrict__ offsets,
-                           uint64_t n_reads, uint64_t min_len, uint64_t min_occ, const uint64_t *__restrict__ slot_off,
-                           pgx_mem *__restrict__ slots, uint32_t *__restrict__ mem_count, unsigned long long *__restrict__ n_ext_total,
-                           unsigned long long *__restrict__ cursor, uint64_t first_read, uint64_t slot_base, uint32_t heavy_ext, uint32_t heavy_cap,
-                           pgx_heavy_item *__restrict__ heavy_list, unsigned long long *__restrict__ heavy_count, const uint8_t *__restrict__ skip,
-                           const uint32_t *__restrict__ packed, uint32_t pk_words, uint32_t *__restrict__ ovf_base, uint64_t ovf_cap) {
+pgx_find_mems_pairs_kernel(PgxPairsArgs pa) {
     typedef typename std::conditional<WIDE, uint64_t, uint32_t>::type pos_t;
+    const volatile PgxPairsArgs __attribute__((address_space(4))) *const ka = (const volatile PgxPairsArgs __attribute__((address_space(4))) *)__builtin_amdgcn_kernarg_segment_ptr();
+#define PGX_PAIRS_COLD(f) (ka->f)
+    if (LCE) asm volatile("" : "+s"(pa.pairs), "+s"(pa.lce_text), "+s"(pa.lce_flags));
+    const uint8_t *__restrict__ const reads = pa.reads;
+    pgx_mem *__restrict__ const slots_fr = reinterpret_cast<pgx_mem *>(reinterpret_cast<uintptr_t>(pa.slots) - (uintptr_t)pa.first_read * sizeof(pgx_mem));
+    uint32_t *__restrict__ const mem_count = pa.mem_count;
+    const uint32_t pk_words = pa.pk_words;
+    const uint32_t heavy_ext = LCE ? 0u : (pa.heavy_ext ? pa.heavy_ext : 0xFFFFFFFFu);
+    const uint32_t chunk_reads = (uint32_t)(pa.n_reads - pa.first_read);
+    const uint32_t min_len = pa.min_len > 0x80000000ull ? 0x80000000u : (uint32_t)pa.min_len;
     __shared__ uint32_t s_ext[512];
     __shared__ pos_t s_C[8];
     __shared__ pos_t s_t2[32];
     __shared__ uint4 s_fe[PACKED ? 16 : 512];
+    typedef uint32_t pgx_u32x4 __attribute__((ext_vector_type(4)));
+    __shared__ pgx_u32x4 s_seedt[2];
     extern __shared__ __align__(16) unsigned char pgx_dyn_lds[];
     static_assert(!COOP || PACKED, "the cooperative loads come with the packed reads");
     static_assert(!LCE || (PACKED && !WIDE && !COOP), "the text comparison reads the packed reads and 32-bit suffix array entries");
     constexpr uint32_t SYMS = PGX_PAIRS_SYMS, STRIDE = S64 ? PGX_PAIRS_STRIDE64 : PGX_PAIRS_SYMS;
     uint32_t *s_rd = reinterpret_cast<uint32_t *>(pgx_dyn_lds);
-    const uint32_t rd_stride = blockDim.x;
+    constexpr uint32_t rd_stride = PGX_FM_THREADS;
     uint4 *s_stage = reinterpret_cast<uint4 *>(pgx_dyn_lds + (size_t)pk_words * PGX_FM_THREADS * 4) + (size_t)(threadIdx.x >> 6) * 512;
     uint64_t *s_pb = reinterpret_cast<uint64_t *>(pgx_dyn_lds + (size_t)pk_words * PGX_FM_THREADS * 4 + (COOP ? (size_t)(PGX_FM_THREADS / 64) * 8192 : 0));
     uint4 *s_sa4 = reinterpret_cast<uint4 *>(pgx_dyn_lds + (size_t)pk_words * PGX_FM_THREADS * 4);
     uint32_t *s_sae = reinterpret_cast<uint32_t *>(s_sa4 + PGX_FM_THREADS);
     uint32_t *s_lcp = s_sae + PGX_FM_THREADS;
-    for (uint32_t i = threadIdx.x; i < 512; i += blockDim.x) s_ext[i] = img.consts->ext_tab[i];
-    if (threadIdx.x < 8) s_C[threadIdx.x] = (pos_t)img.consts->C[threadIdx.x];
-    if (threadIdx.x < 32) s_t2[threadIdx.x] = (pos_t)img.consts->pair_t2w[threadIdx.x];
-    if (WIDE) for (uint32_t i = threadIdx.x; i < img.n_sbp * 24u; i += blockDim.x) s_pb[i] = img.pbase[i];
-    if (PACKED) { if (threadIdx.x < 9) s_fe[threadIdx.x] = img.first_ext[threadIdx.x == 4 ? 0u : (threadIdx.x > 4 ? 256u : 0u) + ((0x47544341u >> (8u * ((threadIdx.x > 4 ? threadIdx.x - 5u : threadIdx.x) & 3u))) & 0xFFu)]; }
-    else for (uint32_t i = threadIdx.x; i < 512; i += blockDim.x) s_fe[i] = img.first_ext[i];
+    for (uint32_t i = threadIdx.x; i < 512; i += PGX_FM_THREADS) s_ext[i] = pa.consts->ext_tab[i];
+    if (threadIdx.x < 8) s_C[threadIdx.x] = (pos_t)pa.consts->C[threadIdx.x];
+    if (threadIdx.x < 32) s_t2[threadIdx.x] = (pos_t)pa.consts->pair_t2w[threadIdx.x];
+    if (WIDE) for (uint32_t i = threadIdx.x; i < pa.n_sbp * 24u; i += PGX_FM_THREADS) s_pb[i] = pa.pbase[i];
+    if (PACKED) { if (threadIdx.x < 9) s_fe[threadIdx.x] = pa.first_ext[threadIdx.x == 4 ? 0u : (threadIdx.x > 4 ? 256u : 0u) + ((0x47544341u >> (8u * ((threadIdx.x > 4 ? threadIdx.x - 5u : threadIdx.x) & 3u))) & 0xFFu)]; }
+    else for (uint32_t i = threadIdx.x; i < 512; i += PGX_FM_THREADS) s_fe[i] = pa.first_ext[i];
+    if (LCE && threadIdx.x < 2) {
+        const uint64_t tp = (uint64_t)(threadIdx.x ? pa.seed_end : pa.seed);
+        const uint32_t tk = threadIdx.x ? pa.seed_end_k : pa.seed_k;
+        const pgx_u32x4 te = {(uint32_t)tp, (uint32_t)(tp >> 32), tk, tk + threadIdx.x};
+        s_seedt[threadIdx.x] = te;
+    }
     __syncthreads();
 
     const int lane = threadIdx.x & 63;
-    const pos_t n = (pos_t)img.n;
-    const pos_t mo = WIDE ? (pos_t)min_occ : (pos_t)(min_occ > 0xFFFFFFFFull ? 0xFFFFFFFFu : (uint32_t)min_occ);
-    const bool mo_huge = !WIDE && min_occ > 0xFFFFFFFFull;
+    const pos_t n = (pos_t)pa.n;
+    const pos_t mo = LCE ? (pos_t)1 : WIDE ? (pos_t)pa.min_occ : (pos_t)(pa.min_occ > 0xFFFFFFFFull ? 0xFFFFFFFFu : (uint32_t)pa.min_occ);
+    const bool mo_huge = !LCE && !WIDE && pa.min_occ > 0xFFFFFFFFull;
     auto ent_k = [](const uint4 &e) { return WIDE ? (pos_t)((uint64_t)e.x | ((uint64_t)(e.w & 0xFFu) << 32)) : (pos_t)e.x; };
     auto ent_q = [](const uint4 &e) { return WIDE ? (pos_t)((uint64_t)e.y | ((uint64_t)((e.w >> 8) & 0xFFu) << 32)) : (pos_t)e.y; };
     auto ent_s = [](const uint4 &e) { return WIDE ? (pos_t)((uint64_t)e.z | ((uint64_t)((e.w >> 16) & 0xFFu) << 32)) : (pos_t)e.z; };
@@ -68,20 +81,27 @@
     uint64_t base = 0;
     int32_t len = 0, x = 0, j = 0;
     pos_t k = 0, kp = 0, s = 0, Jk = 0, Js = 0;
-    uint32_t nm = 0, next = 0, next0 = 0;
+    uint32_t nm = 0, next = 0;
+    uint32_t hmark = 0;
     int ph = 0;
     uint64_t win = 0, win_hi = 0;
     uint32_t win_at = ~0u;
     uint32_t X0 = 0;
     pos_t X0e = 0, X0f = 0;
     uint32_t pend = 0, fresh = 0, restart = 0;
-    uint64_t rnext = 0, rend = 0;
-    bool exhausted = false;
-    unsigned long long ln_blk = 0, ln_seed = 0, ln_two = 0;
+    uint32_t rnext = 0, rend = 0;
+    constexpr uint32_t EXHAUSTED = 0xFFFFFFFFu;
+    uint32_t ln_blk = 0, ln_seed = 0, ln_two = 0;
+    auto ln_flush = [&]() __attribute__((always_inline)) {
+        if (ln_blk) {
+            unsigned long long *const ctr = PGX_PAIRS_COLD(ctr);
+            if ((threadIdx.x & 63u) == 0u) { atomicAdd(ctr + PGX_CTR_PAIRS_LINES, (unsigned long long)(ln_blk - 1u)); atomicAdd(ctr + PGX_CTR_PAIRS_SEEDS, (unsigned long long)ln_seed); atomicAdd(ctr + PGX_CTR_PAIRS_TWO, (unsigned long long)ln_two); }
+            ln_blk = 1u; ln_seed = 0u; ln_two = 0u;
+        }
+    };
     uint32_t did2 = 0;
     uint32_t lce_st = 0, lce_best = 0, lce_pos = 0;
     constexpr bool FUSE = LCE;
-    typedef uint32_t pgx_u32x4 __attribute__((ext_vector_type(4)));
     pgx_u32x4 row = {0u, 0u, 0u, 0u}, hs = row, d0 = row, d1 = row, d2 = row;
     uint32_t lce_f0 = 0u, lce_f1 = 0u;
     auto ld4 = [](const uint4 *q) __attribute__((always_inline)) { return *reinterpret_cast<const pgx_u32x4 *>(q); };
@@ -92,38 +112,45 @@
 #endif
 
     auto begin = [&]() __attribute__((always_inline)) {
-        if (x >= len || (uint64_t)(len - x) < min_len) { ph = 0; mem_count[rid] = nm; return; }
-        if (heavy_ext && next - next0 >= heavy_ext && len <= (int32_t)PGX_FM_HEAVY_MAXLEN) {
-            const unsigned long long at = atomicAdd(heavy_count, 1ull);
-            if (at < (unsigned long long)heavy_cap) {
+        if (x >= len || (uint32_t)(len - x) < min_len) { ph = 0; mem_count[rid] = nm; return; }
+        if ((LCE ? (int32_t)(next - hmark) >= 0 : next - hmark >= heavy_ext) && len <= (int32_t)PGX_FM_HEAVY_MAXLEN) {
+            const unsigned long long at = atomicAdd(PGX_PAIRS_COLD(heavy_count), 1ull);
+            if (at < (unsigned long long)PGX_PAIRS_COLD(heavy_cap)) {
                 pgx_heavy_item it;
                 it.rid = (uint64_t)rid; it.x = (uint32_t)x; it.nm = nm;
-                heavy_list[at] = it;
+                PGX_PAIRS_COLD(heavy_list)[at] = it;
                 ph = 0;
                 return;
             }
         }
         k = 0; kp = 0; s = n;
         if (LCE) lce_st = 0u;
-        if (min_len == 0) { Jk = 0; Js = n; j = x; ph = 2; }
-        else { j = x + (int32_t)min_len - 1; ph = 1; fresh = 1u; }
+        uint32_t ml = min_len;
+        asm volatile("" : "+s"(ml));
+        if (ml == 0) { Jk = 0; Js = n; j = x; ph = 2; }
+        else { j = x + (int32_t)ml - 1; ph = 1; fresh = 1u; }
     };
+    auto has_lcp = [&]() __attribute__((always_inline)) { const uint8_t *q = pa.lce_lcp; asm volatile("" : "+s"(q)); return q != nullptr; };
     auto lce_ask = [&](uint32_t k32, uint32_t t, bool cmp) __attribute__((always_inline)) {
-        if (cmp) __builtin_amdgcn_global_load_lds((const void __attribute__((address_space(1))) *)(img.lce_sa + k32 + t), (void __attribute__((address_space(3))) *)(s_sae + (threadIdx.x >> 6) * 64u), 4, 0, 0);
-        if (img.lce_lcp) {
+        if (cmp) __builtin_amdgcn_global_load_lds((const void __attribute__((address_space(1))) *)(pa.lce_sa + k32 + t), (void __attribute__((address_space(3))) *)(s_sae + (threadIdx.x >> 6) * 64u), 4, 0, 0);
+        if (has_lcp()) {
             const uint32_t e0 = k32 + t + (cmp ? 1u : 0u), lb = e0 & ~3u;
 #pragma unroll
             for (uint32_t q = 0; q < 5u; q++)
                 if (q < 4u || (e0 & 3u) != 0u)
-                    __builtin_amdgcn_global_load_lds((const void __attribute__((address_space(1))) *)(img.lce_lcp + lb + 4u * q),
+                    __builtin_amdgcn_global_load_lds((const void __attribute__((address_space(1))) *)(pa.lce_lcp + lb + 4u * q),
                                                      (void __attribute__((address_space(3))) *)(s_lcp + ((threadIdx.x >> 6) * 5u + q) * 64u), 4, 0, 0);
         }
     };
     auto emit = [&]() __attribute__((always_inline)) {
         pgx_mem m;
         m.start = (uint64_t)x; m.end = (uint64_t)j; m.bwt_start = (uint64_t)Jk; m.size = (int64_t)(uint64_t)Js;
-        const uint64_t slot = nm < PGX_FAST_SLOTS ? 0ull : pgx_slot_extent(slot_off, slot_base, ovf_base, ovf_cap, n_ext_total, (uint64_t)rid, nm, len, x, min_len);
-        slots[pgx_slot_index((uint64_t)rid - first_read, n_reads - first_read, slot, nm)] = m;
+        if (nm < PGX_FAST_SLOTS) slots_fr[pgx_slot_index((uint64_t)rid, (uint64_t)chunk_reads, 0ull, nm)] = m;
+        else {
+            const uint64_t fr = PGX_PAIRS_COLD(first_read), cr = PGX_PAIRS_COLD(n_reads) - fr;
+            const uint64_t slot = pgx_slot_extent(PGX_PAIRS_COLD(slot_off), PGX_PAIRS_COLD(slot_base), PGX_PAIRS_COLD(ovf_base), PGX_PAIRS_COLD(ovf_cap), PGX_PAIRS_COLD(ctr), (uint64_t)rid, nm, len, x, PGX_PAIRS_COLD(min_len));
+            PGX_PAIRS_COLD(slots)[pgx_slot_index((uint64_t)rid - fr, cr, slot, nm)] = m;
+        }
         nm++;
         k = 0; kp = 0; s = n;
         if (LCE) lce_st = 0u;
@@ -137,26 +164,29 @@
     for (;;) {
         __builtin_amdgcn_s_setprio(3);
         unsigned long long idle = __ballot(ph == 0);
-        if (LCE && idle && (uint32_t)__popcll(idle) < img.refill_min && __popcll(idle) != 64) idle = 0ull;
+        if (LCE && idle && (uint32_t)__popcll(idle) < pa.refill_min && __popcll(idle) != 64) idle = 0ull;
 #ifdef PGX_FM_STATS
         const unsigned long long st_r0 = __builtin_readcyclecounter();
         if (idle) st_refills++;
 #endif
         while (idle) {
             if (rnext == rend) {
-                if (exhausted) break;
+                if (rnext == EXHAUSTED) break;
                 unsigned long long got = 0;
-                if (lane == 0) got = first_read + atomicAdd(cursor, 32ull);
+                const unsigned long long n_reads = PGX_PAIRS_COLD(n_reads);
+                if (lane == 0) got = PGX_PAIRS_COLD(first_read) + atomicAdd(PGX_PAIRS_COLD(cursor), 32ull);
                 got = ((unsigned long long)(uint32_t)__builtin_amdgcn_readfirstlane((int)(uint32_t)(got >> 32)) << 32) |
                       (uint32_t)__builtin_amdgcn_readfirstlane((int)(uint32_t)got);
-                if (got >= n_reads) { exhausted = true; break; }
-                rnext = got;
-                rend = got + 32ull < n_reads ? got + 32ull : n_reads;
-            }
-            const uint64_t avail = rend - rnext;
+                if (got >= n_reads) { rnext = rend = EXHAUSTED; break; }
+                rnext = (uint32_t)got;
+                rend = (uint32_t)(got + 32ull < n_reads ? got + 32ull : n_reads);
+            }
+            const uint32_t avail = rend - rnext;
             const uint32_t rank = (uint32_t)__popcll(idle & ((1ull << lane) - 1ull));
-            if (ph == 0 && (uint64_t)rank < avail) {
-                rid = (uint32_t)(rnext + rank);
+            if (ph == 0 && rank < avail) {
+                rid = rnext + rank;
+                const uint8_t *const skip = PGX_PAIRS_COLD(skip);
+                const uint64_t *const offsets = PGX_PAIRS_COLD(offsets);
                 const uint8_t *skp = skip ? skip + rid : reinterpret_cast<const uint8_t *>(offsets);
                 const uint32_t skv = (uint32_t)*skp;
                 const uint64_t o0 = offsets[rid], o1 = offsets[rid + 1];
@@ -166,7 +196,7 @@
                 if (sk) ph = -1;
                 else {
                     if (PACKED) {
-                        const uint32_t *src = packed + (base >> 4);
+                        const uint32_t *src = PGX_PAIRS_COLD(packed) + (base >> 4);
                         const uint32_t nw = ((uint32_t)(base & 15ull) + (uint32_t)len + 15u) >> 4;
 #pragma unroll 1
                         for (uint32_t w0 = 0; w0 < nw; w0 += PGX_PK_GROUP) {
@@ -178,13 +208,14 @@
                         }
                     }
                     x = 0; nm = 0;
-                    next0 = next;
+                    hmark = next;
+                    if (LCE) { const uint32_t hx = PGX_PAIRS_COLD(heavy_ext); hmark += hx != 0u && hx < 0x7FFFFFFFu ? hx : 0x7FFFFFFFu; }
                     begin();
                     if (ph == 0) ph = -1;
                 }
             }
             const uint32_t want = (uint32_t)__popcll(idle);
-            rnext += (uint64_t)want < avail ? (uint64_t)want : avail;
+            rnext += want < avail ? want : avail;
             idle = __ballot(ph == 0);
         }
 #ifdef PGX_FM_STATS
@@ -193,7 +224,7 @@
 #endif
         if (ph == -1) ph = 0;
         if (!__any(ph > 0)) {
-            if (exhausted && rnext == rend) break;
+            if (rnext == EXHAUSTED) break;
             continue;
         }
 #ifdef PGX_FM_STATS
@@ -201,10 +232,11 @@
         st_live += (unsigned long long)__popcll(__ballot(ph > 0));
         st_fresh += (unsigned long long)__popcll(__ballot(ph > 0 && fresh != 0u));
 #endif
-        if (!FUSE) ln_blk += (unsigned long long)__popcll(__ballot(ph > 0 && fresh == 0u));
-        ln_two += (unsigned long long)__popcll(__ballot(did2 != 0u));
+        if (!FUSE) ln_blk += (uint32_t)__popcll(__ballot(ph > 0 && fresh == 0u));
+        if ((ln_blk | ln_seed | ln_two) >> 31) ln_flush();
+        ln_two += (uint32_t)__popcll(__ballot(did2 != 0u));
         did2 = 0u;
-        if (!FUSE) ln_seed += (unsigned long long)__popcll(__ballot(ph > 0 && fresh != 0u));
+        if (!FUSE) ln_seed += (uint32_t)__popcll(__ballot(ph > 0 && fresh != 0u));
         if (COOP) {
             const pos_t kk_c = (ph == 2) ? kp : k;
             const uint32_t myblk = ph > 0 ? (S64 ? (uint32_t)(kk_c >> 6) : (uint32_t)(((uint64_t)(kk_c >> 5) * 0xAAAAAAABull) >> 33)) + pend : 0u;
@@ -212,7 +244,7 @@
             for (int i = 0; i < 8; i++) {
                 const uint32_t q = 8u * (uint32_t)i + ((uint32_t)lane >> 3), piece = ((uint32_t)lane & 7u) ^ (q & 7u);
                 const uint32_t blk = (uint32_t)__shfl((int)myblk, (int)q, 64);
-                __builtin_amdgcn_global_load_lds((const void __attribute__((address_space(1))) *)(img.pairs + ((size_t)blk * 8 + piece)),
+                __builtin_amdgcn_global_load_lds((const void __attribute__((address_space(1))) *)(pa.pairs + ((size_t)blk * 8 + piece)),
                                                  (void __attribute__((address_space(3))) *)(s_stage + 64 * i), 16, 0, 0);
             }
             __builtin_amdgcn_s_setprio(0);
@@ -245,7 +277,7 @@
             const bool small1 = f1.z == 0u || f1.z < mo || mo_huge;
             const uint32_t sdepth = se_pre.w >> 24, se_s = se_pre.z;
             const bool seed_alive = kuse != 0u && se_s != 0u && se_s >= mo && !mo_huge;
-            const bool seed_dead = kuse != 0u && se_s == 0u && sdepth != PGX_SEED_UNUSABLE && min_occ <= 1;
+            const bool seed_dead = kuse != 0u && se_s == 0u && sdepth != PGX_SEED_UNUSABLE && mo <= 1u;
             const bool rem2 = q1 ? (j - 1 >= x) : (j - 1 > x);
             const bool do2 = at_end && rem2 && !seed_alive && !seed_dead && !small1;
             uint32_t ns = do2 ? f2.z : f1.z, nk = do2 ? f2.x : f1.x, nq = do2 ? f2.y : f1.y;
@@ -283,54 +315,55 @@
             bool asked = false;
             if (ask) {
                 const bool endw = j >= len;
-                const int32_t K = endw ? (int32_t)img.seed_end_k : (int32_t)img.seed_k;
+                const pgx_u32x4 tab = *(const volatile pgx_u32x4 *)&s_seedt[endw ? 1u : 0u];
+                const int32_t K = (int32_t)tab.z;
                 const int32_t avail = (ph == 1) ? (j - x + 1) : (j - x);
                 uint32_t kuse = 0u;
-                if (K && avail >= K + (endw ? 1 : 0)) {
+                if (K && avail >= (int32_t)tab.w) {
                     const uint32_t sidx = pgx_packed_seed_index(s_rd, rd_stride, (uint32_t)(base & 15ull) + (uint32_t)((endw ? len - 1 : j) - K + 1), K);
-                    const uint4 *sp = (endw ? img.seed_end : img.seed) + sidx;
+                    const uint4 *sp = reinterpret_cast<const uint4 *>(((uint64_t)tab.y << 32) | tab.x) + sidx;
                     __builtin_amdgcn_global_load_lds((const void __attribute__((address_space(1))) *)sp, (void __attribute__((address_space(3))) *)(s_sa4 + (threadIdx.x >> 6) * 64u), 16, 0, 0);
-                    kuse = (uint32_t)K + (endw ? 1u : 0u);
+                    kuse = tab.w;
                     asked = true;
                 }
                 fresh = 2u | (kuse << 8);
             }
-            ln_seed += (unsigned long long)__popcll(__ballot(asked));
+            ln_seed += (uint32_t)__popcll(__ballot(asked));
         };
         if (FUSE && ph > 0 && fresh >= 2u) prestep();
         const bool sit_out = FUSE && (fresh != 0u || em_now || restart != 0u);
-        if (FUSE) ln_blk += (unsigned long long)__popcll(__ballot(ph > 0 && !sit_out));
+        if (FUSE) ln_blk += (uint32_t)__popcll(__ballot(ph > 0 && !sit_out));
         const bool lce_cmp = lce_lane && (lce_st & 4u) == 0u;
         if (LCE && lce_cmp) {
             lce_pos = s_sae[threadIdx.x];
             lce_g0 = lce_pos + (uint32_t)(j - x);
             const uint32_t w0 = lce_g0 >> 4;
-            const uint32_t *tp = img.lce_text + w0;
+            const uint32_t *tp = pa.lce_text + w0;
             asm volatile("global_load_dwordx4 %0, %3, off\n\tglobal_load_dwordx4 %1, %3, off offset:16\n\tglobal_load_dwordx4 %2, %3, off offset:32"
                          : "+v"(row), "+v"(hs), "+v"(d0) : "v"(tp) : "memory");
             const uint32_t l0 = w0 >> 5, l1 = (w0 + 11u) >> 5;
-            const uint32_t *fp0 = img.lce_flags + (l0 >> 5), *fp1 = img.lce_flags + (l1 >> 5);
+            const uint32_t *fp0 = pa.lce_flags + (l0 >> 5), *fp1 = pa.lce_flags + (l1 >> 5);
             asm volatile("global_load_dword %0, %2, off\n\tglobal_load_dword %1, %3, off" : "+v"(lce_f0), "+v"(lce_f1) : "v"(fp0), "v"(fp1) : "memory");
         }
-        if (LCE) ln_blk += (unsigned long long)(__popcll(__ballot(lce_cmp && ((lce_g0 >> 4) >> 5) != (((lce_g0 >> 4) + 11u) >> 5))) +
+        if (LCE) ln_blk += (uint32_t)(__popcll(__ballot(lce_cmp && ((lce_g0 >> 4) >> 5) != (((lce_g0 >> 4) + 11u) >> 5))) +
                                                 __popcll(__ballot(lce_cmp)) +
-                                                (img.lce_lcp ? __popcll(__ballot(lce_lane && s > 1u)) : 0)) -
-                             (unsigned long long)__popcll(__ballot(lce_lane && !lce_cmp));
+                                                (has_lcp() ? __popcll(__ballot(lce_lane && s > 1u)) : 0)) -
+                             (uint32_t)__popcll(__ballot(lce_lane && !lce_cmp));
         if (ph > 0 && !lce_lane && !sit_out) {
             const bool fr = !FUSE && fresh != 0u;
             bool seed_lane = false;
             uint32_t kuse = 0u;
             uint4 se = make_uint4(0u, 0u, 0u, 0u);
             if (!FUSE) {
-                const uint4 *sp = img.seed;
+                const uint4 *sp = pa.seed;
                 if (fr) {
                     const bool endw = j >= len;
-                    const int32_t K = endw ? (int32_t)img.seed_end_k : (int32_t)img.seed_k;
+                    const int32_t K = endw ? (int32_t)pa.seed_end_k : (int32_t)pa.seed_k;
                     const int32_t avail = (ph == 1) ? (j - x + 1) : (j - x);
                     if (K && avail >= K + (endw ? 1 : 0)) {
                         if (PACKED) {
                             const uint32_t sidx = pgx_packed_seed_index(s_rd, rd_stride, (uint32_t)(base & 15ull) + (uint32_t)((endw ? len - 1 : j) - K + 1), K);
-                            seed_lane = true; sp = (endw ? img.seed_end : img.seed) + sidx; kuse = (uint32_t)K + (endw ? 1u : 0u);
+                            seed_lane = true; sp = (endw ? pa.seed_end : pa.seed) + sidx; kuse = (uint32_t)K + (endw ? 1u : 0u);
                         } else {
                         const uint64_t a = base + (uint64_t)((endw ? len - 1 : j) - K + 1);
                         const uint32_t sh = (uint32_t)(a & 7ull) * 8u;
@@ -338,7 +371,7 @@
                         const uint64_t w0 = wp[0], w1 = wp[1], w2 = wp[2];
                         const uint64_t lo = sh ? (w0 >> sh) | (w1 << (64u - sh)) : w0, hi = sh ? (w1 >> sh) | (w2 << (64u - sh)) : w1;
                         uint32_t sidx;
-                        if (pgx_seed_index(lo, hi, (uint32_t)K, sidx)) { seed_lane = true; sp = (endw ? img.seed_end : img.seed) + sidx; kuse = (uint32_t)K + (endw ? 1u : 0u); }
+                        if (pgx_seed_index(lo, hi, (uint32_t)K, sidx)) { seed_lane = true; sp = (endw ? pa.seed_end : pa.seed) + sidx; kuse = (uint32_t)K + (endw ? 1u : 0u); }
                         }
                     }
                 }
@@ -397,7 +430,7 @@
 #ifdef PGX_FM_STATS
                 const unsigned long long st_l0 = __builtin_readcyclecounter();
 #endif
-                const uint4 *bp = img.pairs + (size_t)(bfirst + pend) * 8;
+                const uint4 *bp = pa.pairs + (size_t)(bfirst + pend) * 8;
                 if (LCE) {
                     const uint4 *rp = bp + t1;
                     asm volatile("global_load_dwordx4 %0, %3, off\n\tglobal_load_dwordx4 %1, %4, off offset:64\n\tglobal_load_dwordx4 %2, %4, off offset:80"
@@ -436,7 +469,7 @@
             pos_t a01 = (pos_t)(row.x + row.y + row.z + row.w + pts + e1p);
             pos_t a02 = (pos_t)((t2 == 0u ? row.x : (t2 == 1u ? row.y : (t2 == 2u ? row.z : row.w))) + e2p);
             if (WIDE) {
-                const uint64_t *pb = s_pb + (size_t)((bfirst + pend) >> img.pairs_sb_shift) * 24u;
+                const uint64_t *pb = s_pb + (size_t)((bfirst + pend) >> pa.pairs_sb_shift) * 24u;
                 a01 += (pos_t)pb[16u + t1];
                 a02 += (pos_t)pb[4u * t1 + t2];
             }
@@ -469,12 +502,14 @@
                 if (bail) {
                     const uint64_t q0 = (uint64_t)p0 > (uint64_t)n ? (uint64_t)n : (uint64_t)p0, q1 = (uint64_t)p1 > (uint64_t)n ? (uint64_t)n : (uint64_t)p1;
                     uint64_t A0 = 0, A1 = 0, B0 = 0, B1 = 0;
+                    PgxDevImage img = {};
+                    img.blocks = PGX_PAIRS_COLD(blocks); img.exc = PGX_PAIRS_COLD(exc); img.sbase2 = PGX_PAIRS_COLD(sbase2); img.d2_sb_shift = PGX_PAIRS_COLD(d2_sb_shift);
 #pragma unroll 1
                     for (int it = 0; it < 2; it++) {
                         const uint64_t q = it ? q1 : q0;
                         uint64_t a, bq;
                         if (WIDE) pgx_dense2w_rank(img, q, PGX_EXT_CV(e1), PGX_EXT_M(e1), a, bq);
-                        else if (img.dense == 1) {
+                        else if (pa.dense == 1) {
                             const PgxDenseBlk db = pgx_dense_load<false>(img, nullptr, q);
                             pgx_dense_rank(db, q, PGX_EXT_CV(e1), PGX_EXT_M(e1), a, bq);
                         } else pgx_dense2_rank(img, (uint32_t)q, PGX_EXT_CV(e1), PGX_EXT_M(e1), a, bq);
@@ -485,8 +520,8 @@
                     {
                         const unsigned long long here = __ballot(true);
                         if (lane == (int)__ffsll((long long)here) - 1) {
-                            atomicAdd(n_ext_total + PGX_CTR_REDO, (unsigned long long)__popcll(here));
-                            atomicAdd(n_ext_total + PGX_CTR_PAIRS_LINES, 2ull * (unsigned long long)__popcll(here));
+                            atomicAdd(PGX_PAIRS_COLD(ctr) + PGX_CTR_REDO, (unsigned long long)__popcll(here));
+                            atomicAdd(PGX_PAIRS_COLD(ctr) + PGX_CTR_PAIRS_LINES, 2ull * (unsigned long long)__popcll(here));
                         }
                     }
                     const bool none = PGX_EXT_KILL(e1) || A0 >= A1;
@@ -499,7 +534,7 @@
                 const uint32_t sdepth = se.w >> 24;
                 const pos_t se_s = ent_s(se);
                 const bool seed_alive = seed_lane && se_s != 0u && se_s >= mo && !mo_huge;
-                const bool seed_dead = seed_lane && se_s == 0u && sdepth != PGX_SEED_UNUSABLE && min_occ <= 1;
+                const bool seed_dead = seed_lane && se_s == 0u && sdepth != PGX_SEED_UNUSABLE && mo <= 1u;
                 const bool do2 = (fr ? (at_end && rem2 && have2 && !seed_alive && !seed_dead) : (two && !bail && !cont1)) && !small1;
                 pos_t s2 = (pos_t)c2, k2 = r2 + s_C[PGX_EXT_V(e2)] + s_t2[8u * t1 + cv2], q2v = q1v + (pos_t)w2;
                 if (fr) { const uint4 f = s_fe[PACKED ? 5u + ((byte2 >> 1) & 3u) : 256u + byte2]; k2 = ent_k(f); q2v = ent_q(f); s2 = ent_s(f); }
@@ -540,9 +575,9 @@
                 ph = to2 ? 2 : ph;
                 j = jn;
                 em_now = em;
-                if (LCE && img.lce_sa && ph == 2 && !em && !restart && !(lce_st & 2u) && s >= 1u && (uint32_t)s <= img.lce_max && mo <= 1u && j < len &&
-                    (uint32_t)(len - j) >= 2u * (img.lce_lcp && (uint32_t)s > PGX_LCE_ENTRY_CAP ? PGX_LCE_ENTRY_CAP : (uint32_t)s) && (uint32_t)(len - j) <= 144u &&
-                    ((uint32_t)s <= 16u || (img.lce_lcp && (uint32_t)(len - x) <= PGX_LCP_CAP - 1u))) {
+                if (LCE && ph == 2 && !em && !restart && !(lce_st & 2u) && s >= 1u && (uint32_t)s <= pa.lce_max && mo <= 1u && j < len &&
+                    (uint32_t)(len - j) >= 2u * (has_lcp() && (uint32_t)s > PGX_LCE_ENTRY_CAP ? PGX_LCE_ENTRY_CAP : (uint32_t)s) && (uint32_t)(len - j) <= 144u &&
+                    ((uint32_t)s <= 16u || (has_lcp() && (uint32_t)(len - x) <= PGX_LCP_CAP - 1u))) {
                     lce_st = 1u;
                     lce_best = 0u;
                     lce_ask((uint32_t)k, 0u, true);
@@ -581,7 +616,7 @@
             else {
                 uint32_t tt = t0;
                 bool cmp_next = true;
-                if (!fin && tt < (uint32_t)s && img.lce_lcp && (uint32_t)(len - x) <= PGX_LCP_CAP - 1u) {
+                if (!fin && tt < (uint32_t)s && has_lcp() && (uint32_t)(len - x) <= PGX_LCP_CAP - 1u) {
                     const uint32_t m = (uint32_t)(j - x), bsh = ((uint32_t)k + t0) & 3u;
                     uint32_t L5[5];
 #pragma unroll
@@ -619,12 +654,13 @@
         if (restart) begin();
         if (FUSE) prefetch();
     }
+    unsigned long long *const n_ext_total = PGX_PAIRS_COLD(ctr);
     unsigned long long tot = next;
 #pragma unroll
     for (int off = 32; off > 0; off >>= 1) tot += __shfl_down(tot, off, 64);
     if (lane == 0 && tot) atomicAdd(n_ext_total + PGX_CTR_EXT, tot);
-    ln_two += (unsigned long long)__popcll(__ballot(did2 != 0u));
-    if (lane == 0 && ln_blk) { atomicAdd(n_ext_total + PGX_CTR_PAIRS_LINES, ln_blk); atomicAdd(n_ext_total + PGX_CTR_PAIRS_SEEDS, ln_seed); atomicAdd(n_ext_total + PGX_CTR_PAIRS_TWO, ln_two); }
+    ln_two += (uint32_t)__popcll(__ballot(did2 != 0u));
+    if (lane == 0 && ln_blk) { atomicAdd(n_ext_total + PGX_CTR_PAIRS_LINES, (unsigned long long)ln_blk); atomicAdd(n_ext_total + PGX_CTR_PAIRS_SEEDS, (unsigned long long)ln_seed); atomicAdd(n_ext_total + PGX_CTR_PAIRS_TWO, (unsigned long long)ln_two); }
 #ifdef PGX_FM_STATS
 #pragma unroll
     for (int off = 32; off > 0; off >>= 1) st_wait += __shfl_down(st_wait, off, 64);
@@ -633,11 +669,8 @@
     if (lane == 0) { atomicAdd(n_ext_total + PGX_CTR_ST_PAIR_TRIPS, st_trips); atomicAdd(n_ext_total + PGX_CTR_ST_PAIR_LIVE, st_live); atomicAdd(n_ext_total + PGX_CTR_ST_PAIR_WAIT, st_wait); atomicAdd(n_ext_total + PGX_CTR_ST_PAIR_FRESH, st_fresh); }
 #endif
 }
-#define PGX_PAIRS_INSTANTIATE(...)                                                                                                                \
-    template __global__ void pgx_find_mems_pairs_kernel<__VA_ARGS__>(PgxDevImage, const uint8_t *, const uint64_t *, uint64_t, uint64_t, uint64_t, const uint64_t *, \
-                                                                     pgx_mem *, uint32_t *, unsigned long long *, unsigned long long *, uint64_t, uint64_t, uint32_t, \
-                                                                     uint32_t, pgx_heavy_item *, unsigned long long *, const uint8_t *, const uint32_t *, uint32_t,  \
-                                                                     uint32_t *, uint64_t);
+#define PGX_PAIRS_INSTANTIATE(...) \
+    template __global__ void pgx_find_mems_pairs_kernel<__VA_ARGS__>(PgxPairsArgs);
 PGX_PAIRS_INSTANTIATE(false, false, false, false, false)
 PGX_PAIRS_INSTANTIATE(true, false, false, false, false)
 PGX_PAIRS_INSTANTIATE(false, true, false, false, false)
```

New measurement: 1.161 billion, median of 6. 1.02x the previous value.
